# wyf0912/ContextGS

Measured on AMD Instinct MI355X. Metric: views/sec fwd+bwd @1920×1080, 1M anchors, higher is better.
Workload: dtype f32

## Files before the change

### contextgs_amd/_lib.py

```python
from __future__ import annotations

import ctypes as C
import os
import threading

_HERE = os.path.dirname(os.path.abspath(__file__))
LIB_PATH = os.environ.get("CGS_LIB_PATH") or os.path.join(_HERE, "libcgs_hip.so")

_lib = None
_lock = threading.Lock()

c_void_p, c_int, c_int32, c_int64, c_size_t, c_float = C.c_void_p, C.c_int, C.c_int32, C.c_int64, C.c_size_t, C.c_float


class RasterCfg(C.Structure):
    _fields_ = [
        ("image_height", c_int32),
        ("image_width", c_int32),
        ("tanfovx", c_float),
        ("tanfovy", c_float),
        ("scale_modifier", c_float),
        ("prefiltered", c_int32),
        ("debug", c_int32),
        ("viewmatrix", c_void_p),
        ("projmatrix", c_void_p),
        ("campos", c_void_p),
        ("bg", c_void_p),
    ]


class AdamTensor(C.Structure):
    _fields_ = [
        ("p", c_void_p),
        ("g", c_void_p),
        ("m", c_void_p),
        ("v", c_void_p),
        ("numel", c_int64),
        ("beta1", C.c_double),
        ("beta2", C.c_double),
        ("width", c_int32),
        ("step_size", c_float),
        ("bias2_sqrt", c_float),
        ("eps", c_float),
        ("weight_decay", c_float),
    ]


_BWD_HEAD = [C.POINTER(RasterCfg), c_int64, c_int64]
_BWD_WS = [c_void_p, c_size_t, c_void_p, c_size_t, c_void_p, c_size_t]
_BWD_TAIL = [c_void_p, c_size_t, c_void_p]
_BWD_FORMS = _BWD_HEAD + [c_void_p] * 3 + [c_int32] * 2 + [c_void_p] * 5 + _BWD_WS + [c_void_p]
_BWD_MAPS = _BWD_FORMS + [c_void_p] * 3
_BWD_OUT = [c_void_p] * 8 + _BWD_TAIL
_BWD_FEAT = [c_void_p, c_int32, c_void_p, c_void_p]

SIGNATURES = {
    "cgs_version": (c_int, []),
    "cgs_last_error": (C.c_char_p, []),
    "cgs_filter": (c_int, [C.POINTER(RasterCfg), c_int64, c_void_p, c_void_p, c_void_p, c_void_p, c_void_p]),
    "cgs_filter_voxel": (c_int, [C.POINTER(RasterCfg), c_int64, c_void_p, c_void_p, c_int64, c_int, c_void_p, c_void_p, c_void_p]),
    "cgs_raster_geom_bytes": (c_size_t, [c_int64]),
    "cgs_raster_bin_bytes": (c_size_t, [c_int64, c_int64]),
    "cgs_raster_img_bytes": (c_size_t, [c_int32, c_int32]),
    "cgs_raster_bwd_scratch_bytes": (c_size_t, [c_int64]),
    "cgs_raster_preprocess": (c_int, [C.POINTER(RasterCfg), c_int64, c_void_p, c_void_p, c_void_p, c_void_p,
                                      c_void_p, c_void_p, c_size_t, c_void_p, C.POINTER(c_int64), c_void_p]),
    "cgs_raster_preprocess_launch": (c_int, [C.POINTER(RasterCfg), c_int64, c_void_p, c_void_p, c_void_p, c_void_p,
                                             c_void_p, c_void_p, c_size_t, c_void_p, c_void_p, C.POINTER(C.c_uint64)]),
    "cgs_raster_preprocess_launch_ex": (c_int, [C.POINTER(RasterCfg), c_int64, c_void_p, c_void_p, c_void_p, c_int32, c_int32,
                                                c_void_p, c_void_p, c_void_p, c_void_p, c_void_p, c_size_t, c_void_p, c_void_p,
                                                C.POINTER(C.c_uint64)]),
    "cgs_raster_backward_ex": (c_int, _BWD_FORMS + _BWD_OUT),
    "cgs_raster_render_aux": (c_int, [C.POINTER(RasterCfg), c_int64, c_int64, c_void_p, c_size_t, c_void_p, c_size_t,
                                      c_void_p, c_size_t, c_void_p, c_void_p, c_void_p, c_void_p]),
    "cgs_raster_backward_aux": (c_int, _BWD_MAPS + _BWD_OUT),
    "cgs_raster_bwd_aux_scratch_bytes": (c_size_t, [c_int64]),
    "cgs_raster_preprocess_launch_opt": (c_int, [C.POINTER(RasterCfg), c_int64, c_void_p, c_void_p, c_void_p, c_int32, c_int32,
                                                 c_void_p, c_void_p, c_void_p, c_void_p, c_void_p, c_size_t, c_void_p, c_void_p,
                                                 C.POINTER(C.c_uint64), C.c_uint32]),
    "cgs_raster_backward_opt": (c_int, _BWD_MAPS + _BWD_OUT + [C.c_uint32]),
    "cgs_raster_render_features": (c_int, [C.POINTER(RasterCfg), c_int64, c_int64, c_void_p, c_size_t, c_void_p, c_size_t,
                                           c_void_p, c_size_t, c_void_p, c_int32, c_void_p, c_void_p]),
    "cgs_raster_backward_feat": (c_int, _BWD_MAPS + _BWD_OUT + [C.c_uint32] + _BWD_FEAT),
    "cgs_raster_bwd_abs_scratch_bytes": (c_size_t, [c_int64]),
    "cgs_raster_backward_abs": (c_int, _BWD_MAPS + _BWD_OUT + [C.c_uint32] + _BWD_FEAT),
    "cgs_raster_bwd_det_bytes": (c_size_t, [c_int64, c_int64, c_int32]),
    "cgs_raster_backward_det": (c_int, _BWD_MAPS + _BWD_OUT + [C.c_uint32, c_int32, c_void_p, c_size_t]),
    "cgs_raster_render_geom": (c_int, [C.POINTER(RasterCfg), c_int64, c_int64, c_void_p, c_size_t, c_void_p, c_size_t,
                                       c_void_p, c_size_t, c_void_p, c_void_p, c_void_p, c_void_p, c_void_p]),
    "cgs_raster_backward_geom": (c_int, _BWD_MAPS + _BWD_OUT + [C.c_uint32] + _BWD_FEAT + [c_void_p] * 4),
    "cgs_raster_contrib": (c_int, [C.POINTER(RasterCfg), c_int64, c_int64, c_void_p, c_size_t, c_void_p, c_size_t, c_void_p,
                                   c_size_t, c_void_p, c_int64] + [c_void_p] * 8),
    "cgs_raster_camera_bytes": (c_size_t, [c_int64]),
    "cgs_raster_camera_backward": (c_int, [C.POINTER(RasterCfg), c_int64, c_void_p, c_void_p, c_int32, c_int32, c_void_p, c_void_p,
                                           c_void_p, c_void_p, c_void_p, c_void_p, c_size_t, c_void_p, c_void_p, C.c_uint32,
                                           c_void_p, c_void_p, c_void_p, c_void_p, c_size_t, c_void_p]),
    "cgs_gaussian_normals_fwd": (c_int, [C.POINTER(RasterCfg), c_int64] + [c_void_p] * 5),
    "cgs_gaussian_normals_bwd": (c_int, [C.POINTER(RasterCfg), c_int64] + [c_void_p] * 6),
    "cgs_depth_normals_fwd": (c_int, [c_int32, c_int32, c_float, c_float, c_float] + [c_void_p] * 3),
    "cgs_depth_normals_bwd": (c_int, [c_int32, c_int32, c_float, c_float, c_float] + [c_void_p] * 4),
    "cgs_normal_consistency_fwd": (c_int, [c_int32, c_int32, c_float, c_float, c_float] + [c_void_p] * 5),
    "cgs_normal_consistency_bwd": (c_int, [c_int32, c_int32, c_float, c_float, c_float] + [c_void_p] * 7),
    "cgs_filter_cov": (c_int,[C.POINTER(RasterCfg), c_int64, c_void_p, c_void_p, c_void_p, c_void_p]),
    "cgs_raster_preprocess_wait": (c_int, [C.c_uint64, C.POINTER(c_int64)]),
    "cgs_raster_preprocess_wait2": (c_int, [C.c_uint64, C.POINTER(c_int64), C.POINTER(c_int)]),
    "cgs_debug_set_depth_keys_full": (c_int, [c_int]),
    "cgs_sort_depth_keys": (c_int, [c_void_p, c_void_p, c_void_p, c_void_p, c_void_p, c_int64, c_void_p, c_size_t, c_void_p,
                                    C.c_uint32, c_void_p]),
    "cgs_raster_render_spec": (c_int, [C.POINTER(RasterCfg), c_int64, c_int64, c_void_p, c_size_t, c_void_p, c_size_t,
                                       c_void_p, c_size_t, c_void_p, c_void_p]),
    "cgs_raster_render": (c_int, [C.POINTER(RasterCfg), c_int64, c_int64, c_void_p, c_size_t, c_void_p, c_size_t,
                                  c_void_p, c_size_t, c_void_p, c_void_p]),
    "cgs_raster_backward": (c_int, _BWD_HEAD + [c_void_p] * 6 + _BWD_WS + [c_void_p] * 7 + _BWD_TAIL),
    "cgs_raster_preprocess_expand_launch": (c_int, [C.POINTER(RasterCfg), c_int64, c_int] + [c_void_p] * 9 + [c_int64, c_void_p,
                                                    c_void_p, c_void_p, c_void_p, c_size_t, c_void_p, c_void_p, C.POINTER(C.c_uint64)]),
    "cgs_raster_stats": (c_int, [C.POINTER(RasterCfg), c_void_p, c_size_t, c_void_p, c_void_p]),
    "cgs_debug_set_bin_mode": (c_int, [c_int]),
    "cgs_debug_bin_compare": (c_int, [C.POINTER(RasterCfg), c_int64, c_int64, c_int64, c_void_p, c_size_t, c_void_p, c_size_t,
                                      c_void_p, c_size_t, c_void_p, c_size_t, c_void_p, c_void_p, c_void_p]),
    "cgs_build_info": (C.c_char_p, []),
    "cgs_scan_scratch_bytes": (c_size_t, [c_int64]),
    "cgs_scan_exclusive_u32": (c_int, [c_void_p, c_void_p, c_int64, c_void_p, c_size_t, c_void_p]),
    "cgs_sort_scratch_bytes": (c_size_t, [c_int64]),
    "cgs_sort_pairs_u32": (c_int, [c_void_p, c_void_p, c_void_p, c_void_p, c_void_p, c_void_p, c_int64, c_int, c_int,
                                   c_void_p, c_size_t, c_void_p]),
    "cgs_quantize_anchor": (c_int, [c_void_p, c_void_p, c_void_p, c_int64, c_int, c_void_p, c_void_p, c_void_p]),
    "cgs_ste_multistep": (c_int, [c_void_p, c_void_p, c_int64, c_int64, c_int, c_void_p, c_void_p]),
    "cgs_entropy_gaussian_fwd": (c_int, [c_void_p, c_void_p, c_void_p, c_void_p, c_int64, c_int64, c_void_p, c_int,
                                         c_void_p, c_void_p]),
    "cgs_entropy_gaussian_bwd": (c_int, [c_void_p, c_void_p, c_void_p, c_void_p, c_int64, c_int64, c_void_p, c_int,
                                         c_void_p, c_void_p, c_void_p, c_void_p, c_void_p, c_void_p]),
    "cgs_mlp2_forward": (c_int, [c_int, c_int, c_int, c_int, c_void_p, c_int64, c_void_p, c_void_p, c_void_p, c_void_p,
                                 c_void_p, c_int64, c_void_p, c_int64, c_void_p]),
    "cgs_mlp2_backward": (c_int, [c_int, c_int, c_int, c_int, c_void_p, c_int64, c_void_p, c_void_p, c_void_p, c_void_p, c_void_p,
                                  c_int64, c_void_p, c_void_p, c_int64, c_int, c_void_p, c_void_p, c_void_p, c_void_p,
                                  c_void_p, c_void_p, c_int64, c_void_p, c_size_t, c_void_p]),
    "cgs_mlp2_backward_rows": (c_int, [c_int, c_int, c_int, c_int, c_void_p, c_int64, c_void_p, c_void_p, c_void_p, c_void_p,
                                       c_void_p, c_int64, c_void_p, c_void_p, c_int64, c_int, c_void_p, c_void_p, c_void_p,
                                       c_void_p, c_void_p, c_void_p, c_void_p, c_int64, c_void_p, c_size_t, c_void_p]),
    "cgs_mlp_wgrad_scratch_bytes": (c_size_t, []),
    "cgs_mlp2_wgrad": (c_int, [c_int, c_int, c_int, c_void_p, c_int64, c_void_p, c_void_p, c_int64, c_void_p, c_void_p, c_void_p,
                               c_void_p, c_void_p, c_int64, c_void_p, c_size_t, c_void_p]),
    "cgs_anchor_mlp3_wgrad": (c_int, [c_void_p, c_int64] + [c_void_p] * 9 + [c_int64, c_void_p, c_size_t, c_void_p]),
    "cgs_anchor_mlp3_forward": (c_int, [c_void_p, c_int64, c_void_p, c_void_p, c_void_p, c_void_p, c_void_p, c_void_p,
                                        c_void_p, c_void_p, c_int64, c_void_p]),
    "cgs_anchor_mlp3_backward": (c_int, [c_void_p, c_int64, c_void_p, c_void_p, c_void_p, c_void_p, c_void_p, c_void_p,
                                         c_void_p, c_void_p, c_void_p, c_int64, c_void_p, c_void_p, c_void_p, c_void_p,
                                         c_void_p, c_void_p, c_void_p, c_int64, c_void_p, c_size_t, c_void_p]),
    "cgs_anchor_mlp3_forward_rows": (c_int, [c_void_p] * 13 + [c_int64, c_void_p]),
    "cgs_anchor_mlp3_backward_rows": (c_int, [c_void_p] * 22 + [c_int64, c_void_p, c_size_t, c_void_p]),
    "cgs_anchor_mlp3_forward_rows_t": (c_int, [c_void_p] * 13 + [c_int64, c_int, c_void_p]),
    "cgs_anchor_mlp3_backward_rows_t": (c_int, [c_void_p] * 22 + [c_int64, c_int, c_void_p, c_size_t, c_void_p]),
    "cgs_rowcat_fwd": (c_int, [c_int, c_void_p, c_void_p, c_void_p, c_void_p, c_int64, c_void_p, c_void_p]),
    "cgs_rowcat_bwd": (c_int, [c_int, c_void_p, c_void_p, c_void_p, c_void_p, c_void_p, c_int64, c_void_p, c_void_p]),
    "cgs_anchor_mlp3_layout": (c_int, [c_void_p]),
    "cgs_gather_rows_segmented": (c_int, [c_int, c_void_p, c_void_p, c_void_p, c_void_p, c_int64, c_int, c_void_p, c_void_p]),
    "cgs_scatter_rows_sorted": (c_int, [c_void_p, c_void_p, c_int64, c_int64, c_int, c_void_p, c_void_p]),
    "cgs_add_rows": (c_int, [c_void_p, c_void_p, c_int64, c_int64, c_int, c_void_p, c_void_p]),
    "cgs_weighted_sum_scratch_bytes": (c_size_t, []),
    "cgs_weighted_sum_fwd": (c_int, [c_void_p, c_void_p, c_int64, c_void_p, c_float, c_void_p, c_size_t, c_void_p, c_void_p]),
    "cgs_weighted_sum_bwd": (c_int, [c_void_p, c_void_p, c_int64, c_float, c_void_p, c_void_p, c_void_p]),
    "cgs_gather_rows": (c_int, [c_void_p, c_void_p, c_int64, c_int, c_void_p, c_void_p]),
    "cgs_mark_rows": (c_int, [c_void_p, c_int64, c_int64, C.c_uint32, c_void_p, c_void_p]),
    "cgs_zero_unmarked_rows": (c_int, [c_void_p, C.c_uint32, c_int64, c_int, c_void_p, c_void_p, c_void_p]),
    "cgs_rowcat_fwd_masked": (c_int, [c_int, c_void_p, c_void_p, c_void_p, c_void_p, c_void_p, c_int64, c_void_p, c_void_p]),
    "cgs_rowcat_bwd_masked": (c_int, [c_int, c_void_p, c_void_p, c_void_p, c_void_p, c_void_p, c_void_p, c_int64, c_void_p,
                                      c_void_p]),
    "cgs_ctx_gather_bwd": (c_int, [c_void_p, c_int64, c_int64, c_void_p, c_void_p, c_void_p, c_void_p, c_void_p, c_void_p,
                                   c_int, c_int, c_int, c_void_p]),
    "cgs_ctx_gather_bwd_acc": (c_int, [c_void_p, c_int64, c_int64, c_void_p, c_void_p, c_void_p, c_void_p, c_void_p, c_void_p,
                                       c_int, c_int, c_int, c_int, c_void_p]),
    "cgs_noise_quant_fwd": (c_int, [c_void_p, c_void_p, c_void_p, c_void_p, c_void_p, c_int64, c_int, c_int, c_int,
                                    C.c_uint64, c_float, c_float, c_float, c_void_p, c_void_p, c_void_p, c_void_p,
                                    c_void_p, c_void_p]),
    "cgs_hyper_noise_gather": (c_int, [c_void_p, c_void_p, c_int64, c_int, C.c_uint64, c_void_p, c_void_p]),
    "cgs_eb_bits_scratch_bytes": (c_size_t, []),
    "cgs_eb_bits_fwd": (c_int, [c_void_p, c_void_p, c_void_p, c_int64, c_int, c_void_p, c_size_t, c_void_p, c_void_p]),
    "cgs_eb_bits_bwd": (c_int, [c_void_p, c_void_p, c_void_p, c_void_p, c_int64, c_int, c_void_p, c_void_p, c_void_p]),
    "cgs_rate_finish_fwd": (c_int, [c_void_p, c_int, c_void_p, c_float, C.c_double, C.c_double, C.c_double, c_float, c_void_p,
                                    c_void_p, c_void_p]),
    "cgs_rate_finish_bwd": (c_int, [c_void_p, c_int, c_float, C.c_double, C.c_double, C.c_double, c_void_p, c_void_p, c_void_p]),
    "cgs_rate_finish_bwd4": (c_int, [c_void_p, c_void_p, c_void_p, c_void_p, c_int, c_float, C.c_double, C.c_double, C.c_double, c_void_p,
                                     c_void_p, c_void_p]),
    "cgs_ctx_choose_blocks": (c_size_t, [c_int64]),
    "cgs_ctx_choose_flags": (c_int, [c_void_p, c_int64, c_void_p, c_void_p, C.c_uint64, c_float, c_void_p, c_void_p, c_void_p,
                                     c_void_p, c_int, c_void_p, c_void_p, c_void_p, c_void_p]),
    "cgs_ctx_choose_slot_ints": (c_int, []),
    "cgs_ctx_choose_flags_slots": (c_int, [c_void_p, c_int64, c_void_p, c_void_p, C.c_uint64, c_float, c_void_p, c_void_p, c_void_p,
                                           c_void_p, c_int, c_void_p, c_void_p, c_void_p, c_int, c_void_p]),
    "cgs_ctx_choose_compact": (c_int, [c_void_p, c_void_p, c_void_p, c_int64, c_void_p, c_int, c_void_p, c_void_p, c_void_p,
                                       c_void_p, c_void_p, c_void_p]),
    "cgs_means_accum_doubles": (c_size_t, []),
    "cgs_means_finalize": (c_int, [c_void_p, c_int64, c_int64, c_int64, c_void_p, c_void_p]),
    "cgs_noise_quant_bwd": (c_int, [c_void_p, c_void_p, c_void_p, c_void_p, c_void_p, c_int64, c_int, c_int, c_int,
                                    C.c_uint64, c_float, c_float, c_float, c_void_p, c_void_p, c_void_p, c_void_p,
                                    c_void_p, c_void_p, c_void_p, c_void_p, c_void_p, c_void_p, c_void_p]),
    "cgs_ctx_level_fwd": (c_int, [c_int, c_void_p, c_int64, c_void_p, c_void_p, c_void_p, c_void_p, c_int64, c_void_p, c_void_p,
                                  c_int64] + [c_void_p] * 8 + [C.c_uint64, c_float, c_float, c_float] + [c_void_p] * 7),
    "cgs_ctx_level_bwd_scratch_bytes": (c_size_t, []),
    "cgs_ctx_level_bwd": (c_int, [c_int] + [c_void_p] * 9 + [c_int64, C.c_uint64, c_float, c_float, c_float, c_void_p, c_int64] +
                          [c_void_p] * 4 + [c_int64] + [c_void_p] * 11 + [c_size_t, c_void_p]),
    "cgs_ctx_level_bwd2": (c_int, [c_int] + [c_void_p] * 9 + [c_int64, C.c_uint64, c_float, c_float, c_float, c_void_p, c_int64] +
                           [c_void_p] * 4 + [c_int64] + [c_void_p] * 12 + [c_size_t, c_void_p]),
    "cgs_ctx_level_hidden_bytes": (c_size_t, [c_int64]),
    "cgs_ctx_level_fwd_h": (c_int, [c_int, c_void_p, c_int64, c_void_p, c_void_p, c_void_p, c_void_p, c_int64, c_void_p, c_void_p,
                                    c_int64] + [c_void_p] * 8 + [C.c_uint64, c_float, c_float, c_float] + [c_void_p] * 8),
    "cgs_ctx_level_bwd_h": (c_int, [c_int] + [c_void_p] * 9 + [c_int64, C.c_uint64, c_float, c_float, c_float, c_void_p, c_int64] +
                            [c_void_p] * 4 + [c_int64] + [c_void_p] * 13 + [c_size_t, c_void_p]),
    "cgs_level_rate_fwd": (c_int, [c_void_p] * 9 + [c_int, c_int64, c_int, c_int, c_int64, c_void_p, c_void_p]),
    "cgs_level_rate_bwd": (c_int, [c_void_p] * 9 + [c_int, c_int64, c_int, c_int, c_int64] + [c_void_p] * 7 +
                           [c_int, c_void_p]),
    "cgs_rate_sub_fwd": (c_int, [c_int, c_void_p, c_int64, c_void_p, c_int64] + [c_void_p] * 10 + [c_int, c_void_p, c_void_p]),
    "cgs_rate_sub_bwd_scratch_bytes": (c_size_t, [c_int, c_int64]),
    "cgs_rate_sub_bwd": (c_int, [c_int, c_void_p, c_int64, c_void_p, c_int64] + [c_void_p] * 10 + [c_int] + [c_void_p] * 12 +
                         [c_size_t, c_void_p]),
    "cgs_eb_likelihood_fwd": (c_int, [c_void_p, c_void_p, c_int64, c_int, c_void_p, c_void_p]),
    "cgs_eb_likelihood_bwd": (c_int, [c_void_p, c_void_p, c_void_p, c_int64, c_int, c_void_p, c_void_p, c_void_p]),
    "cgs_ac_max_bytes": (c_size_t, [c_int64]),
    "cgs_cdf_float_to_u16_host": (c_int, [c_void_p, c_int64, c_int, c_void_p]),
    "cgs_ac_encode_table_host": (c_int, [c_void_p, c_int, c_void_p, c_int64, c_void_p, c_size_t, C.POINTER(c_size_t)]),
    "cgs_ac_decode_table_host": (c_int, [c_void_p, c_int, c_int64, c_void_p, c_size_t, c_void_p]),
    "cgs_ac_encode_const_host": (c_int, [c_void_p, c_int, c_void_p, c_int64, c_void_p, c_size_t, C.POINTER(c_size_t)]),
    "cgs_ac_decode_const_host": (c_int, [c_void_p, c_int, c_int64, c_void_p, c_size_t, c_void_p]),
    "cgs_gaussian_stream_minmax": (c_int, [c_void_p, c_void_p, c_int64, c_void_p, c_int, c_void_p, c_void_p, c_void_p]),
    "cgs_gaussian_ac_encode": (c_int, [c_void_p, c_void_p, c_void_p, c_void_p, c_int64, c_void_p, c_int, c_void_p,
                                       c_void_p, c_void_p, c_void_p, c_void_p, c_void_p, c_void_p]),
    "cgs_gaussian_ac_decode": (c_int, [c_void_p, c_void_p, c_void_p, c_int64, c_void_p, c_int, c_void_p, c_void_p,
                                       c_void_p, c_void_p, c_void_p, c_void_p]),
    "cgs_gaussian_ac_encode_lanes": (c_int, [c_void_p, c_void_p, c_void_p, c_void_p, c_int64, c_void_p, c_int, c_void_p,
                                             c_void_p, c_void_p, c_void_p, c_void_p, c_void_p, c_void_p]),
    "cgs_gaussian_ac_decode_lanes": (c_int, [c_void_p, c_void_p, c_void_p, c_int64, c_void_p, c_int, c_void_p, c_void_p,
                                             c_void_p, c_void_p, c_void_p, c_void_p, c_void_p]),
    "cgs_lanes_compact": (c_int, [c_void_p, c_void_p, c_void_p, c_void_p, c_int, c_void_p, c_int, c_void_p]),
    "cgs_lanes_block_slot_bytes": (c_size_t, [c_int64, c_int]),
    "cgs_table_ac_encode_lanes": (c_int, [c_void_p, c_void_p, c_void_p, c_int, c_void_p, c_int, c_void_p, c_void_p, c_void_p,
                                          c_void_p, c_void_p, c_void_p, c_void_p]),
    "cgs_table_ac_decode_lanes": (c_int, [c_void_p, c_void_p, c_int, c_void_p, c_int, c_void_p, c_void_p, c_void_p, c_int64,
                                          c_void_p, c_void_p, c_void_p, c_int64, c_void_p, c_void_p]),
    "cgs_bernoulli_ac_encode": (c_int, [c_void_p, C.c_uint32, c_void_p, c_int, c_void_p, c_void_p, c_void_p, c_void_p, c_void_p]),
    "cgs_bernoulli_ac_decode": (c_int, [C.c_uint32, c_void_p, c_int, c_void_p, c_void_p, c_void_p, c_void_p]),
    "cgs_means3_scratch_bytes": (c_size_t, []),
    "cgs_means3": (c_int, [c_void_p, c_int64, c_void_p, c_int64, c_int, c_void_p, c_int64, c_void_p, c_size_t, c_void_p,
                           c_void_p]),
    "cgs_mask_ste_fwd":(c_int, [c_void_p, c_int64, c_int, c_void_p, c_void_p, c_void_p]),
    "cgs_mask_ste_bwd": (c_int, [c_void_p, c_void_p, c_int64, c_void_p, c_void_p]),
    "cgs_knn_scratch_bytes": (c_size_t, [c_int64]),
    "cgs_knn_mean_dist2": (c_int, [c_void_p, c_int64, c_void_p, c_void_p, c_size_t, c_void_p]),
    "cgs_streams_compact":(c_int, [c_void_p, c_void_p, c_void_p, c_void_p, c_int, c_void_p, c_void_p]),
    "cgs_anchor_order_scratch_bytes": (c_size_t, [c_int64]),
    "cgs_anchor_order": (c_int, [c_void_p, c_int64, c_void_p, c_void_p, c_void_p, c_void_p, c_size_t, c_void_p]),
    "cgs_anchor_pack_slot_bytes": (c_size_t, [c_int]),
    "cgs_anchor_pack": (c_int, [c_void_p, c_int64, c_int, c_void_p, c_void_p, c_void_p, c_void_p, c_void_p, c_void_p]),
    "cgs_anchor_unpack": (c_int, [c_void_p, c_int64, c_int, c_void_p, c_void_p, c_void_p, c_void_p, c_void_p, c_void_p]),
    "cgs_pread_ranges": (c_int, [c_int, c_void_p, c_void_p, c_void_p, c_void_p, c_int]),
    "cgs_pwrite_ranges": (c_int, [c_int, c_void_p, c_void_p, c_void_p, c_void_p, c_int]),
    "cgs_gaussian_cdf_table": (c_int, [c_void_p, c_void_p, c_void_p, c_int64, c_int64, c_int, c_int, c_void_p, c_void_p]),
    "cgs_rans_max_bytes": (c_size_t, [c_int64]),
    "cgs_rans_encode_host": (c_int, [c_void_p, c_int, c_int64, c_void_p, c_int, c_void_p, c_void_p, c_int, c_void_p,
                                     c_size_t, C.POINTER(c_size_t)]),
    "cgs_rans_decode_host": (c_int, [c_void_p, c_size_t, c_int, c_int64, c_void_p, c_int, c_void_p, c_void_p, c_int,
                                     c_void_p]),
    "cgs_rans_decode_rows_host": (c_int, [c_void_p, c_size_t, c_int, c_int64, c_void_p, c_int, c_void_p, c_void_p, c_int,
                                          c_void_p, c_void_p, c_int64]),
    "cgs_prof_enable": (c_int, [c_int]),
    "cgs_prof_count": (c_int, []),
    "cgs_prof_name": (C.c_char_p, [c_int]),
    "cgs_prof_read": (c_int, [c_int, C.POINTER(C.c_double), C.POINTER(c_int64)]),
    "cgs_densify_stats": (c_int, [c_int64, c_int] + [c_void_p] * 11),
    "cgs_densify_stats_ex": (c_int, [c_int64, c_int] + [c_void_p] * 11 + [c_int32, c_int32]),
    "cgs_nonzero_scratch_bytes": (c_size_t, [c_int64]),
    "cgs_nonzero_launch": (c_int, [c_void_p, c_int64, c_void_p, c_void_p, c_size_t, c_void_p, C.POINTER(C.c_uint64)]),
    "cgs_nonzero_wait": (c_int, [C.c_uint64, C.POINTER(c_int64)]),
    "cgs_level_key_range": (c_int, [c_void_p, c_int64, c_void_p, c_void_p, c_void_p]),
    "cgs_level_unique_scratch_bytes": (c_size_t, [c_int64]),
    "cgs_level_unique": (c_int, [c_void_p, c_int64, c_void_p, c_void_p, c_void_p, c_void_p, c_void_p, c_void_p,
                                 C.POINTER(c_int64), c_void_p, c_size_t, c_void_p]),
    "cgs_compact_rows": (c_int, [c_int, c_void_p, c_void_p, c_void_p, c_void_p, c_float, c_void_p, c_int64, c_void_p]),
    "cgs_adam_step": (c_int, [c_int, C.POINTER(AdamTensor), c_void_p, c_int64, c_void_p]),
    "cgs_l1_ssim_partials": (c_size_t, [c_int, c_int, c_int]),
    "cgs_l1_ssim_fwd": (c_int, [c_void_p, c_void_p, c_int, c_int, c_int, c_void_p, c_void_p, c_void_p]),
    "cgs_l1_ssim_bwd": (c_int, [c_void_p, c_void_p, c_void_p, c_void_p, c_int, c_int, c_int, c_void_p, c_void_p]),
    "cgs_l1_ssim_finish": (c_int, [c_void_p, c_int, c_int, c_int, c_float, c_void_p, c_void_p]),
    "cgs_l1_ssim_bwd_loss": (c_int, [c_void_p, c_void_p, c_void_p, c_void_p, c_void_p, c_float, c_int, c_int, c_int, c_void_p, c_void_p]),
    "cgs_reg_partials": (c_size_t, [c_int64]),
    "cgs_scaling_reg_fwd": (c_int, [c_void_p, c_int64, c_void_p, c_void_p]),
    "cgs_scaling_reg_bwd": (c_int, [c_void_p, c_void_p, c_int64, c_void_p, c_void_p]),
    "cgs_sigmoid_mean_fwd": (c_int, [c_void_p, c_int64, c_void_p, c_void_p]),
    "cgs_sigmoid_mean_bwd": (c_int, [c_void_p, c_void_p, c_int64, c_void_p, c_void_p]),
    "cgs_anchor_gen_count": (c_int, [c_void_p] * 14 + [c_int64, c_int, C.POINTER(c_int64), c_void_p]),
    "cgs_anchor_gen_write": (c_int, [c_void_p] * 20 + [c_int64, c_int, c_void_p]),
    "cgs_anchor_gen_bwd_scratch_bytes": (c_size_t, [c_int64, c_int]),
    "cgs_anchor_gen_backward": (c_int, [c_void_p] * 32 + [c_int64, c_int, c_int, c_void_p, c_size_t, c_void_p]),
    "cgs_expand_scratch_bytes": (c_size_t, [c_int64, c_int]),
    "cgs_expand_count": (c_int, [c_int64, c_int, c_void_p, c_void_p, c_void_p, c_void_p, c_void_p, c_void_p, c_void_p,
                                 c_size_t, C.POINTER(c_int64), c_void_p]),
    "cgs_expand_count_launch": (c_int, [c_int64, c_int, c_void_p, c_void_p, c_void_p, c_void_p, c_void_p, c_void_p, c_void_p,
                                        c_size_t, c_void_p, C.POINTER(C.c_uint64)]),
    "cgs_expand_count_wait": (c_int, [C.c_uint64, C.POINTER(c_int64)]),
    "cgs_expand_write": (c_int, [c_int64, c_int] + [c_void_p] * 15),
    "cgs_expand_backward": (c_int, [c_int64, c_int] + [c_void_p] * 22),
}


def lib() -> C.CDLL:
    global _lib
    if _lib is not None:
        return _lib
    with _lock:
        if _lib is not None:
            return _lib
        import torch
        if not os.path.exists(LIB_PATH):
            raise RuntimeError(
                f"{LIB_PATH} not found. Build it with `python -m contextgs_amd.build` "
                "(or __graft_entry__.build()); contextgs_amd has no CPU fallback.")
        handle = C.CDLL(LIB_PATH)
        for name, (res, args) in SIGNATURES.items():
            fn = getattr(handle, name)
            fn.restype = res
            fn.argtypes = args
        if os.environ.get("CGS_LIB_PATH"):
            import sys
            from . import build as _build
            info = (handle.cgs_build_info() or b"").decode()
            want = _build.source_digest()
            if info.split("|")[0] != want and not os.environ.get("CGS_LIB_ALLOW_STALE"):
                raise RuntimeError(f"CGS_LIB_PATH={LIB_PATH} was built from other sources ({info.split('|')[0][:12]}... vs "
                                   f"{want[:12]}...): rebuild it (tools/variant_lib.sh) or set CGS_LIB_ALLOW_STALE=1")
            print(f"[contextgs_amd] variant library {LIB_PATH} ({info[:12]}...|{info.split('|')[-1]})", file=sys.stderr)
        if os.environ.get("CGS_BIN_MODE"):
            if handle.cgs_debug_set_bin_mode(int(os.environ["CGS_BIN_MODE"])) != 0:
                raise RuntimeError("CGS_BIN_MODE must be 0, 1 or 2")
        _lib = handle
    return _lib


def check(rc: int, what: str) -> None:
    if rc != 0:
        msg = lib().cgs_last_error()
        raise RuntimeError(f"{what} failed (code {rc}): {msg.decode() if msg else '?'}")


def ptr(t) -> int:
    if t is None:
        return None
    assert t.is_contiguous(), "libcgs_hip takes dense row-major buffers"
    return t.data_ptr()


_raw_stream = None


def current_stream() -> int:
    global _raw_stream
    import torch
    if _raw_stream is None:
        _raw_stream = getattr(torch._C, "_cuda_getCurrentRawStream", False)
    if _raw_stream:
        return _raw_stream(torch.cuda.current_device())
    return torch.cuda.current_stream().cuda_stream


def require_device(*tensors) -> None:
    import torch
    cur = None
    for t in tensors:
        if t is None:
            continue
# ... 9 lines not shown
```

### contextgs_amd/csrc/cgs_internal.h

```cpp
#pragma once
#include <hip/hip_runtime.h>
#include <stdint.h>
#include <stdio.h>
#include "../../include/cgs.h"

#define CGS_TILE 16
#define CGS_WAVE 64

void cgs_set_error(const char *fmt, ...);
uint64_t cgs_new_ticket(int kind);

#define CGS_CHECK_HIP(expr)                                                   \
    do {                                                                      \
        hipError_t e__ = (expr);                                              \
        if (e__ != hipSuccess) {                                              \
            cgs_set_error("%s:%d: %s -> %s", __FILE__, __LINE__, #expr,       \
                          hipGetErrorString(e__));                            \
            return CGS_ERR_HIP;                                               \
        }                                                                     \
    } while (0)

#define CGS_CHECK_LAUNCH(stream, debug)                                       \
    do {                                                                      \
        CGS_CHECK_HIP(hipGetLastError());                                     \
// ... 28 lines not shown
    template <typename T> T *take(size_t count) {
        off = cgs_align_up(off, 256);
        size_t bytes = count * sizeof(T);
        T *r = (T *)(base ? base + off : nullptr);
        off += bytes;
        if (base && off > cap) ok = false;
        return r;
    }
    size_t used() const { return cgs_align_up(off, 256); }
};

struct CgsGeom {
    float4 *rec;
    uint32_t *depth_key;
    uint32_t *tiles;
    uint2 *rect;
    uint32_t *order;
    uint32_t *offsets;
    uint32_t *sort_a;
    uint32_t *sort_b;
    uint32_t *sort_c;
    uint32_t *sort_d;
    uint32_t *total;
    void *scratch;
    size_t scratch_bytes;
};

struct CgsBin {
    uint32_t *tile_key_a;
    uint32_t *tile_key_b;
    uint32_t *gid_a;
    uint32_t *gid_b;
    uint32_t *tile_key_c;
    uint32_t *gid_sorted;
    void *scratch;
    size_t scratch_bytes;
    uint32_t *bk_tab;
    uint32_t *bk_counts;
    uint32_t *bk_scan;
    void *bk_scan_scratch;
    size_t bk_scan_scratch_bytes;
};

struct CgsImg {
    uint2 *ranges;
    float *final_T;
    uint32_t *n_contrib;
    uint32_t *tile_last;
    uint32_t *tile_order;
};

size_t cgs_geom_carve(CgsGeom *g, void *ws, size_t bytes, int64_t P);
size_t cgs_bin_carve(CgsBin *b, void *ws, size_t bytes, int64_t P, int64_t R);
size_t cgs_img_carve(CgsImg *im, void *ws, size_t bytes, int32_t H, int32_t W);

int cgs_launch_preprocess(const cgs_raster_cfg *cfg, int64_t P, const float *means3D,
                          const float *colors, const float *opacities, const float *scales,
                          const float *rotations, CgsGeom &g, int32_t *radii, bool filter_only,
                          hipStream_t stream, bool aa = false);
int cgs_launch_emit_pairs(const cgs_raster_cfg *cfg, int64_t P, CgsGeom &g, CgsBin &b,
                          hipStream_t stream);
int cgs_launch_ranges(const cgs_raster_cfg *cfg, int64_t R, CgsBin &b, CgsImg &im,
                      hipStream_t stream);
int cgs_launch_gather_rects(int64_t P, CgsGeom &g, hipStream_t stream);
bool cgs_tile_bin16_ok(int tile_bits);
bool cgs_tile_bin_buckets_ok(const cgs_raster_cfg *cfg);
bool cgs_tile_bin_buckets_fits(int64_t R);
int64_t cgs_bucket_count_slots(int64_t R);
size_t cgs_bucket_tab_words(void);
int cgs_launch_tile_bin_buckets(const cgs_raster_cfg *cfg, int64_t P, int64_t R, CgsGeom &g, CgsBin &b, CgsImg &im,
                                hipStream_t stream, const uint32_t *R_dev);
int cgs_launch_tile_bin16(const cgs_raster_cfg *cfg, int64_t P, int64_t R, int tile_bits, CgsGeom &g, CgsBin &b, CgsImg &im,
                          hipStream_t stream, const uint32_t *R_dev = nullptr);
int cgs_launch_blend_fwd_rows(const cgs_raster_cfg *cfg, CgsGeom &g, CgsBin &b, CgsImg &im, float *out_color,
                              hipStream_t stream);
int cgs_launch_blend_bwd_rows(const cgs_raster_cfg *cfg, CgsGeom &g, CgsBin &b, CgsImg &im, const float *dL_dout,
                              float *dL_dmean2D_px, float *dL_dconic, float *dL_dopacity, float *dL_dcolors,
                              hipStream_t stream, float *dL_dabs_px = nullptr);
int cgs_launch_tile_order(const cgs_raster_cfg *cfg, CgsImg &im, hipStream_t stream);
int cgs_launch_blend_bwd_rows_det(const cgs_raster_cfg *cfg, int64_t P, int64_t R, CgsGeom &g, CgsBin &b, CgsImg &im,
                                  const float *dL_dout, const uint32_t *slot_base, void *slots, float *dL_dmean2D_px,
                                  float *dL_dconic, float *dL_dopacity, float *dL_dcolors, float *dL_dz, float *dL_dabs_px,
                                  hipStream_t stream);
int cgs_launch_blend_fwd(const cgs_raster_cfg *cfg, CgsGeom &g, CgsBin &b, CgsImg &im,
                         float *out_color, hipStream_t stream);
int cgs_launch_blend_bwd(const cgs_raster_cfg *cfg, CgsGeom &g, CgsBin &b, CgsImg &im,
                         const float *dL_dout, float *dL_dmean2D_px, float *dL_dconic,
                         float *dL_dopacity, float *dL_dcolors, hipStream_t stream, float *dL_dabs_px = nullptr);
int cgs_launch_preprocess_bwd(const cgs_raster_cfg *cfg, int64_t P, const float *means3D,
                              const float *scales, const float *rotations,
                              const int32_t *radii, const float *dL_dmean2D_px,
                              const float *dL_dconic, float *dL_dmeans3D, float *dL_dmeans2D,
                              float *dL_dscales, float *dL_drotations, hipStream_t stream,
                              const float *aa_opacities = nullptr, float *aa_dL_dopacities = nullptr,
                              const float *dL_dabs_px = nullptr);

struct CgsExpandSrc {
    int64_t n_anchor;
    int K;
    const uint8_t *flags;
    const uint32_t *pos;
    const float *anchor, *gscaling, *offsets, *neural_opacity, *color_in, *cov_in;
    const int64_t *src_row;
};
int cgs_launch_expand_preprocess(const cgs_raster_cfg *cfg, const CgsExpandSrc &x, float *scaling_out, float *xyz_out,
                                 float *rot_out, CgsGeom &g, int32_t *radii, hipStream_t stream);

#ifdef __HIPCC__
__device__ __forceinline__ int64_t cgs_xcd_item(int64_t n_items) {
    const int64_t chunk = (n_items + 7) / 8;
    const int64_t t = (int64_t)(blockIdx.x & 7u) * chunk + (int64_t)(blockIdx.x >> 3);
    return ((int64_t)(blockIdx.x >> 3) < chunk && t < n_items) ? t : -1;
}
#endif
static inline unsigned cgs_xcd_grid(int64_t n_items) { return (unsigned)(8 * ((n_items + 7) / 8)); }
#define CGS_TICKET_SLOTS 8
#define CGS_TICKET_BYTES ((CGS_TICKET_SLOTS + 1) * 128)
#ifdef __HIPCC__
__device__ __forceinline__ void cgs_publish(double *slot, double v) {
    const unsigned long long old = atomicExch((unsigned long long *)slot, (unsigned long long)__double_as_longlong(v));
    asm volatile("" ::"v"(old) : "memory");
}
__device__ __forceinline__ double cgs_published(const double *slot) {
    return __longlong_as_double((long long)__hip_atomic_load((const unsigned long long *)slot, __ATOMIC_RELAXED, __HIP_MEMORY_SCOPE_AGENT));
}
__device__ __forceinline__ bool cgs_ticket_last(unsigned int *t) {
    const unsigned nb = gridDim.x, S = CGS_TICKET_SLOTS, slot = blockIdx.x % S;
    const unsigned in_slot = (nb - slot + S - 1) / S;
    if (atomicAdd(&t[32 * (1 + slot)], 1u) != in_slot - 1u) return false;
    t[32 * (1 + slot)] = 0u;
    if (atomicAdd(&t[0], 1u) != (nb < S ? nb : S) - 1u) return false;
    t[0] = 0u;
    __threadfence();
    return true;
}
#endif
int cgs_launch_digit_scan(uint32_t *hist, uint32_t *totals, int digits, int64_t ncols, hipStream_t stream);

static inline int cgs_tiles_x(const cgs_raster_cfg *c) { return (c->image_width + CGS_TILE - 1) / CGS_TILE; }
static inline int cgs_tiles_y(const cgs_raster_cfg *c) { return (c->image_height + CGS_TILE - 1) / CGS_TILE; }

int cgs_launch_wgrad2(const float *P, int64_t ldp, int DA, const float *Q, int64_t ldq, int DB, float *dW, float *db,
                      int64_t n, int num_cus, void *scratch, size_t scratch_bytes, hipStream_t s);
size_t cgs_wgrad_scratch_bytes_for(int num_cus);
int cgs_launch_mlp2_bwd_recompute(int in, int hid, int out, const float *X, int64_t ldx, const float *W1,
                                  const float *b1, const float *W2, const float *dY, int64_t ldy, float *dX,
                                  int64_t lddx, int acc, float *dZ1, float *dW2, float *db2, int64_t n, int num_cus,
                                  void *scratch, size_t scratch_bytes, hipStream_t s);
struct CgsWgProduct { const float *P; int64_t ldp; int DA; const float *Q; int64_t ldq; int DB; float *dW; float *db; };
int cgs_launch_wgrad_multi(const CgsWgProduct *prods, int nprod, int64_t n, int num_cus, void *scratch,
                           size_t scratch_bytes, hipStream_t s);
int cgs_launch_wgrad_reduce(const float *partial, int blocks, const CgsWgProduct *prods, int nprod, hipStream_t s);
int cgs_launch_wgrad_reduce_assign(const float *partial, int blocks, const CgsWgProduct *prods, int nprod, hipStream_t s);
```

### contextgs_amd/csrc/mlp_wgrad.hip

```cpp
#include "cgs_internal.h"
#include "mlp_frag.h"

typedef int i32x4 __attribute__((ext_vector_type(4)));

struct WgStream {
    __amdgpu_buffer_rsrc_t rsrc;
    int ld4;
    int col4;
    bool m[4];
    bool partial;
    bool narrow;
};

__device__ __forceinline__ WgStream wg_stream(const float *base, int64_t ld, int dim, int group, int c, int64_t r_begin,
                                              int64_t r_end, bool narrow = false) {
    WgStream st;
    st.narrow = narrow;
    const float *p = base + r_begin * ld;
    const int64_t rows = r_end - r_begin;
    const uint32_t bytes = rows > 0 ? (uint32_t)(((rows - 1) * ld + dim) * 4) : 0u;
    st.rsrc = __builtin_amdgcn_make_buffer_rsrc((void *)p, 0, bytes, 0x00020000);
    st.ld4 = (int)ld * 4;
    const int col0 = narrow ? 64 * group + c : 64 * group + 4 * c;
    st.col4 = col0 * 4;
// ... 157 lines not shown
        if (e < DADB) dW[e] += t;
        else if (db) db[e - DADB] += t;
    }
}

static int wgrad_blocks_per_cu() {
    static int v = 0;
    if (!v) {
        const char *e = nullptr;
        v = e ? atoi(e) : 1;
        if (v < 1) v = 1;
        if (v > 2) v = 2;
    }
    return v;
}

size_t cgs_wgrad_scratch_bytes_for(int num_cus) { return (size_t)2 * num_cus * 25000 * sizeof(float); }

int cgs_launch_wgrad2(const float *P, int64_t ldp, int DA, const float *Q, int64_t ldq, int DB, float *dW, float *db,
                      int64_t n, int num_cus, void *scratch, size_t scratch_bytes, hipStream_t s) {
    if (n <= 0) return CGS_OK;
    constexpr int UNR = 2;
    const int GA = (DA + 63) / 64, GB = (DB + 63) / 64, npairs = GA * GB;
    const int E = DA * DB + DA;
    if (npairs > 8 || E > WG_MAX_E) { cgs_set_error("wgrad: %d x %d not supported", DA, DB); return CGS_ERR_ARG; }
    const int nsub = 8 / npairs;
    int64_t blocks = (n + 255) / 256;
    int64_t cap = (int64_t)(scratch ? wgrad_blocks_per_cu() : 1) * num_cus;
    if (scratch) {
        const int64_t fit = (int64_t)(scratch_bytes / ((size_t)E * sizeof(float)));
        if (fit < 1) { cgs_set_error("wgrad: scratch too small"); return CGS_ERR_ARG; }
        if (cap > fit) cap = fit;
    }
    if (blocks > cap) blocks = cap;
    int64_t rpb = (n + blocks - 1) / blocks;
    const int64_t quantum = (int64_t)nsub * 4 * UNR;
    rpb = (rpb + quantum - 1) / quantum * quantum;
    blocks = (n + rpb - 1) / rpb;
#define WG_LAUNCH(U)                                                                                                  \
    hipLaunchKernelGGL((wgrad4_kernel<U>), dim3((unsigned)blocks), dim3(512), 0, s, P, ldp, DA, Q, ldq, DB, dW, db, n, rpb, \
                       GB, npairs, nsub, (float *)scratch)
    if (UNR == 4) WG_LAUNCH(4);
    else if (UNR == 1) WG_LAUNCH(1);
    else WG_LAUNCH(2);
#undef WG_LAUNCH
    CGS_CHECK_HIP(hipGetLastError());
    if (scratch) {
        hipLaunchKernelGGL(wgrad_reduce_kernel, dim3((unsigned)((E + 63) / 64)), dim3(256), 0, s, (const float *)scratch,
                           (int)blocks, E, DA * DB, dW, db);
        CGS_CHECK_HIP(hipGetLastError());
    }
    return CGS_OK;
}

#define WGM_MAX_TASKS 16
#define WGM_MAX_PROD 4
#define WGM_MAX_E 25000
struct WgmTask {
    const float *P, *Q;
    int ldp, ldq, DA, DB, ga, gb, img_off;
    int narrow;
};
struct WgmArgs {
    WgmTask t[WGM_MAX_TASKS];
    int ntask, nsub, E;
};
struct WgmProducts {
    float *dW[WGM_MAX_PROD], *db[WGM_MAX_PROD];
    int off[WGM_MAX_PROD + 1], dadb[WGM_MAX_PROD];
    int nprod;
};

template <int UNR>
__global__ void __launch_bounds__(1024)
    wgrad_multi_kernel(WgmArgs a, int64_t n, int64_t rows_per_block, float *__restrict__ partial) {
    __shared__ float img[WGM_MAX_E];
    const int tid = threadIdx.x, lane = tid & 63, g = lane >> 4, c = lane & 15;
    const int wave = __builtin_amdgcn_readfirstlane(tid >> 6);
    for (int i = tid; i < a.E; i += 1024) img[i] = 0.f;
    const int ti = wave % a.ntask, sub = wave / a.ntask;
    const int nsub = sub < a.nsub ? a.nsub : 0;
    const float *P = nullptr, *Q = nullptr;
    int ldp = 0, ldq = 0, DA = 0, DB = 0, ga = 0, gb = 0, img_off = 0, narrow = 0;
#pragma unroll
    for (int k = 0; k < WGM_MAX_TASKS; ++k)
        if (k == ti) {
            P = a.t[k].P; Q = a.t[k].Q; ldp = a.t[k].ldp; ldq = a.t[k].ldq; DA = a.t[k].DA; DB = a.t[k].DB;
            ga = a.t[k].ga; gb = a.t[k].gb; img_off = a.t[k].img_off; narrow = a.t[k].narrow;
        }
    const bool nA = narrow & 1, nB = narrow & 2;
    f32x4 acc[4][4], bsum = (f32x4){0.f, 0.f, 0.f, 0.f};
#pragma unroll
    for (int ja = 0; ja < 4; ++ja)
#pragma unroll
        for (int jb = 0; jb < 4; ++jb) acc[ja][jb] = (f32x4){0.f, 0.f, 0.f, 0.f};
    if (nsub > 0) {
        const int64_t r_begin = (int64_t)blockIdx.x * rows_per_block;
        const int64_t r_end = min(n, r_begin + rows_per_block);
        const WgStream sa = wg_stream(P, ldp, DA, ga, c, r_begin, r_end, nA);
        const WgStream sb = wg_stream(Q, ldq, DB, gb, c, r_begin, r_end, nB);
        const int rows = (int)(r_end - r_begin), stride = nsub * 4 * UNR;
        int row0 = sub * 4 * UNR;
        WgFrag<UNR> f0, f1;
        wg_fetch<UNR>(f0, sa, sb, row0, g);
        for (; row0 < rows; row0 += 2 * stride) {
            wg_fetch<UNR>(f1, sa, sb, row0 + stride, g);
            WG_FENCE();
            wg_consume<UNR>(f0, sa, sb, acc, bsum);
            WG_FENCE();
            wg_fetch<UNR>(f0, sa, sb, row0 + 2 * stride, g);
            WG_FENCE();
            wg_consume<UNR>(f1, sa, sb, acc, bsum);
            WG_FENCE();
        }
    }
    __syncthreads();
    for (int s = 0; s < a.nsub; ++s) {
        if (nsub > 0 && sub == s) {
            float *const outW = img + img_off;
            float *const outb = outW + DA * DB;
#pragma unroll
            for (int ja = 0; ja < 4; ++ja) {
                if (ja > 0 && nA) break;
#pragma unroll
                for (int r = 0; r < 4; ++r) {
                    const int ar = nA ? 64 * ga + 4 * g + r : 64 * ga + 4 * (4 * g + r) + ja;
                    if (ar >= DA) continue;
#pragma unroll
                    for (int jb = 0; jb < 4; ++jb) {
                        if (jb > 0 && nB) break;
                        const int b = nB ? 64 * gb + c : 64 * gb + 4 * c + jb;
                        if (b < DB) outW[ar * DB + b] += acc[ja][jb][r];
                    }
                }
            }
            if (gb == 0) {
#pragma unroll
                for (int j = 0; j < 4; ++j) {
                    if (j > 0 && nA) break;
                    float v = bsum[j];
                    v += __shfl_xor(v, 16);
                    v += __shfl_xor(v, 32);
                    const int ac = nA ? 64 * ga + c : 64 * ga + 4 * c + j;
                    if (g == 0 && ac < DA) outb[ac] += v;
                }
            }
        }
        __syncthreads();
    }
    float *dst = partial + (int64_t)blockIdx.x * a.E;
    for (int i = tid; i < a.E; i += 1024) dst[i] = img[i];
}

__global__ void __launch_bounds__(256)
    wgrad_multi_reduce_kernel(const float *__restrict__ partial, int blocks, int E, WgmProducts pr, int assign) {
    __shared__ float s[4][64];
    const int tx = threadIdx.x & 63, ty = threadIdx.x >> 6;
    const int e = blockIdx.x * 64 + tx;
    float a0 = 0.f, a1 = 0.f, a2 = 0.f, a3 = 0.f;
    if (e < E) {
        int b = ty;
        for (; b + 12 < blocks; b += 16) {
            a0 += partial[(int64_t)b * E + e];
            a1 += partial[(int64_t)(b + 4) * E + e];
            a2 += partial[(int64_t)(b + 8) * E + e];
            a3 += partial[(int64_t)(b + 12) * E + e];
        }
        for (; b < blocks; b += 4) a0 += partial[(int64_t)b * E + e];
    }
    s[ty][tx] = (a0 + a1) + (a2 + a3);
    __syncthreads();
    if (ty == 0 && e < E) {
        const float t = (s[0][tx] + s[1][tx]) + (s[2][tx] + s[3][tx]);
        int k = 0;
#pragma unroll
        for (int q = 1; q < WGM_MAX_PROD; ++q)
            if (q < pr.nprod && e >= pr.off[q]) k = q;
        float *dW = nullptr, *db = nullptr;
        int off = 0, dadb = 0;
#pragma unroll
        for (int q = 0; q < WGM_MAX_PROD; ++q)
            if (q == k) { dW = pr.dW[q]; db = pr.db[q]; off = pr.off[q]; dadb = pr.dadb[q]; }
        const int le = e - off;
        if (le < dadb) dW[le] = assign ? t : dW[le] + t;
        else if (db) db[le - dadb] = assign ? t : db[le - dadb] + t;
    }
}

#ifndef WG_TAIL_MIN_WAVES
#define WG_TAIL_MIN_WAVES 1
#endif
template <int UNR>
__global__ void __launch_bounds__(512, WG_TAIL_MIN_WAVES)
    wgrad_tail_kernel(const float *__restrict__ P, int64_t ldp, int DA, const float *__restrict__ Q, int64_t ldq, int DB,
                      int64_t n, int64_t rows_per_block, int GA, int nsub, float *__restrict__ partial) {
    __shared__ float img[128 * 80 + 128];
    const int tid = threadIdx.x, lane = tid & 63, g = lane >> 4, c = lane & 15;
    const int wave = __builtin_amdgcn_readfirstlane(tid >> 6);
    const int E = DA * DB + DA;
    for (int i = tid; i < E; i += 512) img[i] = 0.f;
    const int ga = wave % GA, sub = wave / GA;
    const bool active = sub < nsub;
    f32x4 acc[4][4], accT[4], bsum = (f32x4){0.f, 0.f, 0.f, 0.f};
#pragma unroll
    for (int ja = 0; ja < 4; ++ja) {
        accT[ja] = (f32x4){0.f, 0.f, 0.f, 0.f};
#pragma unroll
        for (int jb = 0; jb < 4; ++jb) acc[ja][jb] = (f32x4){0.f, 0.f, 0.f, 0.f};
    }
    if (active) {
        const int64_t r_begin = (int64_t)blockIdx.x * rows_per_block;
        const int64_t r_end = min(n, r_begin + rows_per_block);
        const WgStream sa = wg_stream(P, ldp, DA, ga, c, r_begin, r_end);
        const WgStream sb = wg_stream(Q, ldq, DB, 0, c, r_begin, r_end);
        const WgStream st = wg_stream(Q, ldq, DB, 1, c, r_begin, r_end, true);
        const int rows = (int)(r_end - r_begin), stride = nsub * 4 * UNR;
        int row0 = sub * 4 * UNR;
        WgFrag<UNR> f0, f1;
        float t0[UNR], t1[UNR];
        auto fetch = [&](WgFrag<UNR> &f, float (&t)[UNR], int rel) {
            wg_fetch<UNR>(f, sa, sb, rel, g);
#pragma unroll
            for (int q = 0; q < UNR; ++q) t[q] = wg_load4(st, rel + 4 * q + g)[0];
        };
        auto consume = [&](const WgFrag<UNR> &f, const float (&t)[UNR]) {
            wg_consume<UNR>(f, sa, sb, acc, bsum);
#pragma unroll
            for (int q = 0; q < UNR; ++q) {
                const f32x4 a = wg_mask(sa, f.a[q]);
                const float tv = st.m[0] ? t[q] : 0.f;
#pragma unroll
                for (int ja = 0; ja < 4; ++ja) accT[ja] = frag_mfma(a[ja], tv, accT[ja]);
            }
        };
        fetch(f0, t0, row0);
        for (; row0 < rows; row0 += 2 * stride) {
            fetch(f1, t1, row0 + stride);
            WG_FENCE();
            consume(f0, t0);
            WG_FENCE();
            fetch(f0, t0, row0 + 2 * stride);
            WG_FENCE();
            consume(f1, t1);
            WG_FENCE();
        }
    }
    __syncthreads();
    for (int s = 0; s < nsub; ++s) {
        if (active && sub == s) {
            float *const outW = img, *const outb = img + DA * DB;
#pragma unroll
            for (int ja = 0; ja < 4; ++ja)
#pragma unroll
                for (int r = 0; r < 4; ++r) {
                    const int ar = 64 * ga + 4 * (4 * g + r) + ja;
                    if (ar >= DA) continue;
#pragma unroll
                    for (int jb = 0; jb < 4; ++jb) outW[ar * DB + 4 * c + jb] += acc[ja][jb][r];
                    if (64 + c < DB) outW[ar * DB + 64 + c] += accT[ja][r];
                }
#pragma unroll
            for (int j = 0; j < 4; ++j) {
                float v = bsum[j];
                v += __shfl_xor(v, 16);
                v += __shfl_xor(v, 32);
                const int ac = 64 * ga + 4 * c + j;
                if (g == 0 && ac < DA) outb[ac] += v;
            }
        }
        __syncthreads();
    }
    float *dst = partial + (int64_t)blockIdx.x * E;
    for (int i = tid; i < E; i += 512) dst[i] = img[i];
}

static int launch_wgrad_tail(const CgsWgProduct &p, int64_t n, int num_cus, void *scratch, size_t scratch_bytes, hipStream_t s) {
    constexpr int UNR = 2;
    const int GA = (p.DA + 63) / 64, nsub = 8 / GA, E = p.DA * p.DB + p.DA;
    int64_t blocks = (n + 255) / 256;
    int64_t cap = (int64_t)num_cus * 2;
    const int64_t fit_blocks = (int64_t)(scratch_bytes / ((size_t)E * sizeof(float)));
    if (cap > fit_blocks) cap = fit_blocks;
    if (blocks > cap) blocks = cap;
    int64_t rpb = (n + blocks - 1) / blocks;
    const int64_t quantum = (int64_t)nsub * 4 * UNR;
    rpb = (rpb + quantum - 1) / quantum * quantum;
    blocks = (n + rpb - 1) / rpb;
    hipLaunchKernelGGL((wgrad_tail_kernel<UNR>), dim3((unsigned)blocks), dim3(512), 0, s, p.P, p.ldp, p.DA, p.Q, p.ldq, p.DB, n, rpb,
                       GA, nsub, (float *)scratch);
    CGS_CHECK_HIP(hipGetLastError());
    hipLaunchKernelGGL(wgrad_reduce_kernel, dim3((unsigned)((E + 63) / 64)), dim3(256), 0, s, (const float *)scratch, (int)blocks, E,
                       p.DA * p.DB, p.dW, p.db);
    CGS_CHECK_HIP(hipGetLastError());
    return CGS_OK;
}

int cgs_launch_wgrad_multi(const CgsWgProduct *prods, int nprod, int64_t n, int num_cus, void *scratch,
                           size_t scratch_bytes, hipStream_t s) {
    if (n <= 0 || nprod <= 0) return CGS_OK;
    if (nprod == 1 && scratch && prods[0].DB > 64 && prods[0].DB <= 80 && prods[0].DA <= 128 && prods[0].db &&
        (size_t)(prods[0].DA * prods[0].DB + prods[0].DA) * sizeof(float) <= scratch_bytes)
        return launch_wgrad_tail(prods[0], n, num_cus, scratch, scratch_bytes, s);
    WgmArgs a;
    WgmProducts pr;
    int ntask = 0, E = 0;
    bool fits = scratch != nullptr && nprod <= WGM_MAX_PROD;
    for (int k = 0; k < nprod && fits; ++k) {
        const CgsWgProduct &p = prods[k];
        const int GA = (p.DA + 63) / 64, GB = (p.DB + 63) / 64;
        pr.dW[k] = p.dW; pr.db[k] = p.db; pr.off[k] = E; pr.dadb[k] = p.DA * p.DB;
        for (int ga = 0; ga < GA && fits; ++ga)
            for (int gb = 0; gb < GB; ++gb) {
                if (ntask >= WGM_MAX_TASKS) { fits = false; break; }
                const int narrow = (p.DA - 64 * ga <= 16 ? 1 : 0) | (p.DB - 64 * gb <= 16 ? 2 : 0);
                a.t[ntask++] = WgmTask{p.P, p.Q, (int)p.ldp, (int)p.ldq, p.DA, p.DB, ga, gb, E, narrow};
            }
        E += p.DA * p.DB + p.DA;
    }
    if (fits && E > WGM_MAX_E) fits = false;
    if (fits && (size_t)E * sizeof(float) > scratch_bytes) fits = false;
    if (!fits) {
        for (int k = 0; k < nprod; ++k) {
            const CgsWgProduct &p = prods[k];
            int rc = cgs_launch_wgrad2(p.P, p.ldp, p.DA, p.Q, p.ldq, p.DB, p.dW, p.db, n, num_cus, scratch, scratch_bytes, s);
            if (rc) return rc;
        }
        return CGS_OK;
    }
    for (int k = ntask; k < WGM_MAX_TASKS; ++k) a.t[k] = WgmTask{nullptr, nullptr, 0, 0, 0, 0, 0, 0, 0, 0};
    {
        bool uniform = ntask > 0;
        for (int k = 1; k < ntask; ++k) uniform = uniform && a.t[k].narrow == a.t[0].narrow;
        for (int k = 0; k < ntask; ++k)
            if (!uniform) a.t[k].narrow = 0;
        a.nsub = 16 / ntask;
    }
    for (int k = nprod; k < WGM_MAX_PROD; ++k) { pr.dW[k] = nullptr; pr.db[k] = nullptr; pr.off[k] = E; pr.dadb[k] = 0; }
    pr.off[WGM_MAX_PROD] = E;
    pr.nprod = nprod;
#ifndef WGM_UNR
#define WGM_UNR 2
#endif
    constexpr int UNR = WGM_UNR;
    a.ntask = ntask;
    a.E = E;
#ifndef WGM_MIN_ROWS
#define WGM_MIN_ROWS 256
#endif
    int64_t blocks = (n + WGM_MIN_ROWS - 1) / WGM_MIN_ROWS;
    int64_t cap = num_cus;
    const int64_t fit_blocks = (int64_t)(scratch_bytes / ((size_t)E * sizeof(float)));
    if (cap > fit_blocks) cap = fit_blocks;
    if (blocks > cap) blocks = cap;
    int64_t rpb = (n + blocks - 1) / blocks;
    const int64_t quantum = (int64_t)a.nsub * 4 * UNR;
    rpb = (rpb + quantum - 1) / quantum * quantum;
    blocks = (n + rpb - 1) / rpb;
    hipLaunchKernelGGL((wgrad_multi_kernel<UNR>), dim3((unsigned)blocks), dim3(1024), 0, s, a, n, rpb, (float *)scratch);
    CGS_CHECK_HIP(hipGetLastError());
    hipLaunchKernelGGL(wgrad_multi_reduce_kernel, dim3((unsigned)((E + 63) / 64)), dim3(256), 0, s, (const float *)scratch,
                       (int)blocks, E, pr, 0);
    CGS_CHECK_HIP(hipGetLastError());
    return CGS_OK;
}

static int wgrad_reduce_launch(const float *partial, int blocks, const CgsWgProduct *prods, int nprod, int assign, hipStream_t s);
int cgs_launch_wgrad_reduce(const float *partial, int blocks, const CgsWgProduct *prods, int nprod, hipStream_t s) {
    return wgrad_reduce_launch(partial, blocks, prods, nprod, 0, s);
}
int cgs_launch_wgrad_reduce_assign(const float *partial, int blocks, const CgsWgProduct *prods, int nprod, hipStream_t s) {
    return wgrad_reduce_launch(partial, blocks, prods, nprod, 1, s);
}
static int wgrad_reduce_launch(const float *partial, int blocks, const CgsWgProduct *prods, int nprod, int assign, hipStream_t s) {
    if (nprod <= 0 || nprod > WGM_MAX_PROD || blocks <= 0) { cgs_set_error("wgrad_reduce: bad args"); return CGS_ERR_ARG; }
    WgmProducts pr;
    int E = 0;
    for (int k = 0; k < nprod; ++k) {
        pr.dW[k] = prods[k].dW; pr.db[k] = prods[k].db; pr.off[k] = E; pr.dadb[k] = prods[k].DA * prods[k].DB;
        E += prods[k].DA * prods[k].DB + prods[k].DA;
    }
    for (int k = nprod; k < WGM_MAX_PROD; ++k) { pr.dW[k] = nullptr; pr.db[k] = nullptr; pr.off[k] = E; pr.dadb[k] = 0; }
    pr.off[WGM_MAX_PROD] = E;
    pr.nprod = nprod;
    hipLaunchKernelGGL(wgrad_multi_reduce_kernel, dim3((unsigned)((E + 63) / 64)), dim3(256), 0, s, partial, blocks, E, pr, assign);
    CGS_CHECK_HIP(hipGetLastError());
    return CGS_OK;
}
```

### contextgs_amd/csrc/rate_sub.hip

```cpp
#include "cgs_internal.h"
#include "mlp_frag.h"
#include "buf_access.h"
#include "ctx_rows.h"
#include "rate_math.h"

#define RS_NB 6
#define RS_NT2 12
#define RS_OP 192
#define RS_SA 116
#define RS_OUT 175
#define RS_K 10
#ifndef RS_WAVES_F
#define RS_WAVES_F 8
#endif
#ifndef RS_WAVES_B
#define RS_WAVES_B 8
#endif

__host__ __device__ __forceinline__ int rs_w2row(int op) {
    const int u = op >> 4, b = u >> 1, sc = u & 1, l = op & 15;
    if (b < 3) { const int e = 16 * b + l; return sc ? 50 + e : e; }
    if (b == 3) {
        if (l < 2) return sc ? 98 + l : 48 + l;
        if (l >= 4 && l < 8) return (sc ? 106 : 100) + (l - 4);
        if (l >= 8 && l < 10) return (sc ? 110 : 104) + (l - 8);
        return -1;
    }
    const int e = (b == 4 ? 0 : 16) + l;
    if (e >= 30) return -1;
    return (sc ? 142 : 112) + e;
}

__device__ __forceinline__ int rs_w2perm(int row) {
    int sc = 0, e = row, base;
    if (row < 100) { sc = row >= 50; e = row - 50 * sc; base = e < 48 ? 32 * (e >> 4) + (e & 15) : 96 + (e - 48); }
    else if (row < 112) { sc = row >= 106; e = row - 100 - 6 * sc; base = e < 4 ? 100 + e : 104 + (e - 4); }
    else { sc = row >= 142; e = row - 112 - 30 * sc; base = e < 16 ? 128 + e : 160 + (e - 16); }
    return base + 16 * sc;
}

struct RsArgs {
    const float *X;
    const int64_t *loc;
    const float *W1, *b1, *W2, *b2;
    const float *yf, *ys, *yo, *Q;
    const float *masks;
    const float *x_means;
    int64_t n, m;
    int use_clamp;
    float *sums;
    const float *g_sums;
    float *side_f, *side_s, *side_o, *side_Q;
    float *dx_sub;
    float *d_masks;
    float *dZ2t, *Ht, *dZ1t, *Xt;
};

template <int IN>
struct RsOps {
    f32x4 xb[ClShape<IN>::NTI];
    ClRow y;
    f32x4 q3, mk4, mk5;
};

template <int IN, bool BWD>
__global__ void __launch_bounds__((BWD ? RS_WAVES_B : RS_WAVES_F) * 64) rs_main_kernel(RsArgs a) {
    constexpr int RS_WAVES = BWD ? RS_WAVES_B : RS_WAVES_F;
    constexpr int NTI = ClShape<IN>::NTI, XP = ClShape<IN>::XP, SB = ClShape<IN>::SB;
    __shared__ __attribute__((aligned(16))) float W2n[RS_OP * RS_SA];
    __shared__ __attribute__((aligned(16))) float W1n[CL_HP * SB];
    __shared__ float b1s[CL_HP];
    __shared__ float b2p[RS_OP];
    __shared__ float part[RS_WAVES][3];
    const int tid = threadIdx.x, nthr = RS_WAVES * 64;
    for (int i = tid; i < (RS_OP * RS_SA + CL_HP * SB) / 4; i += nthr) {
        float *dst = i < RS_OP * RS_SA / 4 ? W2n + 4 * i : W1n + 4 * (i - RS_OP * RS_SA / 4);
        *(f32x4 *)dst = (f32x4){0.f, 0.f, 0.f, 0.f};
    }
    for (int i = tid; i < CL_HP; i += nthr) b1s[i] = i < CL_HID ? a.b1[i] : 0.f;
    for (int i = tid; i < RS_OP; i += nthr) {
        const int row = rs_w2row(i);
        b2p[i] = row >= 0 ? a.b2[row] : 0.f;
    }
    __syncthreads();
    {
        constexpr int N2 = (RS_OUT - 3) * CL_HID / 4;
        constexpr int PER = (N2 + RS_WAVES * 64 - 1) / (RS_WAVES * 64);
        f32x4 v[PER];
#pragma unroll
        for (int k = 0; k < PER; ++k) {
            const int i = tid + k * nthr;
            v[k] = i < N2 ? *(const f32x4 *)(a.W2 + 4 * i) : (f32x4){0.f, 0.f, 0.f, 0.f};
        }
#pragma unroll
        for (int k = 0; k < PER; ++k) {
            const int i = tid + k * nthr;
            if (i < N2) {
                const int row = (4 * i) / CL_HID, h = (4 * i) % CL_HID;
                *(f32x4 *)(W2n + rs_w2perm(row) * RS_SA + h) = v[k];
            }
        }
        constexpr int N1 = CL_HID * IN;
        constexpr int PER1 = (N1 + RS_WAVES * 64 - 1) / (RS_WAVES * 64);
        float w[PER1];
#pragma unroll
        for (int k = 0; k < PER1; ++k) {
            const int i = tid + k * nthr;
            w[k] = i < N1 ? a.W1[i] : 0.f;
        }
#pragma unroll
        for (int k = 0; k < PER1; ++k) {
            const int i = tid + k * nthr;
            if (i < N1) W1n[(i / IN) * SB + i % IN] = w[k];
        }
    }
    __syncthreads();

    const int lane = tid & 63, wave = tid >> 6, g = lane >> 4, c = lane & 15;
    const int64_t m = a.m, ntiles = (m + 15) / 16;
    const uint64_t nb = (uint64_t)a.n, mb = (uint64_t)m, tb = (uint64_t)ntiles * 64;
    const ClBuf bX = cl_buf(a.X, nb * IN * 4), bLoc = cl_buf(a.loc, mb * 8), bQ = cl_buf(a.Q, nb * 12),
                bM = cl_buf(a.masks, mb * RS_K * 4);
    const ClRowBufs YB = {cl_buf(a.yf, nb * CL_D * 4), cl_buf(a.ys, nb * CL_S * 4), cl_buf(a.yo, nb * CL_O * 4)};
    const bool has_masks = a.masks != nullptr;
    float xm[3] = {0.f, 0.f, 0.f}, gsum[3] = {0.f, 0.f, 0.f};
    if (a.use_clamp) { xm[0] = a.x_means[0]; xm[1] = a.x_means[1]; xm[2] = a.x_means[2]; }
    if (BWD) { gsum[0] = a.g_sums[0]; gsum[1] = a.g_sums[1]; gsum[2] = a.g_sums[2]; }
    const int use_clamp = a.use_clamp;
    const int lo4 = (4 * g) / 3, lo5 = (16 + 4 * g) / 3;

    auto idx_issue = [&](int64_t s) { return cl_li64(bLoc, cl_sel(s < m, (uint32_t)s * 8)); };
    auto op_issue = [&](RsOps<IN> &op, int64_t s, int64_t r) {
        const bool v = s < m;
        cl_xrow_load<IN>(bX, (uint32_t)r * (IN * 4), g, v, op.xb);
        cl_row_issue(op.y, YB, (uint32_t)r, g, v);
        op.q3 = cl_l96(bQ, cl_sel(v, (uint32_t)r * 12));
        op.mk4 = cl_l64(bM, cl_sel(v && has_masks, (uint32_t)s * (RS_K * 4) + (uint32_t)lo4 * 4));
        op.mk5 = cl_l64(bM, cl_sel(v && has_masks, (uint32_t)s * (RS_K * 4) + (uint32_t)lo5 * 4));
    };

    const int64_t tstride = (int64_t)gridDim.x * RS_WAVES;
    int64_t tile = (int64_t)blockIdx.x * RS_WAVES + wave;
    float accb[3] = {0.f, 0.f, 0.f};
    RsOps<IN> opn;
    int64_t rn;
    {
        const int64_t s0 = tile < ntiles ? tile * 16 + c : m;
        const int64_t r0 = idx_issue(s0);
        op_issue(opn, s0, r0);
        rn = idx_issue(s0 + tstride * 16);
    }
    for (; tile < ntiles; tile += tstride) {
        const int64_t s = tile * 16 + c, sn = s + tstride * 16;
        const bool valid = s < m;
        asm volatile("" ::: "memory");
        RsOps<IN> op = opn;
        cl_xrow_mask<IN>(g, op.xb);
        cl_row_mask(op.y, g);
        CLB_FENCE();
        op_issue(opn, sn, rn);
        rn = idx_issue(sn + tstride * 16);
        CLB_FENCE();

        f32x4 acc1[CL_NT1];
#pragma unroll
        for (int t = 0; t < CL_NT1; ++t) acc1[t] = (f32x4){0.f, 0.f, 0.f, 0.f};
        {
            f32x4 wc[4], wn[4];
#pragma unroll
            for (int i = 0; i < 4; ++i) wc[i] = *(const f32x4 *)(W1n + (16 * i + c) * SB + 4 * g);
#pragma unroll
            for (int grp = 0; grp < 2 * NTI; ++grp) {
                const int q = grp >> 1, t0 = (grp & 1) * 4, nt = (grp & 1) ? 3 : 4;
                if (grp + 1 < 2 * NTI) {
                    const int qn = (grp + 1) >> 1, tn = ((grp + 1) & 1) * 4;
#pragma unroll
                    for (int i = 0; i < 4; ++i)
                        if (tn + i < CL_NT1) wn[i] = *(const f32x4 *)(W1n + (16 * (tn + i) + c) * SB + 16 * qn + 4 * g);
                }
                CLB_FENCE();
#pragma unroll
                for (int j = 0; j < 4; ++j)
#pragma unroll
                    for (int i = 0; i < 4; ++i)
                        if (i < nt) acc1[t0 + i] = frag_mfma(wc[i][j], op.xb[q][j], acc1[t0 + i]);
                CLB_FENCE();
#pragma unroll
                for (int i = 0; i < 4; ++i) wc[i] = wn[i];
            }
        }
#pragma unroll
        for (int t = 0; t < CL_NT1; ++t)
#pragma unroll
            for (int r = 0; r < 4; ++r) acc1[t][r] = fmaxf(acc1[t][r] + b1s[16 * t + 4 * g + r], 0.f);
        uint32_t hpos = 0;
        if (BWD) {
            const ClBuf bXt = cl_buf(a.Xt, tb * XP * 4), bHt = cl_buf(a.Ht, tb * CL_HP * 4);
#pragma unroll
            for (int q = 0; q < NTI; ++q)
#pragma unroll
                for (int r = 0; r < 4; ++r) {
                    const int col = 16 * q + 4 * g + r;
                    const float v = col == IN ? (valid ? 1.f : 0.f) : op.xb[q][r];
                    cl_s32(bXt, (((uint32_t)tile * XP + (uint32_t)col) * 16 + (uint32_t)c) * 4, v);
                }
#pragma unroll
            for (int t = 0; t < CL_NT1; ++t)
#pragma unroll
                for (int r = 0; r < 4; ++r) {
                    const int col = 16 * t + 4 * g + r;
                    const float v = valid ? (col == CL_HID ? 1.f : acc1[t][r]) : 0.f;
                    cl_s32(bHt, (((uint32_t)tile * CL_HP + (uint32_t)col) * 16 + (uint32_t)c) * 4, v);
                    hpos |= acc1[t][r] > 0.f ? (1u << (4 * t + r)) : 0u;
                }
        }
        f32x4 acc2[RS_NT2];
#pragma unroll
        for (int u = 0; u < RS_NT2; ++u) acc2[u] = (f32x4){0.f, 0.f, 0.f, 0.f};
        {
            f32x4 wa = *(const f32x4 *)(W2n + c * RS_SA + 4 * g), wb = *(const f32x4 *)(W2n + (16 + c) * RS_SA + 4 * g);
#pragma unroll
            for (int grp = 0; grp < CL_NT1 * (RS_NT2 / 2); ++grp) {
                const int t = grp / (RS_NT2 / 2), u = 2 * (grp % (RS_NT2 / 2));
                f32x4 na = wa, nb = wb;
                if (grp + 1 < CL_NT1 * (RS_NT2 / 2)) {
                    const int tn = (grp + 1) / (RS_NT2 / 2), un = 2 * ((grp + 1) % (RS_NT2 / 2));
                    na = *(const f32x4 *)(W2n + (16 * un + c) * RS_SA + 16 * tn + 4 * g);
                    nb = *(const f32x4 *)(W2n + (16 * (un + 1) + c) * RS_SA + 16 * tn + 4 * g);
                }
                CLB_FENCE();
#pragma unroll
                for (int r = 0; r < 4; ++r) {
                    acc2[u] = frag_mfma(wa[r], acc1[t][r], acc2[u]);
                    acc2[u + 1] = frag_mfma(wb[r], acc1[t][r], acc2[u + 1]);
                }
                CLB_FENCE();
                wa = na; wb = nb;
            }
        }
        ClRow sd;
        float gq[3] = {0.f, 0.f, 0.f};
        float pm[4] = {0.f, 0.f, 0.f, 0.f};
#pragma unroll
        for (int b = 0; b < RS_NB; ++b) {
            const f32x4 yv = b < 3 ? op.y.F[b] : (b == 3 ? (g == 0 ? op.y.F[3] : op.y.S) : op.y.O[b - 4]);
            f32x4 gxv = (f32x4){0.f, 0.f, 0.f, 0.f};
#pragma unroll
            for (int r = 0; r < 4; ++r) {
                bool slot = true;
                if (b == 3) slot = g == 1 || ((g == 0 || g == 2) && r < 2);
                if (b == 5) slot = g != 3 || r < 2;
                const int kind = b < 3 ? 0 : (b == 3 ? (g == 0 ? 0 : 1) : 2);
                const bool ok = valid && slot;
                const float mean = acc2[2 * b][r] + b2p[32 * b + 4 * g + r];
                const float scale = acc2[2 * b + 1][r] + b2p[32 * b + 16 + 4 * g + r];
                const float q = kind == 0 ? op.q3[0] : (kind == 1 ? op.q3[1] : op.q3[2]);
                const float xmean = kind == 0 ? xm[0] : (kind == 1 ? xm[1] : xm[2]);
                float w = 1.f;
                int wi = 0;
                if (b >= 4) {
                    wi = (b == 4 ? (4 * g + r) / 3 - lo4 : (16 + 4 * g + r) / 3 - lo5);
                    const f32x4 mk = b == 4 ? op.mk4 : op.mk5;
                    if (has_masks) w = wi ? mk[1] : mk[0];
                }
                const RateTerms rt = rate_terms(yv[r], mean, scale, q, xmean, use_clamp);
                if (!BWD) {
                    const float bits = rate_bits(rt) * w;
                    if (kind == 0) accb[0] += ok ? bits : 0.f;
                    else if (kind == 1) accb[1] += ok ? bits : 0.f;
                    else accb[2] += ok ? bits : 0.f;
                } else {
                    const float gb = (kind == 0 ? gsum[0] : (kind == 1 ? gsum[1] : gsum[2])) * w;
                    const RateGrads G = rate_grads(rt, scale, gb);
                    acc2[2 * b][r] = ok ? G.gm : 0.f;
                    acc2[2 * b + 1][r] = ok ? G.gs : 0.f;
                    gxv[r] = ok ? G.gx : 0.f;
                    const float gqv = ok ? G.gq : 0.f;
                    if (kind == 0) gq[0] += gqv;
                    else if (kind == 1) gq[1] += gqv;
                    else gq[2] += gqv;
                    if (b >= 4) {
                        const float bw = ok ? gsum[2] * rate_bits(rt) : 0.f;
                        const int pi = 2 * (b - 4);
                        pm[pi] += wi ? 0.f : bw;
                        pm[pi + 1] += wi ? bw : 0.f;
                    }
                }
            }
            if (BWD) {
                if (b < 3) sd.F[b] = gxv;
                else if (b == 3) { sd.F[3] = gxv; sd.S = gxv; }
                else sd.O[b - 4] = gxv;
            }
        }
        if (!BWD) continue;

        const ClRowBufs SDB = {cl_buf(a.side_f, mb * CL_D * 4), cl_buf(a.side_s, mb * CL_S * 4), cl_buf(a.side_o, mb * CL_O * 4)};
        cl_row_store(sd, SDB, (uint32_t)s, g, valid);
#pragma unroll
        for (int k = 0; k < 3; ++k) {
            gq[k] += __shfl_xor(gq[k], 16);
            gq[k] += __shfl_xor(gq[k], 32);
        }
        cl_s32(cl_buf(a.side_Q, mb * 12), cl_sel(valid && g < 3, (uint32_t)s * 12 + (uint32_t)g * 4), g == 0 ? gq[0] : (g == 1 ? gq[1] : gq[2]));
        if (a.d_masks) {
            float P[4][4];
#pragma unroll
            for (int gg = 0; gg < 4; ++gg)
#pragma unroll
                for (int i = 0; i < 4; ++i) P[gg][i] = __shfl(pm[i], gg * 16 + c, 64);
            float mw[3] = {0.f, 0.f, 0.f};
#pragma unroll
            for (int j = 0; j < 3; ++j) {
                const int k = g < 3 ? 3 * g + j : 9;
#pragma unroll
                for (int gg = 0; gg < 4; ++gg) {
                    const int l4 = (4 * gg) / 3, l5 = (16 + 4 * gg) / 3;
                    mw[j] += (l4 == k ? P[gg][0] : 0.f) + (l4 + 1 == k ? P[gg][1] : 0.f);
                    mw[j] += (l5 == k ? P[gg][2] : 0.f) + (l5 + 1 == k ? P[gg][3] : 0.f);
                }
            }
            const ClBuf bDm = cl_buf(a.d_masks, mb * RS_K * 4);
            const uint32_t o = (uint32_t)s * (RS_K * 4) + (uint32_t)g * 12;
            cl_s96(bDm, cl_sel(valid && g < 3, o), (f32x4){mw[0], mw[1], mw[2], 0.f});
            cl_s32(bDm, cl_sel(valid && g == 3, o), mw[0]);
        }
        {
            const ClBuf bZ2 = cl_buf(a.dZ2t, tb * RS_OP * 4);
#pragma unroll
            for (int u = 0; u < RS_NT2; ++u)
#pragma unroll
                for (int r = 0; r < 4; ++r)
                    cl_s32(bZ2, (((uint32_t)tile * RS_OP + (uint32_t)(16 * u + 4 * g + r)) * 16 + (uint32_t)c) * 4, acc2[u][r]);
        }
        f32x4 adh[CL_NT1];
#pragma unroll
        for (int t = 0; t < CL_NT1; ++t) adh[t] = (f32x4){0.f, 0.f, 0.f, 0.f};
        {
            float wc[CL_NT1], wn[CL_NT1];
#pragma unroll
            for (int t = 0; t < CL_NT1; ++t) wc[t] = W2n[(4 * g) * RS_SA + 16 * t + c];
#pragma unroll
            for (int st = 0; st < 4 * RS_NT2; ++st) {
                const int u = st >> 2, j = st & 3;
                if (st + 1 < 4 * RS_NT2) {
                    const int un = (st + 1) >> 2, jn = (st + 1) & 3;
#pragma unroll
                    for (int t = 0; t < CL_NT1; ++t) wn[t] = W2n[(16 * un + 4 * g + jn) * RS_SA + 16 * t + c];
                }
                CLB_FENCE();
#pragma unroll
                for (int t = 0; t < CL_NT1; ++t) adh[t] = frag_mfma(wc[t], acc2[u][j], adh[t]);
                CLB_FENCE();
#pragma unroll
                for (int t = 0; t < CL_NT1; ++t) wc[t] = wn[t];
            }
        }
        {
            const ClBuf bZ1 = cl_buf(a.dZ1t, tb * CL_HP * 4);
#pragma unroll
            for (int t = 0; t < CL_NT1; ++t)
#pragma unroll
                for (int r = 0; r < 4; ++r) {
                    adh[t][r] = (hpos >> (4 * t + r)) & 1u ? adh[t][r] : 0.f;
                    cl_s32(bZ1, (((uint32_t)tile * CL_HP + (uint32_t)(16 * t + 4 * g + r)) * 16 + (uint32_t)c) * 4, adh[t][r]);
                }
        }
        f32x4 adx[NTI];
#pragma unroll
        for (int v = 0; v < NTI; ++v) adx[v] = (f32x4){0.f, 0.f, 0.f, 0.f};
        {
            constexpr int NST = 4 * CL_NT1;
            float wc[NTI], wn[NTI];
#pragma unroll
            for (int v = 0; v < NTI; ++v) wc[v] = W1n[(4 * g) * SB + 16 * v + c];
#pragma unroll
            for (int st = 0; st < NST; ++st) {
                const int t = st >> 2, r = st & 3;
                if (st + 1 < NST) {
                    const int tn = (st + 1) >> 2, rn = (st + 1) & 3;
#pragma unroll
                    for (int v = 0; v < NTI; ++v) wn[v] = W1n[(16 * tn + 4 * g + rn) * SB + 16 * v + c];
                }
                CLB_FENCE();
#pragma unroll
                for (int v = 0; v < NTI; ++v) adx[v] = frag_mfma(wc[v], adh[t][r], adx[v]);
                CLB_FENCE();
#pragma unroll
                for (int v = 0; v < NTI; ++v) wc[v] = wn[v];
            }
        }
        cl_xrow_store<IN>(cl_buf(a.dx_sub, mb * IN * 4), (uint32_t)s * (IN * 4), g, valid, adx);
    }
    if (!BWD) {
#pragma unroll
        for (int k = 0; k < 3; ++k) {
            float v = accb[k];
#pragma unroll
            for (int o = 32; o >= 1; o >>= 1) v += __shfl_xor(v, o);
            if (lane == 0) part[wave][k] = v;
        }
        __syncthreads();
        if (tid < 3) {
            float v = 0.f;
            for (int w = 0; w < RS_WAVES; ++w) v += part[w][tid];
            atomicAdd(&a.sums[tid], v);
        }
    }
}

#define RW_WAVES 8
struct RwArgs {
    const float *dZ2t, *Ht, *dZ1t, *Xt;
    int64_t ntiles, tiles_per_block;
    float *partial;
};

template <int NA, int NB>
__device__ __forceinline__ void rw_accumulate(ClBuf A, int colsA, int a0, ClBuf B, int colsB, int64_t t0, int64_t t1, int g, int c,
                                              f32x4 (&acc)[NA][NB]) {
#pragma unroll
    for (int i = 0; i < NA; ++i)
#pragma unroll
        for (int j = 0; j < NB; ++j) acc[i][j] = (f32x4){0.f, 0.f, 0.f, 0.f};
    f32x4 an[2][NA], bn[2][NB];
    auto issue = [&](int64_t tile, f32x4 (&pa)[NA], f32x4 (&pb)[NB]) {
        const bool on = tile < t1;
#pragma unroll
        for (int i = 0; i < NA; ++i)
            pa[i] = cl_l128(A, cl_sel(on, (((uint32_t)tile * (uint32_t)colsA + (uint32_t)(16 * (a0 + i) + c)) * 16 + 4 * (uint32_t)g) * 4));
#pragma unroll
        for (int j = 0; j < NB; ++j)
            pb[j] = cl_l128(B, cl_sel(on, (((uint32_t)tile * (uint32_t)colsB + (uint32_t)(16 * j + c)) * 16 + 4 * (uint32_t)g) * 4));
    };
    auto products = [&](const f32x4 (&av)[NA], const f32x4 (&bv)[NB]) {
#pragma unroll
        for (int r = 0; r < 4; ++r)
#pragma unroll
            for (int i = 0; i < NA; ++i)
#pragma unroll
                for (int j = 0; j < NB; ++j) acc[i][j] = frag_mfma(av[i][r], bv[j][r], acc[i][j]);
    };
    issue(t0, an[0], bn[0]);
    issue(t0 + 1, an[1], bn[1]);
    for (int64_t tile = t0; tile < t1; tile += 2) {
#pragma unroll
        for (int st = 0; st < 2; ++st) {
            f32x4 av[NA], bv[NB];
#pragma unroll
            for (int i = 0; i < NA; ++i) av[i] = an[st][i];
#pragma unroll
            for (int j = 0; j < NB; ++j) bv[j] = bn[st][j];
            CLB_FENCE();
            issue(tile + st + 2, an[st], bn[st]);
            CLB_FENCE();
            products(av, bv);
        }
    }
}

template <int IN>
__global__ void __launch_bounds__(RW_WAVES * 64) rs_wgrad_kernel(RwArgs a) {
    constexpr int NTI = ClShape<IN>::NTI, XP = ClShape<IN>::XP;
    constexpr int E1 = CL_HID * IN + CL_HID, E = E1 + RS_OUT * CL_HID + RS_OUT;
    const int tid = threadIdx.x, lane = tid & 63, wave = tid >> 6, g = lane >> 4, c = lane & 15;
    const int64_t t0 = (int64_t)blockIdx.x * a.tiles_per_block;
    const int64_t t1 = t0 + a.tiles_per_block < a.ntiles ? t0 + a.tiles_per_block : a.ntiles;
    const uint64_t tb = (uint64_t)a.ntiles * 64;
    float *img = a.partial + (int64_t)blockIdx.x * E;
    float *img1 = img, *imgb1 = img + CL_HID * IN, *img2 = img + E1, *imgb2 = img2 + RS_OUT * CL_HID;
    if (wave < 6) {
        f32x4 acc[2][CL_NT1];
        rw_accumulate<2, CL_NT1>(cl_buf(a.dZ2t, tb * RS_OP * 4), RS_OP, 2 * wave, cl_buf(a.Ht, tb * CL_HP * 4), CL_HP, t0, t1, g, c, acc);
#pragma unroll
        for (int i = 0; i < 2; ++i)
#pragma unroll
            for (int r = 0; r < 4; ++r) {
                const int row = rs_w2row(16 * (2 * wave + i) + 4 * g + r);
                if (row < 0) continue;
#pragma unroll
                for (int j = 0; j < CL_NT1; ++j) {
                    const int h = 16 * j + c;
                    if (h < CL_HID) img2[row * CL_HID + h] = acc[i][j][r];
                    else if (h == CL_HID) imgb2[row] = acc[i][j][r];
                }
            }
        if (wave == 0) {
            for (int i = lane; i < 3 * CL_HID; i += 64) img2[(RS_OUT - 3) * CL_HID + i] = 0.f;
            if (lane < 3) imgb2[RS_OUT - 3 + lane] = 0.f;
        }
    } else {
        const ClBuf bA = cl_buf(a.dZ1t, tb * CL_HP * 4), bB = cl_buf(a.Xt, tb * XP * 4);
        auto dump = [&](int t, const f32x4 (&row)[NTI]) {
#pragma unroll
            for (int r = 0; r < 4; ++r) {
                const int hid = 16 * t + 4 * g + r;
                if (hid >= CL_HID) continue;
#pragma unroll
                for (int j = 0; j < NTI; ++j) {
                    const int k = 16 * j + c;
                    if (k < IN) img1[hid * IN + k] = row[j][r];
                    else if (k == IN) imgb1[hid] = row[j][r];
                }
            }
        };
        if (wave == 6) {
            f32x4 acc[4][NTI];
            rw_accumulate<4, NTI>(bA, CL_HP, 0, bB, XP, t0, t1, g, c, acc);
#pragma unroll
            for (int i = 0; i < 4; ++i) dump(i, acc[i]);
        } else {
            f32x4 acc[3][NTI];
            rw_accumulate<3, NTI>(bA, CL_HP, 4, bB, XP, t0, t1, g, c, acc);
#pragma unroll
            for (int i = 0; i < 3; ++i) dump(4 + i, acc[i]);
        }
    }
}

static int rs_cus() {
    static int cus = 0;
    if (!cus) {
        int dev = 0;
        hipDeviceProp_t p;
        if (hipGetDevice(&dev) == hipSuccess && hipGetDeviceProperties(&p, dev) == hipSuccess) cus = p.multiProcessorCount;
        if (cus <= 0) cus = 256;
    }
    return cus;
}

static bool rs_fits(int64_t rows, int64_t row_bytes) { return rows >= 0 && (uint64_t)rows * (uint64_t)row_bytes < CL_MAX_BYTES; }

static int rs_check(const char *what, int in_dim, const float *X, int64_t n, const int64_t *loc, int64_t m, const float *W1,
                    const float *b1, const float *W2, const float *b2, const float *yf, const float *ys, const float *yo,
                    const float *Q, const float *x_means, int use_clamp) {
    if (n < 0 || m < 0 || (in_dim != 71 && in_dim != 15)) { cgs_set_error("%s: bad args (in_dim 71 or 15)", what); return CGS_ERR_ARG; }
    if (m == 0) return CGS_OK;
    if (!X || !loc || !W1 || !b1 || !W2 || !b2 || !yf || !ys || !yo || !Q || (use_clamp && !x_means)) { cgs_set_error("%s: NULL", what); return CGS_ERR_ARG; }
    const int64_t ntiles = (m + 15) / 16;
    if (!rs_fits(n, in_dim * 4) || !rs_fits(n, CL_D * 4) || !rs_fits(m, CL_D * 4) || !rs_fits(ntiles * 16, RS_OP * 4)) {
        cgs_set_error("%s: an operand exceeds 4 GB (n %lld, m %lld)", what, (long long)n, (long long)m);
        return CGS_ERR_ARG;
    }
    return CGS_OK;
}

static int64_t rs_grid(int64_t m, int waves) {
    const int64_t tiles = (m + 15) / 16, want = (tiles + waves - 1) / waves;
    return want < rs_cus() ? want : rs_cus();
}

extern "C" int cgs_rate_sub_fwd(int in_dim, const float *X, int64_t n, const int64_t *loc, int64_t m, const float *W1,
                                const float *b1, const float *W2, const float *b2, const float *yf, const float *ys,
                                const float *yo, const float *Q, const float *masks, const float *x_means, int use_clamp,
                                float *sums3, void *stream) {
    int rc = rs_check("rate_sub_fwd", in_dim, X, n, loc, m, W1, b1, W2, b2, yf, ys, yo, Q, x_means, use_clamp);
    if (rc || m == 0) return rc;
    if (!sums3) { cgs_set_error("rate_sub_fwd: NULL"); return CGS_ERR_ARG; }
    RsArgs a = {};
    a.X = X; a.loc = loc; a.W1 = W1; a.b1 = b1; a.W2 = W2; a.b2 = b2; a.yf = yf; a.ys = ys; a.yo = yo; a.Q = Q; a.masks = masks;
    a.x_means = use_clamp ? x_means : nullptr; a.n = n; a.m = m; a.use_clamp = use_clamp ? 1 : 0; a.sums = sums3;
    const unsigned grid = (unsigned)rs_grid(m, RS_WAVES_F);
    CgsProfScope prof(CGS_PROF_RATE_FWD, (hipStream_t)stream);
    if (in_dim == 71) hipLaunchKernelGGL((rs_main_kernel<71, false>), dim3(grid), dim3(RS_WAVES_F * 64), 0, (hipStream_t)stream, a);
    else hipLaunchKernelGGL((rs_main_kernel<15, false>), dim3(grid), dim3(RS_WAVES_F * 64), 0, (hipStream_t)stream, a);
    CGS_CHECK_HIP(hipGetLastError());
    return CGS_OK;
}

static int64_t rw_blocks(int64_t ntiles) {
    int64_t blocks = (ntiles + 7) / 8;
    if (blocks > rs_cus()) blocks = rs_cus();
    return blocks < 1 ? 1 : blocks;
}

extern "C" size_t cgs_rate_sub_bwd_scratch_bytes(int in_dim, int64_t m) {
    if (m <= 0 || (in_dim != 71 && in_dim != 15)) return 0;
    const int64_t ntiles = (m + 15) / 16, xp = in_dim == 71 ? 80 : 16;
    const int64_t E = (int64_t)CL_HID * in_dim + CL_HID + RS_OUT * CL_HID + RS_OUT;
    return (size_t)(ntiles * 16 * (RS_OP + 2 * CL_HP + xp) + rw_blocks(ntiles) * E) * sizeof(float);
}

extern "C" int cgs_rate_sub_bwd(int in_dim, const float *X, int64_t n, const int64_t *loc, int64_t m, const float *W1,
                                const float *b1, const float *W2, const float *b2, const float *yf, const float *ys,
                                const float *yo, const float *Q, const float *masks, const float *x_means, int use_clamp,
                                const float *g_sums3, float *side_f, float *side_s, float *side_o, float *side_Q, float *dx_sub,
                                float *d_masks, float *dW1, float *db1, float *dW2, float *db2, void *scratch, size_t scratch_bytes,
                                void *stream) {
    int rc = rs_check("rate_sub_bwd", in_dim, X, n, loc, m, W1, b1, W2, b2, yf, ys, yo, Q, x_means, use_clamp);
    if (rc) return rc;
    if (m == 0) { cgs_set_error("rate_sub_bwd: m == 0 (the caller zero-fills the weight gradients of an empty subset)"); return CGS_ERR_ARG; }
    if (!g_sums3 || !side_f || !side_s || !side_o || !side_Q || !dx_sub || !dW1 || !db1 || !dW2 || !db2 || !scratch) {
        cgs_set_error("rate_sub_bwd: NULL");
        return CGS_ERR_ARG;
    }
    if (scratch_bytes < cgs_rate_sub_bwd_scratch_bytes(in_dim, m)) { cgs_set_error("rate_sub_bwd: scratch too small"); return CGS_ERR_WORKSPACE; }
    const int64_t ntiles = (m + 15) / 16, xp = in_dim == 71 ? 80 : 16;
    float *ws = (float *)scratch;
    RsArgs a = {};
    a.X = X; a.loc = loc; a.W1 = W1; a.b1 = b1; a.W2 = W2; a.b2 = b2; a.yf = yf; a.ys = ys; a.yo = yo; a.Q = Q; a.masks = masks;
    a.x_means = use_clamp ? x_means : nullptr; a.n = n; a.m = m; a.use_clamp = use_clamp ? 1 : 0; a.g_sums = g_sums3;
    a.side_f = side_f; a.side_s = side_s; a.side_o = side_o; a.side_Q = side_Q; a.dx_sub = dx_sub; a.d_masks = masks ? d_masks : nullptr;
    a.dZ2t = ws; a.Ht = a.dZ2t + ntiles * 16 * RS_OP; a.dZ1t = a.Ht + ntiles * 16 * CL_HP; a.Xt = a.dZ1t + ntiles * 16 * CL_HP;
    float *partial = a.Xt + ntiles * 16 * xp;
    const unsigned grid = (unsigned)rs_grid(m, RS_WAVES_B);
    {
        CgsProfScope prof(CGS_PROF_RATE_BWD, (hipStream_t)stream);
        if (in_dim == 71) hipLaunchKernelGGL((rs_main_kernel<71, true>), dim3(grid), dim3(RS_WAVES_B * 64), 0, (hipStream_t)stream, a);
        else hipLaunchKernelGGL((rs_main_kernel<15, true>), dim3(grid), dim3(RS_WAVES_B * 64), 0, (hipStream_t)stream, a);
        CGS_CHECK_HIP(hipGetLastError());
    }
    CgsProfScope prof(CGS_PROF_LMLP_WGRAD, (hipStream_t)stream);
    RwArgs w;
    w.dZ2t = a.dZ2t; w.Ht = a.Ht; w.dZ1t = a.dZ1t; w.Xt = a.Xt; w.ntiles = ntiles; w.partial = partial;
    const int64_t blocks = rw_blocks(ntiles);
    w.tiles_per_block = (ntiles + blocks - 1) / blocks;
    const unsigned wgrid = (unsigned)((ntiles + w.tiles_per_block - 1) / w.tiles_per_block);
    if (in_dim == 71) hipLaunchKernelGGL((rs_wgrad_kernel<71>), dim3(wgrid), dim3(RW_WAVES * 64), 0, (hipStream_t)stream, w);
    else hipLaunchKernelGGL((rs_wgrad_kernel<15>), dim3(wgrid), dim3(RW_WAVES * 64), 0, (hipStream_t)stream, w);
    CGS_CHECK_HIP(hipGetLastError());
    const CgsWgProduct prods[2] = {{nullptr, 0, CL_HID, nullptr, 0, in_dim, dW1, db1}, {nullptr, 0, RS_OUT, nullptr, 0, CL_HID, dW2, db2}};
    return cgs_launch_wgrad_reduce_assign(partial, (int)wgrid, prods, 2, (hipStream_t)stream);
}
```

### contextgs_amd/ctx_ops.py

```python
from __future__ import annotations

import ctypes as C
import itertools
import threading
import weakref

import collections
import os

import torch

from . import _lib

_f32 = torch.float32


def _c(t):
    t = t if t.dtype == _f32 else t.float()
    return t if t.is_contiguous() else t.contiguous()


def _ptrs(ts):
    return (C.c_void_p * len(ts))(*[None if t is None else t.data_ptr() for t in ts])


def _ints(v):
    return (C.c_int * len(v))(*v)


def _u8(t):
    return None if t is None else (t if t.dtype == torch.uint8 else t.view(torch.uint8)).contiguous()


class _RowCat(torch.autograd.Function):
    @staticmethod
    def forward(ctx, spec, *srcs):
        srcs = [_c(s) for s in srcs]
        _lib.require_device(*srcs)
        idxs = [sp[0] for sp in spec]
        masks = ctx.masks = [_u8(sp[2]) for sp in spec]
        n = next((i.shape[0] for i in idxs if i is not None), srcs[0].shape[0])
        for s, i in zip(srcs, idxs):
            if i is None and s.shape[0] != n:
                raise ValueError("rowcat: an un-indexed source must have one row per output row")
        widths = [int(s.shape[1]) for s in srcs]
        out = torch.empty(n, sum(widths), dtype=_f32, device=srcs[0].device)
        if n > 0:
            _lib.check(_lib.lib().cgs_rowcat_fwd_masked(len(srcs), _ptrs(srcs), _ptrs(idxs), _ptrs(masks), _ints(widths),
                                                        _ints(widths), n, _lib.ptr(out), _lib.current_stream()),
                       "cgs_rowcat_fwd")
        ctx.spec, ctx.widths, ctx.n = spec, widths, n
        ctx.rows = [int(s.shape[0]) for s in srcs]
        return out

    @staticmethod
    def backward(ctx, g):
        g = _c(g)
        grads, modes = [], []
        for k, ((idx, distinct, _m), w, rows) in enumerate(zip(ctx.spec, ctx.widths, ctx.rows)):
            if not ctx.needs_input_grad[1 + k]:
                grads.append(None)
                modes.append(0)
            elif idx is None:
                grads.append(torch.empty(rows, w, dtype=_f32, device=g.device))
                modes.append(1)
            else:
                full = distinct and ctx.n == rows
                grads.append((torch.empty if full else torch.zeros)(rows, w, dtype=_f32, device=g.device))
                modes.append(1 if distinct else 2)
        if any(modes) and ctx.n > 0:
            _lib.check(_lib.lib().cgs_rowcat_bwd_masked(len(grads), _ptrs(grads), _ptrs([sp[0] for sp in ctx.spec]),
                                                        _ptrs(ctx.masks), _ints(ctx.widths), _ints(ctx.widths), _ints(modes),
                                                        ctx.n, _lib.ptr(g), _lib.current_stream()), "cgs_rowcat_bwd")
        return (None, *grads)


def rowcat(parts):
    spec = tuple((p[1], bool(p[2]), p[3] if len(p) > 3 else None) for p in parts)
    return _RowCat.apply(spec, *[p[0] for p in parts])


def gather_rows_nograd(x, idx):
    x = _c(x)
    n, w = int(idx.shape[0]), int(x[0].numel())
    out = torch.empty((n,) + tuple(x.shape[1:]), dtype=_f32, device=x.device)
    if n > 0:
        _lib.check(_lib.lib().cgs_rowcat_fwd(1, _ptrs([x]), _ptrs([idx]), _ints([w]), _ints([w]), n, _lib.ptr(out),
                                             _lib.current_stream()), "cgs_rowcat_fwd")
    return out


_ROW_STAMPS = {}
_ROW_STAMPS_LOCK = threading.Lock()


def add_rows_(out, idx, g):
    n = int(idx.shape[0])
    if n == 0:
        return out
    w = int(out[0].numel())
    if (out.is_cuda and out.dtype == _f32 and g.dtype == _f32 and out.is_contiguous() and idx.dtype == torch.int64
            and idx.is_contiguous() and 1 <= w <= 256 and int(g.numel()) == n * w):
        g = g.contiguous()
        _lib.check(_lib.lib().cgs_add_rows(_lib.ptr(g), _lib.ptr(idx), n, int(out.shape[0]), w, _lib.ptr(out), _lib.current_stream()),
                   "cgs_add_rows")
        return out
    out.view(out.shape[0], -1).index_add_(0, idx, g.reshape(n, -1).to(out.dtype))
    return out


def zero_unlisted_rows(idx, n_full, arrays):
    if int(n_full) == 0 or not arrays:
        return
    dev = arrays[0].device
    L = _lib.lib()
    key = (str(dev), int(n_full))
    stream = _lib.current_stream()
    with _ROW_STAMPS_LOCK:
        st = _ROW_STAMPS.get(key)
        if st is None or st[1] >= 0xFFFFFFF0:
            if st is None and len(_ROW_STAMPS) >= 8:
                _ROW_STAMPS.pop(next(iter(_ROW_STAMPS)))
            st = _ROW_STAMPS[key] = [torch.zeros(max(int(n_full), 1), dtype=torch.int32, device=dev), 0]
        st[1] += 1
        gen, stamp = st[1], st[0]
        _lib.check(L.cgs_mark_rows(_lib.ptr(idx), int(idx.shape[0]), int(n_full), gen, _lib.ptr(stamp), stream), "cgs_mark_rows")
        for a0 in range(0, len(arrays), 4):
            part = arrays[a0:a0 + 4]
            _lib.check(L.cgs_zero_unmarked_rows(_lib.ptr(stamp), gen, int(n_full), len(part), _ptrs(part),
                                                _ints([int(a[0].numel()) for a in part]), stream), "cgs_zero_unmarked_rows")


_seed_counter = itertools.count(1)


def next_seed() -> int:
    return (torch.initial_seed() * 0x9E3779B97F4A7C15 + next(_seed_counter) * 0xD1B54A32D192ED03) & (2 ** 63 - 1)


class HyperDirect:

    def __init__(self, n_rows: int, channels: int, sizes):
        self.n, self.c, self.sizes = int(n_rows), int(channels), tuple(int(t) for t in sizes)
        self.buf, self.done = None, set()

    def buffer(self, device):
        if self.buf is None:
            self.buf = torch.empty(self.n, self.c, dtype=_f32, device=device)
        return self.buf

    def take(self):
        buf, done = self.buf, self.done
        self.buf, self.done = None, set()
        return buf, done
# ... 122 lines not shown
    def forward(ctx, src, feat, scal, off):
        ctx.src_ref = weakref.ref(src)
        ctx.joined = src.joined
        ctx.set_materialize_grads(False)
        return feat.new_empty(1)

    @staticmethod
    def backward(ctx, _g):
        ctx.joined.clear()
        src = ctx.src_ref()
        if src is None:
            return None, None, None, None
        if src.rows_written != src.rows_read:
            raise RuntimeError("RowSource: a level that read rows in the forward did not run its backward "
                               f"({src.rows_written} of {src.rows_read} rows have gradients)")
        src.anchor_finish()
        gf, gs, go = src.grad_buffers()
        src.grads = None
        need = ctx.needs_input_grad
        return (None, gf.view(src.shapes[0]) if need[1] else None, gs.view(src.shapes[1]) if need[2] else None,
                go.view(src.shapes[2]) if need[3] else None)


class RateSide:

    _ABSENT = (None,) * 5

    def __init__(self):
        self._loan = self._rate = self._branch = None

    def lend(self, X, weights):
        assert self._loan is None, "RateSide: this level's input rows were lent twice"
        self._loan = (X, weights)

    @property
    def lazy(self) -> bool:
        return self._loan is not None

    def loan(self):
        assert self._loan is not None, "RateSide: the level lent nothing (or its backward already took the loan back)"
        return self._loan

    def give(self, smap, f, s, o, q, dx=None, dW=None):
        assert self._rate is None and self._branch is None, "RateSide: rate gradients given twice before the level took them"
        self._rate = (smap, f, s, o, q)
        if dW is not None:
            self._branch = (dx, dW)

    def take(self):
        rate, self._rate = self._rate, None
        return rate if (rate is not None and rate[1].numel() > 0) else self._ABSENT

    def take_branch(self):
        branch, self._branch, self._loan = self._branch, None, None
        return branch if branch is not None else (None, None)


class _NoiseQuant(torch.autograd.Function):
    @staticmethod
    def forward(ctx, xf, xs, xo, qadj, seed, q0, outs, src, rows, token, side):
        qadj = _c(qadj)
        if src is not None:
            xf, xs, xo = src.f, src.s, src.o
            n = int(rows.shape[0])
            assert rows.dtype == torch.int64 and rows.is_contiguous()
            src.rows_read += n
        else:
            xf, xs, xo = _c(xf), _c(xs), _c(xo)
            n = xf.shape[0]
        _lib.require_device(xf, xs, xo, qadj)
        ctx.set_materialize_grads(False)
        D, S, O = xf.shape[1], xs.shape[1], xo.shape[1]
        if outs is None:
            mk = lambda w: torch.empty(n, w, dtype=_f32, device=qadj.device)
            yf, ys, yo = mk(D), mk(S), mk(O)
        else:
            yf, ys, yo = outs
            assert yf.shape == (n, D) and ys.shape == (n, S) and yo.shape == (n, O)
            assert yf.is_contiguous() and ys.is_contiguous() and yo.is_contiguous()
        Q = torch.empty(n, 3, dtype=_f32, device=qadj.device)
        _lib.check(_lib.lib().cgs_noise_quant_fwd(
            _lib.ptr(xf), _lib.ptr(xs), _lib.ptr(xo), _lib.ptr(qadj), _lib.ptr(rows), n, D, S, O, seed,
            q0[0], q0[1], q0[2], _lib.ptr(yf), _lib.ptr(ys), _lib.ptr(yo), _lib.ptr(Q),
            _lib.ptr(src.sums_buffer()) if src is not None else None, _lib.current_stream()), "cgs_noise_quant_fwd")
        ctx.save_for_backward(qadj, rows)
        ctx.dims, ctx.seed, ctx.q0, ctx.src, ctx.side = (n, D, S, O), seed, q0, src, side
        return yf, ys, yo, Q

    @staticmethod
    def backward(ctx, gf, gs, go, gQ):
        qadj, rows = ctx.saved_tensors
        n, D, S, O = ctx.dims
        src = ctx.src
        gf, gs, go, gQ = (None if t is None else _c(t) for t in (gf, gs, go, gQ))
        dq = torch.empty(n, 3, dtype=_f32, device=qadj.device) if (ctx.needs_input_grad[3] or src is not None) else None
        dx = src.grad_buffers() if src is not None else (None, None, None)
        sd = ctx.side.take() if ctx.side is not None else (None,) * 5
        if dq is not None:
            _lib.check(_lib.lib().cgs_noise_quant_bwd(
                _lib.ptr(gf), _lib.ptr(gs), _lib.ptr(go), _lib.ptr(gQ), _lib.ptr(qadj), n, D, S, O, ctx.seed, ctx.q0[0],
                ctx.q0[1], ctx.q0[2], _lib.ptr(dq), _lib.ptr(rows) if src is not None else None, _lib.ptr(dx[0]),
                _lib.ptr(dx[1]), _lib.ptr(dx[2]), *[_lib.ptr(t) for t in sd], _lib.current_stream()), "cgs_noise_quant_bwd")
        if src is not None:
            src.rows_written += n
            gf = gs = go = None
        return gf, gs, go, dq, None, None, None, None, None, None, None


def noise_quant(xf, xs, xo, qadj, q0, seed=None, outs=None, src=None, rows=None, side=None):
    assert side is None or src is not None
    return _NoiseQuant.apply(xf, xs, xo, qadj, next_seed() if seed is None else int(seed),
                             tuple(float(v) for v in q0), outs, src, rows, None if src is None else src.token, side)


def _carve(n, widths, device, zero=False):
    flat = (torch.zeros if zero else torch.empty)(n * sum(widths), dtype=_f32, device=device)
    return [t.view(n, w) for t, w in zip(torch.split(flat, [n * w for w in widths]), widths)]


def _sub_map(loc, n_level):
    m = torch.full((n_level,), -1, dtype=torch.int32, device=loc.device)
    m[loc] = torch.arange(int(loc.shape[0]), dtype=torch.int32, device=loc.device)
    return m


def _level_rate_fwd(lv, masks_p, grows, x_means, use_clamp, K, sums_p, stream):
    yf, ys, yo, Q, pred, loc = lv
    _lib.check(_lib.lib().cgs_level_rate_fwd(
        _lib.ptr(yf), _lib.ptr(ys), _lib.ptr(yo), _lib.ptr(Q), _lib.ptr(loc), _lib.ptr(pred), masks_p, _lib.ptr(grows),
        _lib.ptr(x_means), use_clamp, int(pred.shape[0]), int(yf.shape[1]), K, int(pred.shape[1]), sums_p, stream), "cgs_level_rate_fwd")


def _level_rate_bwd(lv, masks_p, grows, x_means, use_clamp, K, g_p, d_masks_p, compact, stream):
    yf, ys, yo, Q, pred, loc = lv
    n_sub, D = int(pred.shape[0]), int(yf.shape[1])
    d = _carve(n_sub if compact else int(yf.shape[0]), (D, 6, 3 * K, 3), yf.device, zero=not compact)
    d_pred = torch.empty_like(pred)
    _lib.check(_lib.lib().cgs_level_rate_bwd(
        _lib.ptr(yf), _lib.ptr(ys), _lib.ptr(yo), _lib.ptr(Q), _lib.ptr(loc), _lib.ptr(pred), masks_p, _lib.ptr(grows),
        _lib.ptr(x_means), use_clamp, n_sub, D, K, int(pred.shape[1]), g_p, _lib.ptr(d_pred), *[_lib.ptr(t) for t in d], d_masks_p,
        int(compact), stream), "cgs_level_rate_bwd")
    return d, d_pred


def _rate_sub_fwd(side, lv, masks_p, x_means, use_clamp, sums_p, stream):
    yf, ys, yo, Q, _pred, loc = lv
    X, (W1, b1, W2, b2) = side.loan()
    _lib.check(_lib.lib().cgs_rate_sub_fwd(
        int(X.shape[1]), _lib.ptr(X), int(X.shape[0]), _lib.ptr(loc), int(loc.shape[0]), _lib.ptr(W1), _lib.ptr(b1), _lib.ptr(W2),
        _lib.ptr(b2), _lib.ptr(yf), _lib.ptr(ys), _lib.ptr(yo), _lib.ptr(Q), masks_p, _lib.ptr(x_means), use_clamp, sums_p, stream),
        "cgs_rate_sub_fwd")


def _rate_sub_bwd(side, lv, masks_p, x_means, use_clamp, K, g_p, d_masks_p, stream):
    Lc = _lib.lib()
    yf, ys, yo, Q, _pred, loc = lv
    X, W = side.loan()
    n_sub, in_f, dev = int(loc.shape[0]), int(X.shape[1]), yf.device
    *d, dx = _carve(n_sub, (int(yf.shape[1]), 6, 3 * K, 3, in_f), dev)
    wflat = torch.empty(sum(w.numel() for w in W), dtype=_f32, device=dev)
    dW = tuple(t.view(w.shape) for t, w in zip(torch.split(wflat, [w.numel() for w in W]), W))
    ws = torch.empty(int(Lc.cgs_rate_sub_bwd_scratch_bytes(in_f, n_sub)), dtype=torch.uint8, device=dev)
    _lib.check(Lc.cgs_rate_sub_bwd(
        in_f, _lib.ptr(X), int(X.shape[0]), _lib.ptr(loc), n_sub, *[_lib.ptr(w) for w in W], _lib.ptr(yf), _lib.ptr(ys), _lib.ptr(yo),
        _lib.ptr(Q), masks_p, _lib.ptr(x_means), use_clamp, g_p, *[_lib.ptr(t) for t in d], _lib.ptr(dx), d_masks_p,
        *[_lib.ptr(t) for t in dW], _lib.ptr(ws), ws.numel(), stream), "cgs_rate_sub_bwd")
    return d, dx, dW


def _rate_finish_fwd(table_p, levels, hsum, finish, device, stream):
    out = torch.empty(4, dtype=_f32, device=device)
    raw = torch.empty(2 + levels, dtype=_f32, device=device)
    _lib.check(_lib.lib().cgs_rate_finish_fwd(table_p, levels, _lib.ptr(_c(hsum)), *[float(v) for v in finish], _lib.ptr(out),
                                              _lib.ptr(raw), stream), "cgs_rate_finish_fwd")
    return out, raw


def _rate_finish_bwd(gs, levels, finish, device, stream):
    dS = torch.empty(levels, 3, dtype=_f32, device=device)
    dh = torch.empty(1, dtype=_f32, device=device)
    entry = _lib.lib().cgs_rate_finish_bwd if len(gs) == 1 else _lib.lib().cgs_rate_finish_bwd4
    _lib.check(entry(*[_lib.ptr(None if g is None else _c(g)) for g in gs], levels, *[float(v) for v in finish[:4]], _lib.ptr(dS),
                     _lib.ptr(dh), stream), "cgs_rate_finish_bwd")
    return dS, dh


class _LevelRate(torch.autograd.Function):
    @staticmethod
    def forward(ctx, yf, ys, yo, Q, pred, loc, masks, grows, x_means, use_clamp, K, side, out):
        lv = (_c(yf), _c(ys), _c(yo), _c(Q), _c(pred), loc)
        _lib.require_device(lv[0], lv[4])
        if out is not None:
            sums = torch.empty(0, dtype=_f32, device=yf.device).set_(out.untyped_storage(), out.storage_offset(), (3,), (1,))
        else:
            sums = torch.zeros(3, dtype=_f32, device=yf.device)
        masks = None if masks is None else _c(masks)
        x_means = None if x_means is None else _c(x_means)
        _level_rate_fwd(lv, _lib.ptr(masks), grows, x_means, int(use_clamp), K, _lib.ptr(sums), _lib.current_stream())
        ctx.save_for_backward(*lv, masks, grows, x_means)
        ctx.cfg = (int(use_clamp), K)
        ctx.side = side
        return sums

    @staticmethod
    def backward(ctx, g):
        *lv, masks, grows, x_means = ctx.saved_tensors
        use_clamp, K = ctx.cfg
        loc = lv[5]
        side = ctx.side if loc is not None else None
        d_masks = torch.zeros_like(masks) if (masks is not None and ctx.needs_input_grad[6]) else None
        d, d_pred = _level_rate_bwd(lv, _lib.ptr(masks), grows, x_means, use_clamp, K, _lib.ptr(_c(g)), _lib.ptr(d_masks),
                                    side is not None, _lib.current_stream())
        if side is not None:
            side.give(_sub_map(loc, int(lv[0].shape[0])), *d)
            d = (None,) * 4
        return (*d, d_pred, None, d_masks, None, None, None, None, None, None)


def level_rate(yf, ys, yo, Q, pred, loc, masks, grows, x_means, use_clamp, K, side=None, out=None):
    return _LevelRate.apply(yf, ys, yo, Q, pred, loc, masks, grows, x_means, bool(use_clamp), int(K), side, out)


class _RateFinish(torch.autograd.Function):

    @staticmethod
    def forward(ctx, hsum, cfg, *rows):
        base = rows[0]
        for j, r in enumerate(rows):
            if r.data_ptr() != base.data_ptr() + 12 * j:
                raise ValueError("rate_finish: level sums must be consecutive rows of one table")
        out, raw = _rate_finish_fwd(_lib.ptr(base), len(rows), hsum, cfg, base.device, _lib.current_stream())
        ctx.cfg, ctx.L = cfg, len(rows)
        ctx.mark_non_differentiable(raw)
        return out, raw

    @staticmethod
    def backward(ctx, g, _g_raw):
        dS, dh = _rate_finish_bwd((g,), ctx.L, ctx.cfg, g.device, _lib.current_stream())
        return (dh, None, *dS.unbind(0))


def rate_finish(level_sums, hsum, rate, n_feat, n_scaling, n_offsets, dead_frac):
    return _RateFinish.apply(hsum, (float(rate), float(n_feat), float(n_scaling), float(n_offsets), float(dead_frac)), *level_sums)


class _RateAll(torch.autograd.Function):

    @staticmethod
    def forward(ctx, hsum, masks, x_means, meta, *lv):
        nl = len(lv) // 6
        K, use_clamp = int(meta["K"]), int(bool(meta["use_clamp"]))
        masks, x_means, hsum = _c(masks), _c(x_means), _c(hsum)
        lv = [t.contiguous() if k % 6 == 5 else _c(t) for k, t in enumerate(lv)]
        _lib.require_device(masks, x_means, lv[0], lv[4])
        S = meta.get("sum_table")
        if S is None or tuple(S.shape) != (nl, 3):
            S = torch.zeros(nl, 3, dtype=_f32, device=masks.device)
        stream = _lib.current_stream()
        ctx.lazy = tuple(sd is not None and sd.lazy for sd in meta["sides"])
        for j in range(nl):
            lvj, (lo, hi) = lv[6 * j:6 * j + 6], meta["spans"][j]
            n_sub = int(lvj[5].shape[0])
            assert hi - lo == n_sub and (ctx.lazy[j] or int(lvj[4].shape[0]) == n_sub)
            masks_p, sums_p = masks.data_ptr() + 4 * K * lo, S.data_ptr() + 12 * j
            if not ctx.lazy[j]:
                _level_rate_fwd(lvj, masks_p, None, x_means, use_clamp, K, sums_p, stream)
            elif n_sub > 0:
                _rate_sub_fwd(meta["sides"][j], lvj, masks_p, x_means, use_clamp, sums_p, stream)
        out, raw = _rate_finish_fwd(_lib.ptr(S), nl, hsum, meta["finish"], masks.device, stream)
        ctx.save_for_backward(masks, x_means, *lv)
        ctx.meta = meta
        ctx.mark_non_differentiable(raw)
        ctx.set_materialize_grads(False)
        return out[0], out[1], out[2], out[3], raw

    @staticmethod
    def backward(ctx, g0, g1, g2, g3, _g_raw):
        masks, x_means, *lv = ctx.saved_tensors
        meta, nl = ctx.meta, len(lv) // 6
        K, use_clamp = int(meta["K"]), int(bool(meta["use_clamp"]))
        stream = _lib.current_stream()
        dS, dh = _rate_finish_bwd((g0, g1, g2, g3), nl, meta["finish"], masks.device, stream)
        d_masks = (torch.empty_like if all(ctx.lazy) else torch.zeros_like)(masks) if ctx.needs_input_grad[1] else None
        grads = []
        for j in range(nl):
            lvj, (lo, _hi), side, mp = lv[6 * j:6 * j + 6], meta["spans"][j], meta["sides"][j], meta["maps"][j]
            loc, n_l = lvj[5], int(lvj[0].shape[0])
            masks_p, g_p = masks.data_ptr() + 4 * K * lo, dS.data_ptr() + 12 * j
            d_masks_p = None if d_masks is None else d_masks.data_ptr() + 4 * K * lo
            if ctx.lazy[j]:
                if int(loc.shape[0]) > 0:
                    d, dx, dW = _rate_sub_bwd(side, lvj, masks_p, x_means, use_clamp, K, g_p, d_masks_p, stream)
                    side.give(mp if mp is not None else _sub_map(loc, n_l), *d, dx=dx, dW=dW)
                grads += [None] * 6
                continue
            d, d_pred = _level_rate_bwd(lvj, masks_p, None, x_means, use_clamp, K, g_p, d_masks_p, side is not None, stream)
            if side is not None:
                side.give(mp if mp is not None else _sub_map(loc, n_l), *d)
                d = [None] * 4
            grads += [*d, d_pred, None]
        return (dh, d_masks, None, None, *grads)


def rate_all(hsum, masks, x_means, meta, level_tensors):
    o = _RateAll.apply(hsum, masks, x_means, meta, *level_tensors)
    return o[:4], o[4]


class _CtxAssemble(torch.autograd.Function):

    @staticmethod
    def forward(ctx, anchor, base_f, base_s, own, idx, pos, csr):
        anchor, base_f, base_s, own = _c(anchor), _c(base_f), _c(base_s), _c(own)
        _lib.require_device(anchor, base_f, base_s, own)
        n = idx.shape[0]
        srcs, idxs = [anchor, base_f, base_s, own], [idx, pos, pos, None]
        widths = [int(s.shape[1]) for s in srcs]
        out = torch.empty(n, sum(widths), dtype=_f32, device=anchor.device)
        if n > 0:
            _lib.check(_lib.lib().cgs_rowcat_fwd(4, _ptrs(srcs), _ptrs(idxs), _ints(widths), _ints(widths), n,
                                                 _lib.ptr(out), _lib.current_stream()), "cgs_rowcat_fwd")
        ctx.csr, ctx.widths, ctx.n = csr, widths, n
        ctx.rows = (anchor.shape[0], base_f.shape[0])
        return out

    @staticmethod
    def backward(ctx, g):
        g = _c(g)
        offs, order, prow = ctx.csr
        wa, DF, DS, WO = ctx.widths
        n_anchor, n_par = ctx.rows
        need = ctx.needs_input_grad
        dev = g.device
        d_anchor = torch.zeros(n_anchor, wa, dtype=_f32, device=dev) if need[0] else None
        d_f = torch.empty(n_par, DF, dtype=_f32, device=dev) if need[1] else None
        d_s = torch.empty(n_par, DS, dtype=_f32, device=dev) if need[2] else None
        d_own = None
        if ctx.n > 0:
            if d_anchor is not None or d_f is not None or d_s is not None:
                _lib.check(_lib.lib().cgs_ctx_gather_bwd(_lib.ptr(g), g.shape[1], n_par, _lib.ptr(offs), _lib.ptr(order),
                                                         _lib.ptr(prow), _lib.ptr(d_anchor), _lib.ptr(d_f), _lib.ptr(d_s),
                                                         wa, DF, DS, _lib.current_stream()), "cgs_ctx_gather_bwd")
            if need[3]:
                d_own = g[:, wa + DF + DS:]
        else:
            d_f = None if d_f is None else d_f.zero_()
            d_s = None if d_s is None else d_s.zero_()
            d_own = torch.zeros(0, WO, dtype=_f32, device=dev) if need[3] else None
        return d_anchor, d_f, d_s, d_own, None, None, None


def ctx_assemble(anchor, base_f, base_s, own, idx, pos, csr):
    return _CtxAssemble.apply(anchor, base_f, base_s, own, idx, pos, csr)


def _mask_ste_bwd(x, g):
    d = torch.empty_like(x)
    _lib.check(_lib.lib().cgs_mask_ste_bwd(_lib.ptr(x), _lib.ptr(_c(g)), x.numel(), _lib.ptr(d), _lib.current_stream()),
               "cgs_mask_ste_bwd")
    return d


class _MaskSTE(torch.autograd.Function):

    @staticmethod
    def forward(ctx, logits):
        x = _c(logits)
        _lib.require_device(x)
        n, K = x.shape[0], x[0].numel() if x.shape[0] else 1
        mask = torch.empty_like(x)
        alive = torch.empty(n, dtype=torch.bool, device=x.device)
        _lib.check(_lib.lib().cgs_mask_ste_fwd(_lib.ptr(x), n, K, _lib.ptr(mask), _lib.ptr(alive), _lib.current_stream()),
                   "cgs_mask_ste_fwd")
        ctx.save_for_backward(x)
        ctx.mark_non_differentiable(alive)
        ctx.set_materialize_grads(False)
        return mask, alive

    @staticmethod
    def backward(ctx, g, _g_alive):
        (x,) = ctx.saved_tensors
        return None if g is None else _mask_ste_bwd(x, g)


class _MaskSTEAttach(torch.autograd.Function):

    @staticmethod
    def forward(ctx, logits, values):
        ctx.save_for_backward(logits.detach())
        ctx.set_materialize_grads(False)
        return values.view_as(values)

    @staticmethod
    def backward(ctx, g):
        (x,) = ctx.saved_tensors
        return (None if g is None else _mask_ste_bwd(_c(x), g)), None


def mask_ste_values(logits):
    with torch.no_grad():
        m, alive = _MaskSTE.apply(logits.detach())
    return m, alive


def mask_ste_attach(logits, values):
    return _MaskSTEAttach.apply(logits, values)


def mask_ste(logits):
    return _MaskSTE.apply(logits)


_means3_ws = {}


def means3(a, b, c, exp_b=False):
    a, b, c = _c(a.detach()), _c(b.detach()), _c(c.detach())
    _lib.require_device(a, b, c)
    L = _lib.lib()
    ws = _means3_ws.get(a.device)
    if ws is None:
        ws = _means3_ws[a.device] = torch.empty(L.cgs_means3_scratch_bytes(), dtype=torch.uint8, device=a.device)
    out = torch.empty(3, dtype=_f32, device=a.device)
    _lib.check(L.cgs_means3(_lib.ptr(a), a.numel(), _lib.ptr(b), b.numel(), int(bool(exp_b)), _lib.ptr(c), c.numel(),
                            _lib.ptr(ws), ws.numel(), _lib.ptr(out), _lib.current_stream()), "cgs_means3")
    return out


_PINNED_FREE = []
CHOOSE_SLOTS = 32


def _pinned_i32(k):
    while _PINNED_FREE:
        b = _PINNED_FREE.pop()
        if b.numel() >= k:
            return b
    return torch.empty(max(k, 16), dtype=torch.int32, pin_memory=True)


def choose_rows_begin(perm, n, mask, given, seed, thresh, anchor, anchor_ref, mask_ref, bounds):
    L = _lib.lib()
    dev = (perm if perm is not None else anchor if anchor is not None else mask).device
    mask_u8, given_u8, mref_u8 = _u8(mask), _u8(given), _u8(mask_ref)
    nlev = len(bounds) - 1
    nblk = int(L.cgs_ctx_choose_blocks(n))
    flags = torch.empty(max(n, 1), dtype=torch.uint8, device=dev)
    counts = torch.empty(max(nblk, 1), dtype=torch.int32, device=dev)
    slots, sw = CHOOSE_SLOTS, int(L.cgs_ctx_choose_slot_ints())
    meta = torch.empty(slots * sw, dtype=torch.int32, device=dev)
    b_host = (C.c_int64 * (nlev + 1))(*[int(b) for b in bounds])
    args = (_lib.ptr(perm), n, _lib.ptr(mask_u8), _lib.ptr(given_u8), int(seed), float(thresh),
            _lib.ptr(None if anchor is None else _c(anchor)), _lib.ptr(None if anchor_ref is None else _c(anchor_ref)), _lib.ptr(mref_u8),
# ... 246 lines not shown
```

### include/cgs.h

```cpp
#ifndef CGS_H
#define CGS_H

#include <stddef.h>
#include <stdint.h>

#ifdef __cplusplus
extern "C" {
#endif

#define CGS_VERSION 100

#define CGS_OK 0
#define CGS_ERR_ARG 1
#define CGS_ERR_HIP 2
#define CGS_ERR_WORKSPACE 3
#define CGS_ERR_BOUNDS 4
#define CGS_ERR_RESPEC 5

int cgs_version(void);
const char *cgs_last_error(void);


typedef struct cgs_raster_cfg {
    int32_t image_height;
// ... 295 lines not shown
                        size_t scratch_bytes, uint32_t *overflow, uint32_t epoch, void *stream);

int cgs_prof_enable(int on);
int cgs_prof_count(void);
const char *cgs_prof_name(int id);
int cgs_prof_read(int id, double *total_ms, int64_t *launches);


int cgs_quantize_anchor(const float *anchors, const float *min_v,
                        const float *max_v, int64_t N, int round_digits,
                        float *anchors_q, float *quantized, void *stream);

int cgs_ste_multistep(const float *x, const float *Q, int64_t n, int64_t q_div,
                      int use_clamp, float *out, void *stream);

int cgs_entropy_gaussian_fwd(const float *x, const float *mean,
                             const float *scale, const float *Q, int64_t n,
                             int64_t q_div, const float *x_mean, int use_clamp,
                             float *bits, void *stream);
int cgs_entropy_gaussian_bwd(const float *x, const float *mean,
                             const float *scale, const float *Q, int64_t n,
                             int64_t q_div, const float *x_mean, int use_clamp,
                             const float *g_bits, float *g_x, float *g_mean,
                             float *g_scale, float *g_Q, void *stream);

int cgs_mlp2_forward(int in, int hid, int out, int act, const float *X,
                     int64_t ldx, const float *W1, const float *b1,
                     const float *W2, const float *b2, float *Y, int64_t ldy,
                     float *H, int64_t n, void *stream);
size_t cgs_mlp_wgrad_scratch_bytes(void);
int cgs_mlp2_backward(int in, int hid, int out, int act, const float *X,
                      int64_t ldx, const float *W1, const float *b1, const float *W2,
                      const float *Y, const float *dY, int64_t ldy,
                      const float *H, float *dX, int64_t lddx,
                      int accumulate_dx, float *dZ1, float *dZ2, float *dW1,
                      float *db1, float *dW2, float *db2, int64_t n,
                      void *scratch, size_t scratch_bytes, void *stream);
int cgs_mlp2_backward_rows(int in, int hid, int out, int act, const float *X, int64_t ldx,
                           const float *W1, const float *b1, const float *W2, const float *Y,
                           const float *dY, int64_t ldy, const float *H, float *dX, int64_t lddx,
                           int accumulate_dx, const int64_t *dx_rows, float *dZ1, float *dZ2,
                           float *dW1, float *db1, float *dW2, float *db2, int64_t n,
                           void *scratch, size_t scratch_bytes, void *stream);
int cgs_mlp2_wgrad(int in, int hid, int out, const float *X, int64_t ldx, const float *H,
                   const float *dZ2, int64_t lddz2, const float *dZ1, float *dW1, float *db1,
                   float *dW2, float *db2, int64_t n, void *scratch, size_t scratch_bytes,
                   void *stream);

int cgs_rowcat_fwd(int nsrc, const void *const *data, const int64_t *const *idx,
                   const int *width, const int *ld, int64_t n, float *out,
                   void *stream);
int cgs_rowcat_bwd(int nsrc, void *const *ddata, const int64_t *const *idx,
                   const int *width, const int *ld, const int *mode, int64_t n,
                   const float *dout, void *stream);
int cgs_rowcat_fwd_masked(int nsrc, const void *const *data, const int64_t *const *idx,
                          const uint8_t *const *rowmask, const int *width, const int *ld,
                          int64_t n, float *out, void *stream);
int cgs_rowcat_bwd_masked(int nsrc, void *const *ddata, const int64_t *const *idx,
                          const uint8_t *const *rowmask, const int *width, const int *ld,
                          const int *mode, int64_t n, const float *dout, void *stream);

int cgs_scatter_rows_sorted(const float *g, const int64_t *idx, int64_t n, int64_t N, int w,
                            float *out, void *stream);
int cgs_add_rows(const float *g, const int64_t *idx, int64_t n, int64_t N, int w, float *out,
                 void *stream);
int cgs_gather_rows(const float *x, const int64_t *idx, int64_t n, int w,
                    float *out, void *stream);
int cgs_mark_rows(const int64_t *idx, int64_t n, int64_t n_full, uint32_t gen,
                  uint32_t *stamp, void *stream);
int cgs_zero_unmarked_rows(const uint32_t *stamp, uint32_t gen, int64_t n_full,
                           int narr, float *const *dst, const int *width,
                           void *stream);
int cgs_ctx_gather_bwd(const float *dout, int64_t ldo, int64_t n_parents,
                       const int64_t *offs, const int64_t *order,
                       const int64_t *parent_row, float *d_anchor, float *d_f,
                       float *d_s, int wa, int DF, int DS, void *stream);
int cgs_ctx_gather_bwd_acc(const float *dout, int64_t ldo, int64_t n_parents,
                       const int64_t *offs, const int64_t *order,
                       const int64_t *parent_row, float *d_anchor, float *d_f,
                       float *d_s, int wa, int DF, int DS, int accumulate_anchor, void *stream);
int cgs_noise_quant_fwd(const float *xf, const float *xs, const float *xo,
                        const float *qadj, const int64_t *rows, int64_t n, int D,
                        int S, int O, uint64_t seed, float q0f, float q0s, float q0o,
                        float *yf, float *ys, float *yo, float *Q, double *sums3,
                        void *stream);
int cgs_hyper_noise_gather(const float *hyper, const int64_t *perm, int64_t n, int C,
                           uint64_t seed, float *out, void *stream);
size_t cgs_eb_bits_scratch_bytes(void);
int cgs_eb_bits_fwd(const float *v, const int64_t *rows, const float *raw, int64_t n, int C,
                    void *scratch, size_t scratch_bytes, float *out, void *stream);
int cgs_eb_bits_bwd(const float *v, const int64_t *rows, const float *raw, const float *g_sum,
                    int64_t n, int C, float *g_v_sub, float *g_raw, void *stream);
int cgs_rate_finish_fwd(const float *S, int L, const float *hsum, float rate, double n_feat,
                        double n_scaling, double n_offsets, float dead_frac, float *out4,
                        float *raw, void *stream);
int cgs_rate_finish_bwd(const float *g4, int L, float rate, double n_feat, double n_scaling,
                        double n_offsets, float *dS, float *dh, void *stream);
int cgs_rate_finish_bwd4(const float *g_all, const float *g_feat, const float *g_scaling,
                         const float *g_offsets, int L, float rate, double n_feat, double n_scaling,
                         double n_offsets, float *dS, float *dh, void *stream);
size_t cgs_ctx_choose_blocks(int64_t n);
int cgs_ctx_choose_flags(const int64_t *perm, int64_t n, const uint8_t *mask,
                         const uint8_t *given, uint64_t seed, float thresh,
                         const float *anchor, const float *anchor_ref,
                         const uint8_t *mask_ref, const int64_t *bounds_host, int nlevels,
                         uint8_t *flags, uint32_t *block_counts, int32_t *meta, void *stream);
int cgs_ctx_choose_slot_ints(void);
int cgs_ctx_choose_flags_slots(const int64_t *perm, int64_t n, const uint8_t *mask,
                               const uint8_t *given, uint64_t seed, float thresh,
                               const float *anchor, const float *anchor_ref,
                               const uint8_t *mask_ref, const int64_t *bounds_host, int nlevels,
                               uint8_t *flags, uint32_t *block_counts, int32_t *meta_slots, int nslots, void *stream);
int cgs_ctx_choose_compact(const uint8_t *flags, const uint32_t *block_counts,
                           const int64_t *perm, int64_t n, const int64_t *bounds_host,
                           int nlevels, int64_t *nz, int64_t *rows, int64_t *loc,
                           int32_t *sub_map, const int64_t *chosen_counts_host, void *stream);
size_t cgs_means_accum_doubles(void);
int cgs_means_finalize(double *sums3, int64_t na, int64_t nb, int64_t nc, float *out3,
                       void *stream);
int cgs_noise_quant_bwd(const float *dyf, const float *dys, const float *dyo,
                        const float *dQ_ext, const float *qadj, int64_t n, int D,
                        int S, int O, uint64_t seed, float q0f, float q0s, float q0o,
                        float *dqadj, const int64_t *rows, float *dxf, float *dxs,
                        float *dxo, const int32_t *side_map, const float *side_f,
                        const float *side_s, const float *side_o,
                        const float *side_Q, void *stream);
int cgs_level_rate_fwd(const float *yf, const float *ys, const float *yo,
                       const float *Q, const int64_t *loc, const float *pred,
                       const float *masks, const int64_t *grows,
                       const float *x_means, int use_clamp, int64_t n_sub, int D,
                       int K, int64_t ldpred, float *sums, void *stream);
int cgs_level_rate_bwd(const float *yf, const float *ys, const float *yo,
                       const float *Q, const int64_t *loc, const float *pred,
                       const float *masks, const int64_t *grows,
                       const float *x_means, int use_clamp, int64_t n_sub, int D,
                       int K, int64_t ldpred, const float *g_sums, float *d_pred, float *d_yf,
                       float *d_ys, float *d_yo, float *dQ, float *d_masks,
                       int compact, void *stream);

int cgs_rate_sub_fwd(int in_dim, const float *X, int64_t n, const int64_t *loc, int64_t m,
                     const float *W1, const float *b1, const float *W2, const float *b2,
                     const float *yf, const float *ys, const float *yo, const float *Q,
                     const float *masks, const float *x_means, int use_clamp, float *sums3,
                     void *stream);
size_t cgs_rate_sub_bwd_scratch_bytes(int in_dim, int64_t m);
int cgs_rate_sub_bwd(int in_dim, const float *X, int64_t n, const int64_t *loc, int64_t m,
                     const float *W1, const float *b1, const float *W2, const float *b2,
                     const float *yf, const float *ys, const float *yo, const float *Q,
                     const float *masks, const float *x_means, int use_clamp,
                     const float *g_sums3, float *side_f, float *side_s, float *side_o,
                     float *side_Q, float *dx_sub, float *d_masks, float *dW1, float *db1,
                     float *dW2, float *db2, void *scratch, size_t scratch_bytes, void *stream);

int cgs_ctx_level_fwd(int in_dim, const float *anchor, int64_t n_anchor, const int64_t *a_rows,
                      const uint8_t *a_mask, const float *base_f, const float *base_s, int64_t n_par,
                      const int64_t *pos, const float *hyp, int64_t n, const float *W1, const float *b1, const float *W2q, const float *b2q,
                      const float *xf, const float *xs, const float *xo, const int64_t *rows, uint64_t seed,
                      float q0f, float q0s, float q0o, float *X, float *yf, float *ys, float *yo, float *Q,
                      double *sums3, void *stream);
size_t cgs_ctx_level_bwd_scratch_bytes(void);
int cgs_ctx_level_bwd(int in_dim, const float *X, const float *W1, const float *b1, const float *W2q,
                      const float *b2q, const float *dyf, const float *dys, const float *dyo,
                      const float *dQ_ext, int64_t n, uint64_t seed, float q0f, float q0s, float q0o,
                      const int64_t *rows, int64_t n_anchor, float *dxf, float *dxs, float *dxo,
                      const int32_t *side_map, int64_t m_side, const float *side_f, const float *side_s, const float *side_o, const float *side_Q,
                      const float *dx_sub, float *dX, float *dW1, float *db1, float *dW2q, float *db2q,
                      void *scratch, size_t scratch_bytes, void *stream);
int cgs_ctx_level_bwd2(int in_dim, const float *X, const float *W1, const float *b1, const float *W2q,
                       const float *b2q, const float *dyf, const float *dys, const float *dyo,
                       const float *dQ_ext, int64_t n, uint64_t seed, float q0f, float q0s, float q0o,
                       const int64_t *rows, int64_t n_anchor, float *dxf, float *dxs, float *dxo,
                       const int32_t *side_map, int64_t m_side, const float *side_f, const float *side_s, const float *side_o, const float *side_Q,
                       const float *dx_sub, float *dX, float *d_hyp_rows, float *dW1, float *db1, float *dW2q, float *db2q,
                       void *scratch, size_t scratch_bytes, void *stream);
size_t cgs_ctx_level_hidden_bytes(int64_t n);
int cgs_ctx_level_fwd_h(int in_dim, const float *anchor, int64_t n_anchor, const int64_t *a_rows,
                        const uint8_t *a_mask, const float *base_f, const float *base_s, int64_t n_par,
                        const int64_t *pos, const float *hyp, int64_t n, const float *W1, const float *b1, const float *W2q, const float *b2q,
                        const float *xf, const float *xs, const float *xo, const int64_t *rows, uint64_t seed,
                        float q0f, float q0s, float q0o, float *X, float *yf, float *ys, float *yo, float *Q,
                        double *sums3, float *H, void *stream);
int cgs_ctx_level_bwd_h(int in_dim, const float *X, const float *W1, const float *b1, const float *W2q,
                        const float *b2q, const float *dyf, const float *dys, const float *dyo,
                        const float *dQ_ext, int64_t n, uint64_t seed, float q0f, float q0s, float q0o,
                        const int64_t *rows, int64_t n_anchor, float *dxf, float *dxs, float *dxo,
                        const int32_t *side_map, int64_t m_side, const float *side_f, const float *side_s, const float *side_o, const float *side_Q,
                        const float *dx_sub, float *dX, float *d_hyp_rows, float *dW1, float *db1, float *dW2q, float *db2q,
                        const float *H, void *scratch, size_t scratch_bytes, void *stream);

int cgs_anchor_mlp3_layout(int *out4);

int cgs_anchor_mlp3_forward(const float *X, int64_t ldx,
                            const float *const *W1, const float *const *b1,
                            const float *const *W2, const float *const *b2,
                            float *Y_op, float *Y_color, float *Y_cov,
                            float *Hcat, int64_t n, void *stream);
int cgs_anchor_mlp3_backward(const float *X, int64_t ldx,
                             const float *const *W1, const float *const *W2,
                             const float *Y_op, const float *Y_color,
                             const float *dY_op, const float *dY_color,
                             const float *dY_cov, const float *Hcat, float *dX,
                             int64_t lddx, float *dZ1cat, float *dZ2_op,
                             float *dZ2_color, float *dW1cat, float *db1cat,
                             float *const *dW2, float *const *db2, int64_t n,
                             void *scratch, size_t scratch_bytes, void *stream);
int cgs_anchor_mlp3_forward_rows(const float *feat_src, const int64_t *src_row,
                                 const float *anchor_vis, const float *cam3, float *X_out,
                                 const float *const *W1, const float *const *b1,
                                 const float *const *W2, const float *const *b2, float *Y_op,
                                 float *Y_color, float *Y_cov, float *Hcat, int64_t n, void *stream);
int cgs_anchor_mlp3_backward_rows(const float *X, const float *feat_src, const int64_t *src_row, const float *anchor_vis,
                                  const float *cam3, const float *const *W1, const float *const *W2,
                                  const float *Y_op, const float *Y_color, const float *dY_op,
                                  const float *dY_color, const float *dY_cov, const float *Hcat,
                                  float *d_feat_src, float *d_anchor_vis, float *dZ1cat, float *dZ2_op,
                                  float *dZ2_color, float *dW1cat, float *db1cat, float *const *dW2,
                                  float *const *db2, int64_t n, void *scratch, size_t scratch_bytes,
                                  void *stream);
int cgs_anchor_mlp3_forward_rows_t(const float *feat_src, const int64_t *src_row,
                                   const float *anchor_vis, const float *cam3, float *X_out,
                                   const float *const *W1, const float *const *b1,
                                   const float *const *W2, const float *const *b2, float *Y_op,
                                   float *Y_color, float *Y_cov, float *Hcat, int64_t n, int tiled, void *stream);
int cgs_anchor_mlp3_backward_rows_t(const float *X, const float *feat_src, const int64_t *src_row, const float *anchor_vis,
                                    const float *cam3, const float *const *W1, const float *const *W2,
                                    const float *Y_op, const float *Y_color, const float *dY_op,
                                    const float *dY_color, const float *dY_cov, const float *Hcat,
                                    float *d_feat_src, float *d_anchor_vis, float *dZ1cat, float *dZ2_op,
                                    float *dZ2_color, float *dW1cat, float *db1cat, float *const *dW2,
                                    float *const *db2, int64_t n, int tiled, void *scratch, size_t scratch_bytes,
                                    void *stream);
int cgs_anchor_mlp3_wgrad(const float *X, int64_t ldx, const float *Hcat, const float *dZ1cat,
                          const float *dZ2_op, const float *dZ2_color, const float *dY_cov,
                          float *dW1cat, float *db1cat, float *const *dW2, float *const *db2,
                          int64_t n, void *scratch, size_t scratch_bytes, void *stream);

int cgs_gather_rows_segmented(int nseg, const float *const *src, const int64_t *ld,
                              const int64_t *begin, const int64_t *idx, int64_t n, int w,
                              float *out, void *stream);

int cgs_eb_likelihood_fwd(const float *v, const float *raw, int64_t n, int C,
                          float *lik, void *stream);
int cgs_eb_likelihood_bwd(const float *v, const float *raw, const float *g_lik,
                          int64_t n, int C, float *g_v, float *g_raw,
                          void *stream);

size_t cgs_ac_max_bytes(int64_t n_sym);
int cgs_cdf_float_to_u16_host(const float *cdf, int64_t n_sym, int Lp,
                              uint16_t *out);
int cgs_ac_encode_table_host(const uint16_t *cdf, int Lp, const int16_t *sym,
                             int64_t n_sym, uint8_t *out, size_t out_cap,
                             size_t *out_len);
int cgs_ac_decode_table_host(const uint16_t *cdf, int Lp, int64_t n_sym,
                             const uint8_t *in, size_t in_len,
                             int16_t *sym_out);
int cgs_ac_encode_const_host(const uint16_t *row, int Lp, const int16_t *sym,
                             int64_t n_sym, uint8_t *out, size_t out_cap,
                             size_t *out_len);
int cgs_ac_decode_const_host(const uint16_t *row, int Lp, int64_t n_sym,
                             const uint8_t *in, size_t in_len,
                             int16_t *sym_out);

int cgs_gaussian_stream_minmax(const float *x, const float *Q, int64_t q_div,
                               const int64_t *stream_off, int n_streams,
                               int32_t *min_out, int32_t *max_out,
                               void *stream);
int cgs_gaussian_ac_encode(const float *x, const float *mean,
                           const float *scale, const float *Q, int64_t q_div,
                           const int64_t *stream_off, int n_streams,
                           const int32_t *min_v, const int32_t *max_v,
                           uint8_t *out, const int64_t *out_off,
                           uint32_t *out_len, int32_t *status, void *stream);
int cgs_gaussian_ac_decode(const float *mean, const float *scale,
                           const float *Q, int64_t q_div,
                           const int64_t *stream_off, int n_streams,
                           const int32_t *min_v, const int32_t *max_v,
                           const uint8_t *in, const int64_t *in_off,
                           float *x_out, void *stream);
int cgs_streams_compact(const uint8_t *src, const int64_t *src_off,
                        const uint32_t *len, const int64_t *dst_off,
                        int n_streams, uint8_t *dst, void *stream);
int cgs_pread_ranges(int n, const char *const *paths, const int64_t *file_off,
                     const int64_t *nbytes, void *const *dst, int threads);
int cgs_pwrite_ranges(int n, const char *const *paths, const int64_t *file_off,
                      const int64_t *nbytes, const void *const *src, int threads);
size_t cgs_lanes_block_slot_bytes(int64_t n_symbols, int bytes_per_symbol);
int cgs_gaussian_ac_encode_lanes(const float *x, const float *mean,
                                 const float *scale, const float *Q,
                                 int64_t q_div, const int64_t *blk_off,
                                 int n_blocks, const int32_t *min_v,
                                 const int32_t *max_v, uint8_t *out,
                                 const int64_t *out_off, uint32_t *out_len,
                                 int32_t *status, void *stream);
int cgs_lanes_compact(const uint8_t *src, const int64_t *src_off,
                      const int64_t *blk_off, const int64_t *dst_off,
                      int n_blocks, uint8_t *dst, int bytes_per_symbol,
                      void *stream);
int cgs_gaussian_ac_decode_lanes(const float *mean, const float *scale,
                                 const float *Q, int64_t q_div,
                                 const int64_t *blk_off, int n_blocks,
                                 const int32_t *min_v, const int32_t *max_v,
                                 const uint8_t *in, const int64_t *in_off,
                                 float *x_out, int32_t *status, void *stream);
int cgs_table_ac_encode_lanes(const int32_t *sym, const int64_t *blk_off,
                              const int32_t *blk_ch, int n_blocks,
                              const int32_t *cdf, int max_len,
// ... 192 lines not shown
```

Baseline: 166.3.

## Batch rate-sub levels into single multi-level kernel launches with load-balanced block partition

Per-level rate_sub forward/backward launches are grouped, via a begin/end group API, into one multi-level kernel. Each block looks up its level from a prefix table, and a greedy cost-weighted partition spreads the CU budget across levels. Weight-gradient reductions for several levels are also merged into one sets kernel. This targets launch overhead and under-filled grids on small levels, at the cost of more bookkeeping and deferred-launch state.

```diff
diff --git a/contextgs_amd/_lib.py b/contextgs_amd/_lib.py
--- a/contextgs_amd/_lib.py
+++ b/contextgs_amd/_lib.py
@@ -44,6 +44,12 @@
         ("eps", c_float),
         ("weight_decay", c_float),
     ]
+
+
+class RateSubLevel(C.Structure):
+    _fields_ = [("in_dim", c_int32), ("use_clamp", c_int32), ("n", c_int64), ("m", c_int64)] + [
+        (k, c_void_p) for k in ("X", "loc", "W1", "b1", "W2", "b2", "yf", "ys", "yo", "Q", "masks", "x_means", "sums3", "g_sums3",
+                                "side_f", "side_s", "side_o", "side_Q", "dx_sub", "d_masks", "dW1", "db1", "dW2", "db2")]
 
 
 _BWD_HEAD = [C.POINTER(RasterCfg), c_int64, c_int64]
@@ -214,6 +220,12 @@
     "cgs_rate_sub_bwd_scratch_bytes": (c_size_t, [c_int, c_int64]),
     "cgs_rate_sub_bwd": (c_int, [c_int, c_void_p, c_int64, c_void_p, c_int64] + [c_void_p] * 10 + [c_int] + [c_void_p] * 12 +
                          [c_size_t, c_void_p]),
+    "cgs_rate_sub_fwd_multi": (c_int, [c_int, C.POINTER(RateSubLevel), c_void_p]),
+    "cgs_rate_sub_bwd_multi_scratch_bytes": (c_size_t, [c_int, C.POINTER(RateSubLevel)]),
+    "cgs_rate_sub_bwd_multi": (c_int, [c_int, C.POINTER(RateSubLevel), c_void_p, c_size_t, c_void_p]),
+    "cgs_rate_sub_group_begin": (c_int, []),
+    "cgs_rate_sub_group_end": (c_int, [c_int]),
+    "cgs_rate_sub_partition": (c_int, [c_int, C.POINTER(c_int), C.POINTER(c_int64), c_int, C.POINTER(c_int), C.POINTER(c_int)]),
     "cgs_eb_likelihood_fwd": (c_int, [c_void_p, c_void_p, c_int64, c_int, c_void_p, c_void_p]),
     "cgs_eb_likelihood_bwd": (c_int, [c_void_p, c_void_p, c_void_p, c_int64, c_int, c_void_p, c_void_p, c_void_p]),
     "cgs_ac_max_bytes": (c_size_t, [c_int64]),
diff --git a/contextgs_amd/csrc/cgs_internal.h b/contextgs_amd/csrc/cgs_internal.h
--- a/contextgs_amd/csrc/cgs_internal.h
+++ b/contextgs_amd/csrc/cgs_internal.h
@@ -204,3 +204,6 @@
                            size_t scratch_bytes, hipStream_t s);
 int cgs_launch_wgrad_reduce(const float *partial, int blocks, const CgsWgProduct *prods, int nprod, hipStream_t s);
 int cgs_launch_wgrad_reduce_assign(const float *partial, int blocks, const CgsWgProduct *prods, int nprod, hipStream_t s);
+#define CGS_WG_REDUCE_MAX_SETS 8
+struct CgsWgReduceSet { const float *partial; int blocks; const CgsWgProduct *prods; int nprod; };
+int cgs_launch_wgrad_reduce_assign_sets(const CgsWgReduceSet *sets, int nsets, hipStream_t s);
diff --git a/contextgs_amd/csrc/mlp_wgrad.hip b/contextgs_amd/csrc/mlp_wgrad.hip
--- a/contextgs_amd/csrc/mlp_wgrad.hip
+++ b/contextgs_amd/csrc/mlp_wgrad.hip
@@ -333,11 +333,10 @@
     for (int i = tid; i < a.E; i += 1024) dst[i] = img[i];
 }
 
-__global__ void __launch_bounds__(256)
-    wgrad_multi_reduce_kernel(const float *__restrict__ partial, int blocks, int E, WgmProducts pr, int assign) {
-    __shared__ float s[4][64];
+__device__ __forceinline__ void wgrad_multi_reduce_body(const float *__restrict__ partial, int blocks, int E, const WgmProducts &pr,
+                                                        int assign, int bx, float (*s)[64]) {
     const int tx = threadIdx.x & 63, ty = threadIdx.x >> 6;
-    const int e = blockIdx.x * 64 + tx;
+    const int e = bx * 64 + tx;
     float a0 = 0.f, a1 = 0.f, a2 = 0.f, a3 = 0.f;
     if (e < E) {
         int b = ty;
@@ -366,6 +365,30 @@
         if (le < dadb) dW[le] = assign ? t : dW[le] + t;
         else if (db) db[le - dadb] = assign ? t : db[le - dadb] + t;
     }
+}
+
+__global__ void __launch_bounds__(256)
+    wgrad_multi_reduce_kernel(const float *__restrict__ partial, int blocks, int E, WgmProducts pr, int assign) {
+    __shared__ float s[4][64];
+    wgrad_multi_reduce_body(partial, blocks, E, pr, assign, (int)blockIdx.x, s);
+}
+
+struct WgrSet {
+    const float *partial;
+    int blocks, E;
+    WgmProducts pr;
+};
+struct WgrSets {
+    WgrSet s[CGS_WG_REDUCE_MAX_SETS];
+    int first_block[CGS_WG_REDUCE_MAX_SETS + 1];
+    int nsets;
+};
+__global__ void __launch_bounds__(256) wgrad_multi_reduce_sets_kernel(WgrSets t, int assign) {
+    __shared__ float s[4][64];
+    const int bx = (int)blockIdx.x;
+    int k = 0;
+    for (int q = 1; q < CGS_WG_REDUCE_MAX_SETS; ++q) k += (q < t.nsets && bx >= t.first_block[q]) ? 1 : 0;
+    wgrad_multi_reduce_body(t.s[k].partial, t.s[k].blocks, t.s[k].E, t.s[k].pr, assign, bx - t.first_block[k], s);
 }
 
 #ifndef WG_TAIL_MIN_WAVES
@@ -552,9 +575,7 @@
 int cgs_launch_wgrad_reduce_assign(const float *partial, int blocks, const CgsWgProduct *prods, int nprod, hipStream_t s) {
     return wgrad_reduce_launch(partial, blocks, prods, nprod, 1, s);
 }
-static int wgrad_reduce_launch(const float *partial, int blocks, const CgsWgProduct *prods, int nprod, int assign, hipStream_t s) {
-    if (nprod <= 0 || nprod > WGM_MAX_PROD || blocks <= 0) { cgs_set_error("wgrad_reduce: bad args"); return CGS_ERR_ARG; }
-    WgmProducts pr;
+static int wgrad_reduce_table(const CgsWgProduct *prods, int nprod, WgmProducts &pr) {
     int E = 0;
     for (int k = 0; k < nprod; ++k) {
         pr.dW[k] = prods[k].dW; pr.db[k] = prods[k].db; pr.off[k] = E; pr.dadb[k] = prods[k].DA * prods[k].DB;
@@ -563,7 +584,32 @@
     for (int k = nprod; k < WGM_MAX_PROD; ++k) { pr.dW[k] = nullptr; pr.db[k] = nullptr; pr.off[k] = E; pr.dadb[k] = 0; }
     pr.off[WGM_MAX_PROD] = E;
     pr.nprod = nprod;
+    return E;
+}
+static int wgrad_reduce_launch(const float *partial, int blocks, const CgsWgProduct *prods, int nprod, int assign, hipStream_t s) {
+    if (nprod <= 0 || nprod > WGM_MAX_PROD || blocks <= 0) { cgs_set_error("wgrad_reduce: bad args"); return CGS_ERR_ARG; }
+    WgmProducts pr;
+    const int E = wgrad_reduce_table(prods, nprod, pr);
     hipLaunchKernelGGL(wgrad_multi_reduce_kernel, dim3((unsigned)((E + 63) / 64)), dim3(256), 0, s, partial, blocks, E, pr, assign);
     CGS_CHECK_HIP(hipGetLastError());
     return CGS_OK;
 }
+int cgs_launch_wgrad_reduce_assign_sets(const CgsWgReduceSet *sets, int nsets, hipStream_t s) {
+    if (nsets <= 0 || nsets > CGS_WG_REDUCE_MAX_SETS) { cgs_set_error("wgrad_reduce: bad args"); return CGS_ERR_ARG; }
+    if (nsets == 1) return wgrad_reduce_launch(sets[0].partial, sets[0].blocks, sets[0].prods, sets[0].nprod, 1, s);
+    WgrSets t = {};
+    int grid = 0;
+    for (int k = 0; k < nsets; ++k) {
+        if (sets[k].nprod <= 0 || sets[k].nprod > WGM_MAX_PROD || sets[k].blocks <= 0) { cgs_set_error("wgrad_reduce: bad args"); return CGS_ERR_ARG; }
+        t.s[k].partial = sets[k].partial;
+        t.s[k].blocks = sets[k].blocks;
+        t.s[k].E = wgrad_reduce_table(sets[k].prods, sets[k].nprod, t.s[k].pr);
+        t.first_block[k] = grid;
+        grid += (t.s[k].E + 63) / 64;
+    }
+    for (int k = nsets; k <= CGS_WG_REDUCE_MAX_SETS; ++k) t.first_block[k] = grid;
+    t.nsets = nsets;
+    hipLaunchKernelGGL(wgrad_multi_reduce_sets_kernel, dim3((unsigned)grid), dim3(256), 0, s, t, 1);
+    CGS_CHECK_HIP(hipGetLastError());
+    return CGS_OK;
+}
diff --git a/contextgs_amd/csrc/rate_sub.hip b/contextgs_amd/csrc/rate_sub.hip
--- a/contextgs_amd/csrc/rate_sub.hip
+++ b/contextgs_amd/csrc/rate_sub.hip
@@ -47,7 +47,7 @@
     const float *masks;
     const float *x_means;
     int64_t n, m;
-    int use_clamp;
+    int use_clamp, in_dim;
     float *sums;
     const float *g_sums;
     float *side_f, *side_s, *side_o, *side_Q;
@@ -63,15 +63,17 @@
     f32x4 q3, mk4, mk5;
 };
 
+#define RS_LDS_W1 (RS_OP * RS_SA)
+#define RS_LDS_B1 (RS_LDS_W1 + CL_HP * ClShape<71>::SB)
+#define RS_LDS_B2 (RS_LDS_B1 + CL_HP)
+#define RS_LDS_PART (RS_LDS_B2 + RS_OP)
+#define RS_LDS_FLOATS (RS_LDS_PART + 3 * (RS_WAVES_F > RS_WAVES_B ? RS_WAVES_F : RS_WAVES_B))
+
 template <int IN, bool BWD>
-__global__ void __launch_bounds__((BWD ? RS_WAVES_B : RS_WAVES_F) * 64) rs_main_kernel(RsArgs a) {
+__device__ __forceinline__ void rs_main_body(const RsArgs &a, float *lds, int block, int nblocks) {
     constexpr int RS_WAVES = BWD ? RS_WAVES_B : RS_WAVES_F;
     constexpr int NTI = ClShape<IN>::NTI, XP = ClShape<IN>::XP, SB = ClShape<IN>::SB;
-    __shared__ __attribute__((aligned(16))) float W2n[RS_OP * RS_SA];
-    __shared__ __attribute__((aligned(16))) float W1n[CL_HP * SB];
-    __shared__ float b1s[CL_HP];
-    __shared__ float b2p[RS_OP];
-    __shared__ float part[RS_WAVES][3];
+    float *W2n = lds, *W1n = lds + RS_LDS_W1, *b1s = lds + RS_LDS_B1, *b2p = lds + RS_LDS_B2, *part = lds + RS_LDS_PART;
     const int tid = threadIdx.x, nthr = RS_WAVES * 64;
     for (int i = tid; i < (RS_OP * RS_SA + CL_HP * SB) / 4; i += nthr) {
         float *dst = i < RS_OP * RS_SA / 4 ? W2n + 4 * i : W1n + 4 * (i - RS_OP * RS_SA / 4);
@@ -116,7 +118,7 @@
     }
     __syncthreads();
 
-    const int lane = tid & 63, wave = tid >> 6, g = lane >> 4, c = lane & 15;
+    const int lane = tid & 63, wave = __builtin_amdgcn_readfirstlane(tid >> 6), g = lane >> 4, c = lane & 15;
     const int64_t m = a.m, ntiles = (m + 15) / 16;
     const uint64_t nb = (uint64_t)a.n, mb = (uint64_t)m, tb = (uint64_t)ntiles * 64;
     const ClBuf bX = cl_buf(a.X, nb * IN * 4), bLoc = cl_buf(a.loc, mb * 8), bQ = cl_buf(a.Q, nb * 12),
@@ -139,8 +141,8 @@
         op.mk5 = cl_l64(bM, cl_sel(v && has_masks, (uint32_t)s * (RS_K * 4) + (uint32_t)lo5 * 4));
     };
 
-    const int64_t tstride = (int64_t)gridDim.x * RS_WAVES;
-    int64_t tile = (int64_t)blockIdx.x * RS_WAVES + wave;
+    const int64_t tstride = (int64_t)nblocks * RS_WAVES;
+    int64_t tile = (int64_t)block * RS_WAVES + wave;
     float accb[3] = {0.f, 0.f, 0.f};
     RsOps<IN> opn;
     int64_t rn;
@@ -398,15 +400,39 @@
             float v = accb[k];
 #pragma unroll
             for (int o = 32; o >= 1; o >>= 1) v += __shfl_xor(v, o);
-            if (lane == 0) part[wave][k] = v;
+            if (lane == 0) part[3 * wave + k] = v;
         }
         __syncthreads();
         if (tid < 3) {
             float v = 0.f;
-            for (int w = 0; w < RS_WAVES; ++w) v += part[w][tid];
+            for (int w = 0; w < RS_WAVES; ++w) v += part[3 * w + tid];
             atomicAdd(&a.sums[tid], v);
         }
     }
+}
+
+#define RS_MAX_LEVELS 8
+struct RsMulti {
+    RsArgs lv[RS_MAX_LEVELS];
+    int first_block[RS_MAX_LEVELS + 1];
+    int L;
+};
+
+template <class T>
+__device__ __forceinline__ int rs_level_of(const T &t, int bx) {
+    int level = 0;
+#pragma unroll
+    for (int l = 1; l < RS_MAX_LEVELS; ++l) level += (l < t.L && bx >= t.first_block[l]) ? 1 : 0;
+    return level;
+}
+
+template <bool BWD>
+__global__ void __launch_bounds__((BWD ? RS_WAVES_B : RS_WAVES_F) * 64) rs_main_multi_kernel(RsMulti t) {
+    __shared__ __attribute__((aligned(16))) float lds[RS_LDS_FLOATS];
+    const int bx = (int)blockIdx.x, level = rs_level_of(t, bx);
+    const int block = bx - t.first_block[level], nblocks = t.first_block[level + 1] - t.first_block[level];
+    if (t.lv[level].in_dim == 71) rs_main_body<71, BWD>(t.lv[level], lds, block, nblocks);
+    else rs_main_body<15, BWD>(t.lv[level], lds, block, nblocks);
 }
 
 #define RW_WAVES 8
@@ -414,6 +440,7 @@
     const float *dZ2t, *Ht, *dZ1t, *Xt;
     int64_t ntiles, tiles_per_block;
     float *partial;
+    int in_dim;
 };
 
 template <int NA, int NB>
@@ -460,14 +487,14 @@
 }
 
 template <int IN>
-__global__ void __launch_bounds__(RW_WAVES * 64) rs_wgrad_kernel(RwArgs a) {
+__device__ __forceinline__ void rs_wgrad_body(const RwArgs &a, int block) {
     constexpr int NTI = ClShape<IN>::NTI, XP = ClShape<IN>::XP;
     constexpr int E1 = CL_HID * IN + CL_HID, E = E1 + RS_OUT * CL_HID + RS_OUT;
     const int tid = threadIdx.x, lane = tid & 63, wave = tid >> 6, g = lane >> 4, c = lane & 15;
-    const int64_t t0 = (int64_t)blockIdx.x * a.tiles_per_block;
+    const int64_t t0 = (int64_t)block * a.tiles_per_block;
     const int64_t t1 = t0 + a.tiles_per_block < a.ntiles ? t0 + a.tiles_per_block : a.ntiles;
     const uint64_t tb = (uint64_t)a.ntiles * 64;
-    float *img = a.partial + (int64_t)blockIdx.x * E;
+    float *img = a.partial + (int64_t)block * E;
     float *img1 = img, *imgb1 = img + CL_HID * IN, *img2 = img + E1, *imgb2 = img2 + RS_OUT * CL_HID;
     if (wave < 6) {
         f32x4 acc[2][CL_NT1];
@@ -516,6 +543,19 @@
             for (int i = 0; i < 3; ++i) dump(4 + i, acc[i]);
         }
     }
+}
+
+struct RwMulti {
+    RwArgs lv[RS_MAX_LEVELS];
+    int first_block[RS_MAX_LEVELS + 1];
+    int L;
+};
+
+__global__ void __launch_bounds__(RW_WAVES * 64) rs_wgrad_multi_kernel(RwMulti t) {
+    const int bx = (int)blockIdx.x, level = rs_level_of(t, bx);
+    const int block = bx - t.first_block[level];
+    if (t.lv[level].in_dim == 71) rs_wgrad_body<71>(t.lv[level], block);
+    else rs_wgrad_body<15>(t.lv[level], block);
 }
 
 static int rs_cus() {
@@ -531,41 +571,135 @@
 
 static bool rs_fits(int64_t rows, int64_t row_bytes) { return rows >= 0 && (uint64_t)rows * (uint64_t)row_bytes < CL_MAX_BYTES; }
 
-static int rs_check(const char *what, int in_dim, const float *X, int64_t n, const int64_t *loc, int64_t m, const float *W1,
-                    const float *b1, const float *W2, const float *b2, const float *yf, const float *ys, const float *yo,
-                    const float *Q, const float *x_means, int use_clamp) {
-    if (n < 0 || m < 0 || (in_dim != 71 && in_dim != 15)) { cgs_set_error("%s: bad args (in_dim 71 or 15)", what); return CGS_ERR_ARG; }
-    if (m == 0) return CGS_OK;
-    if (!X || !loc || !W1 || !b1 || !W2 || !b2 || !yf || !ys || !yo || !Q || (use_clamp && !x_means)) { cgs_set_error("%s: NULL", what); return CGS_ERR_ARG; }
-    const int64_t ntiles = (m + 15) / 16;
-    if (!rs_fits(n, in_dim * 4) || !rs_fits(n, CL_D * 4) || !rs_fits(m, CL_D * 4) || !rs_fits(ntiles * 16, RS_OP * 4)) {
-        cgs_set_error("%s: an operand exceeds 4 GB (n %lld, m %lld)", what, (long long)n, (long long)m);
+static int rs_check(const char *what, const cgs_rate_sub_level &v) {
+    if (v.n < 0 || v.m < 0 || (v.in_dim != 71 && v.in_dim != 15)) { cgs_set_error("%s: bad args (in_dim 71 or 15)", what); return CGS_ERR_ARG; }
+    if (v.m == 0) return CGS_OK;
+    if (!v.X || !v.loc || !v.W1 || !v.b1 || !v.W2 || !v.b2 || !v.yf || !v.ys || !v.yo || !v.Q || (v.use_clamp && !v.x_means)) {
+        cgs_set_error("%s: NULL", what);
         return CGS_ERR_ARG;
     }
+    const int64_t ntiles = (v.m + 15) / 16;
+    if (!rs_fits(v.n, v.in_dim * 4) || !rs_fits(v.n, CL_D * 4) || !rs_fits(v.m, CL_D * 4) || !rs_fits(ntiles * 16, RS_OP * 4)) {
+        cgs_set_error("%s: an operand exceeds 4 GB (n %lld, m %lld)", what, (long long)v.n, (long long)v.m);
+        return CGS_ERR_ARG;
+    }
     return CGS_OK;
 }
 
-static int64_t rs_grid(int64_t m, int waves) {
-    const int64_t tiles = (m + 15) / 16, want = (tiles + waves - 1) / waves;
-    return want < rs_cus() ? want : rs_cus();
+static int64_t rs_cost(int in_dim) { return 4 * CL_NT1 * ((in_dim + 15) / 16) + 4 * CL_NT1 * RS_NT2; }
+
+extern "C" int cgs_rate_sub_partition(int L, const int *in_dim, const int64_t *m, int C, int *blocks, int *first_block) {
+    if (L < 0 || L > RS_MAX_LEVELS || C < 1 || (L > 0 && (!in_dim || !m || !blocks)) || !first_block) {
+        cgs_set_error("rate_sub_partition: bad args (at most %d levels)", RS_MAX_LEVELS);
+        return CGS_ERR_ARG;
+    }
+    int64_t cap[RS_MAX_LEVELS], load[RS_MAX_LEVELS];
+    int total = 0;
+    for (int l = 0; l < L; ++l) {
+        if (m[l] < 0 || (in_dim[l] != 71 && in_dim[l] != 15)) { cgs_set_error("rate_sub_partition: bad args (in_dim 71 or 15)"); return CGS_ERR_ARG; }
+        const int64_t tiles = (m[l] + 15) / 16;
+        if (tiles > ((int64_t)1 << 40)) { cgs_set_error("rate_sub_partition: bad args (m %lld)", (long long)m[l]); return CGS_ERR_ARG; }
+        cap[l] = (tiles + 7) / 8;
+        load[l] = tiles * rs_cost(in_dim[l]);
+        blocks[l] = tiles > 0 ? 1 : 0;
+        total += blocks[l];
+    }
+    for (; total < C; ++total) {
+        int best = -1;
+        for (int l = 0; l < L; ++l) {
+            if (blocks[l] == 0 || blocks[l] >= cap[l]) continue;
+            if (best < 0 || load[l] * blocks[best] > load[best] * blocks[l]) best = l;
+        }
+        if (best < 0) break;
+        ++blocks[best];
+    }
+    first_block[0] = 0;
+    for (int l = 0; l < L; ++l) first_block[l + 1] = first_block[l] + blocks[l];
+    return CGS_OK;
+}
+
+static void rs_fill(RsArgs &a, const cgs_rate_sub_level &v) {
+    a = RsArgs{};
+    a.X = v.X; a.loc = v.loc; a.W1 = v.W1; a.b1 = v.b1; a.W2 = v.W2; a.b2 = v.b2; a.yf = v.yf; a.ys = v.ys; a.yo = v.yo; a.Q = v.Q;
+    a.masks = v.masks; a.x_means = v.use_clamp ? v.x_means : nullptr; a.n = v.n; a.m = v.m; a.use_clamp = v.use_clamp ? 1 : 0;
+    a.in_dim = v.in_dim;
+}
+
+template <bool BWD>
+static int rs_main_launch(RsMulti &t, hipStream_t stream) {
+    int in_dim[RS_MAX_LEVELS], blocks[RS_MAX_LEVELS];
+    int64_t m[RS_MAX_LEVELS];
+    for (int l = 0; l < t.L; ++l) { in_dim[l] = t.lv[l].in_dim; m[l] = t.lv[l].m; }
+    int rc = cgs_rate_sub_partition(t.L, in_dim, m, rs_cus(), blocks, t.first_block);
+    if (rc) return rc;
+    for (int l = t.L; l < RS_MAX_LEVELS; ++l) t.first_block[l + 1] = t.first_block[t.L];
+    constexpr int waves = BWD ? RS_WAVES_B : RS_WAVES_F;
+    hipLaunchKernelGGL((rs_main_multi_kernel<BWD>), dim3((unsigned)t.first_block[t.L]), dim3(waves * 64), 0, stream, t);
+    CGS_CHECK_HIP(hipGetLastError());
+    return CGS_OK;
+}
+
+struct RsGroup {
+    bool open, failed;
+    int bwd, L;
+    cgs_rate_sub_level lv[RS_MAX_LEVELS];
+    void *scratch[RS_MAX_LEVELS];
+    void *stream;
+};
+static thread_local RsGroup rs_group;
+
+static int rs_group_record(int bwd, const cgs_rate_sub_level &v, void *scratch, void *stream) {
+    RsGroup &g = rs_group;
+    if (g.L >= RS_MAX_LEVELS || (g.L > 0 && (g.bwd != bwd || g.stream != stream))) {
+        g.failed = true;
+        cgs_set_error("rate_sub group: at most %d calls, all forward or all backward, on one stream", RS_MAX_LEVELS);
+        return CGS_ERR_ARG;
+    }
+    g.bwd = bwd; g.stream = stream; g.lv[g.L] = v; g.scratch[g.L] = scratch;
+    ++g.L;
+    return CGS_OK;
+}
+
+static int rs_fwd_check(const cgs_rate_sub_level &v) {
+    int rc = rs_check("rate_sub_fwd", v);
+    if (rc || v.m == 0) return rc;
+    if (!v.sums3) { cgs_set_error("rate_sub_fwd: NULL"); return CGS_ERR_ARG; }
+    return CGS_OK;
+}
+
+static int rs_fwd_run(int L, const cgs_rate_sub_level *levels, hipStream_t stream) {
+    RsMulti t = {};
+    for (int l = 0; l < L; ++l) {
+        if (levels[l].m == 0) continue;
+        RsArgs &a = t.lv[t.L++];
+        rs_fill(a, levels[l]);
+        a.sums = levels[l].sums3;
+    }
+    if (t.L == 0) return CGS_OK;
+    CgsProfScope prof(CGS_PROF_RATE_FWD, stream);
+    return rs_main_launch<false>(t, stream);
+}
+
+extern "C" int cgs_rate_sub_fwd_multi(int L, const cgs_rate_sub_level *levels, void *stream) {
+    if (L < 0 || L > RS_MAX_LEVELS || (L > 0 && !levels)) { cgs_set_error("rate_sub_fwd: bad args (at most %d levels)", RS_MAX_LEVELS); return CGS_ERR_ARG; }
+    for (int l = 0; l < L; ++l) {
+        int rc = rs_fwd_check(levels[l]);
+        if (rc) return rc;
+    }
+    return rs_fwd_run(L, levels, (hipStream_t)stream);
 }
 
 extern "C" int cgs_rate_sub_fwd(int in_dim, const float *X, int64_t n, const int64_t *loc, int64_t m, const float *W1,
                                 const float *b1, const float *W2, const float *b2, const float *yf, const float *ys,
                                 const float *yo, const float *Q, const float *masks, const float *x_means, int use_clamp,
                                 float *sums3, void *stream) {
-    int rc = rs_check("rate_sub_fwd", in_dim, X, n, loc, m, W1, b1, W2, b2, yf, ys, yo, Q, x_means, use_clamp);
+    cgs_rate_sub_level v = {};
+    v.in_dim = in_dim; v.use_clamp = use_clamp; v.n = n; v.m = m; v.X = X; v.loc = loc; v.W1 = W1; v.b1 = b1; v.W2 = W2; v.b2 = b2;
+    v.yf = yf; v.ys = ys; v.yo = yo; v.Q = Q; v.masks = masks; v.x_means = x_means; v.sums3 = sums3;
+    int rc = rs_fwd_check(v);
     if (rc || m == 0) return rc;
-    if (!sums3) { cgs_set_error("rate_sub_fwd: NULL"); return CGS_ERR_ARG; }
-    RsArgs a = {};
-    a.X = X; a.loc = loc; a.W1 = W1; a.b1 = b1; a.W2 = W2; a.b2 = b2; a.yf = yf; a.ys = ys; a.yo = yo; a.Q = Q; a.masks = masks;
-    a.x_means = use_clamp ? x_means : nullptr; a.n = n; a.m = m; a.use_clamp = use_clamp ? 1 : 0; a.sums = sums3;
-    const unsigned grid = (unsigned)rs_grid(m, RS_WAVES_F);
-    CgsProfScope prof(CGS_PROF_RATE_FWD, (hipStream_t)stream);
-    if (in_dim == 71) hipLaunchKernelGGL((rs_main_kernel<71, false>), dim3(grid), dim3(RS_WAVES_F * 64), 0, (hipStream_t)stream, a);
-    else hipLaunchKernelGGL((rs_main_kernel<15, false>), dim3(grid), dim3(RS_WAVES_F * 64), 0, (hipStream_t)stream, a);
-    CGS_CHECK_HIP(hipGetLastError());
-    return CGS_OK;
+    if (rs_group.open) return rs_group_record(0, v, nullptr, stream);
+    return rs_fwd_run(1, &v, (hipStream_t)stream);
 }
 
 static int64_t rw_blocks(int64_t ntiles) {
@@ -579,6 +713,98 @@
     const int64_t ntiles = (m + 15) / 16, xp = in_dim == 71 ? 80 : 16;
     const int64_t E = (int64_t)CL_HID * in_dim + CL_HID + RS_OUT * CL_HID + RS_OUT;
     return (size_t)(ntiles * 16 * (RS_OP + 2 * CL_HP + xp) + rw_blocks(ntiles) * E) * sizeof(float);
+}
+
+static size_t rs_scratch_start(size_t end) { return (end + 255) / 256 * 256; }
+
+extern "C" size_t cgs_rate_sub_bwd_multi_scratch_bytes(int L, const cgs_rate_sub_level *levels) {
+    size_t end = 0;
+    for (int l = 0; l < L && levels; ++l) {
+        const size_t piece = cgs_rate_sub_bwd_scratch_bytes(levels[l].in_dim, levels[l].m);
+        if (piece) end = rs_scratch_start(end) + piece;
+    }
+    return end;
+}
+
+static int rs_bwd_check(const cgs_rate_sub_level &v, const void *scratch) {
+    int rc = rs_check("rate_sub_bwd", v);
+    if (rc || v.m == 0) return rc;
+    if (!v.g_sums3 || !v.side_f || !v.side_s || !v.side_o || !v.side_Q || !v.dx_sub || !v.dW1 || !v.db1 || !v.dW2 || !v.db2 || !scratch) {
+        cgs_set_error("rate_sub_bwd: NULL");
+        return CGS_ERR_ARG;
+    }
+    return CGS_OK;
+}
+
+static int rs_bwd_run(int L, const cgs_rate_sub_level *levels, void *const *scratch, hipStream_t stream) {
+    RsMulti t = {};
+    RwArgs w[RS_MAX_LEVELS];
+    CgsWgProduct prods[RS_MAX_LEVELS][2];
+    int wgrid[RS_MAX_LEVELS];
+    for (int l = 0; l < L; ++l) {
+        const cgs_rate_sub_level &v = levels[l];
+        if (v.m == 0) continue;
+        const int k = t.L++;
+        const int64_t ntiles = (v.m + 15) / 16, xp = v.in_dim == 71 ? 80 : 16;
+        RsArgs &a = t.lv[k];
+        rs_fill(a, v);
+        a.g_sums = v.g_sums3;
+        a.side_f = v.side_f; a.side_s = v.side_s; a.side_o = v.side_o; a.side_Q = v.side_Q; a.dx_sub = v.dx_sub;
+        a.d_masks = v.masks ? v.d_masks : nullptr;
+        a.dZ2t = (float *)scratch[l]; a.Ht = a.dZ2t + ntiles * 16 * RS_OP; a.dZ1t = a.Ht + ntiles * 16 * CL_HP;
+        a.Xt = a.dZ1t + ntiles * 16 * CL_HP;
+        RwArgs &r = w[k];
+        r.dZ2t = a.dZ2t; r.Ht = a.Ht; r.dZ1t = a.dZ1t; r.Xt = a.Xt; r.ntiles = ntiles; r.partial = a.Xt + ntiles * 16 * xp;
+        r.in_dim = v.in_dim;
+        const int64_t blocks = rw_blocks(ntiles);
+        r.tiles_per_block = (ntiles + blocks - 1) / blocks;
+        wgrid[k] = (int)((ntiles + r.tiles_per_block - 1) / r.tiles_per_block);
+        prods[k][0] = CgsWgProduct{nullptr, 0, CL_HID, nullptr, 0, v.in_dim, v.dW1, v.db1};
+        prods[k][1] = CgsWgProduct{nullptr, 0, RS_OUT, nullptr, 0, CL_HID, v.dW2, v.db2};
+    }
+    if (t.L == 0) return CGS_OK;
+    {
+        CgsProfScope prof(CGS_PROF_RATE_BWD, stream);
+        int rc = rs_main_launch<true>(t, stream);
+        if (rc) return rc;
+    }
+    CgsProfScope prof(CGS_PROF_LMLP_WGRAD, stream);
+    int order[RS_MAX_LEVELS];
+    for (int k = 0; k < t.L; ++k) {
+        int i = k;
+        for (; i > 0 && wgrid[order[i - 1]] > wgrid[k]; --i) order[i] = order[i - 1];
+        order[i] = k;
+    }
+    RwMulti wm = {};
+    CgsWgReduceSet sets[RS_MAX_LEVELS];
+    for (int i = 0; i < t.L; ++i) {
+        const int k = order[i];
+        wm.lv[i] = w[k];
+        wm.first_block[i + 1] = wm.first_block[i] + wgrid[k];
+        sets[i] = CgsWgReduceSet{w[k].partial, wgrid[k], prods[k], 2};
+    }
+    for (int i = t.L; i < RS_MAX_LEVELS; ++i) wm.first_block[i + 1] = wm.first_block[t.L];
+    wm.L = t.L;
+    hipLaunchKernelGGL(rs_wgrad_multi_kernel, dim3((unsigned)wm.first_block[t.L]), dim3(RW_WAVES * 64), 0, stream, wm);
+    CGS_CHECK_HIP(hipGetLastError());
+    return cgs_launch_wgrad_reduce_assign_sets(sets, t.L, stream);
+}
+
+extern "C" int cgs_rate_sub_bwd_multi(int L, const cgs_rate_sub_level *levels, void *scratch, size_t scratch_bytes, void *stream) {
+    if (L < 0 || L > RS_MAX_LEVELS || (L > 0 && !levels)) { cgs_set_error("rate_sub_bwd: bad args (at most %d levels)", RS_MAX_LEVELS); return CGS_ERR_ARG; }
+    void *piece[RS_MAX_LEVELS] = {};
+    size_t end = 0;
+    for (int l = 0; l < L; ++l) {
+        const cgs_rate_sub_level &v = levels[l];
+        int rc = rs_bwd_check(v, scratch);
+        if (rc) return rc;
+        if (v.m == 0) continue;
+        const size_t start = rs_scratch_start(end);
+        end = start + cgs_rate_sub_bwd_scratch_bytes(v.in_dim, v.m);
+        if (end > scratch_bytes) { cgs_set_error("rate_sub_bwd: scratch too small"); return CGS_ERR_WORKSPACE; }
+        piece[l] = (char *)scratch + start;
+    }
+    return rs_bwd_run(L, levels, piece, (hipStream_t)stream);
 }
 
 extern "C" int cgs_rate_sub_bwd(int in_dim, const float *X, int64_t n, const int64_t *loc, int64_t m, const float *W1,
@@ -587,38 +813,30 @@
                                 const float *g_sums3, float *side_f, float *side_s, float *side_o, float *side_Q, float *dx_sub,
                                 float *d_masks, float *dW1, float *db1, float *dW2, float *db2, void *scratch, size_t scratch_bytes,
                                 void *stream) {
-    int rc = rs_check("rate_sub_bwd", in_dim, X, n, loc, m, W1, b1, W2, b2, yf, ys, yo, Q, x_means, use_clamp);
+    cgs_rate_sub_level v = {};
+    v.in_dim = in_dim; v.use_clamp = use_clamp; v.n = n; v.m = m; v.X = X; v.loc = loc; v.W1 = W1; v.b1 = b1; v.W2 = W2; v.b2 = b2;
+    v.yf = yf; v.ys = ys; v.yo = yo; v.Q = Q; v.masks = masks; v.x_means = x_means; v.g_sums3 = g_sums3;
+    v.side_f = side_f; v.side_s = side_s; v.side_o = side_o; v.side_Q = side_Q; v.dx_sub = dx_sub; v.d_masks = d_masks;
+    v.dW1 = dW1; v.db1 = db1; v.dW2 = dW2; v.db2 = db2;
+    int rc = rs_bwd_check(v, scratch);
     if (rc) return rc;
     if (m == 0) { cgs_set_error("rate_sub_bwd: m == 0 (the caller zero-fills the weight gradients of an empty subset)"); return CGS_ERR_ARG; }
-    if (!g_sums3 || !side_f || !side_s || !side_o || !side_Q || !dx_sub || !dW1 || !db1 || !dW2 || !db2 || !scratch) {
-        cgs_set_error("rate_sub_bwd: NULL");
-        return CGS_ERR_ARG;
-    }
     if (scratch_bytes < cgs_rate_sub_bwd_scratch_bytes(in_dim, m)) { cgs_set_error("rate_sub_bwd: scratch too small"); return CGS_ERR_WORKSPACE; }
-    const int64_t ntiles = (m + 15) / 16, xp = in_dim == 71 ? 80 : 16;
-    float *ws = (float *)scratch;
-    RsArgs a = {};
-    a.X = X; a.loc = loc; a.W1 = W1; a.b1 = b1; a.W2 = W2; a.b2 = b2; a.yf = yf; a.ys = ys; a.yo = yo; a.Q = Q; a.masks = masks;
-    a.x_means = use_clamp ? x_means : nullptr; a.n = n; a.m = m; a.use_clamp = use_clamp ? 1 : 0; a.g_sums = g_sums3;
-    a.side_f = side_f; a.side_s = side_s; a.side_o = side_o; a.side_Q = side_Q; a.dx_sub = dx_sub; a.d_masks = masks ? d_masks : nullptr;
-    a.dZ2t = ws; a.Ht = a.dZ2t + ntiles * 16 * RS_OP; a.dZ1t = a.Ht + ntiles * 16 * CL_HP; a.Xt = a.dZ1t + ntiles * 16 * CL_HP;
-    float *partial = a.Xt + ntiles * 16 * xp;
-    const unsigned grid = (unsigned)rs_grid(m, RS_WAVES_B);
-    {
-        CgsProfScope prof(CGS_PROF_RATE_BWD, (hipStream_t)stream);
-        if (in_dim == 71) hipLaunchKernelGGL((rs_main_kernel<71, true>), dim3(grid), dim3(RS_WAVES_B * 64), 0, (hipStream_t)stream, a);
-        else hipLaunchKernelGGL((rs_main_kernel<15, true>), dim3(grid), dim3(RS_WAVES_B * 64), 0, (hipStream_t)stream, a);
-        CGS_CHECK_HIP(hipGetLastError());
-    }
-    CgsProfScope prof(CGS_PROF_LMLP_WGRAD, (hipStream_t)stream);
-    RwArgs w;
-    w.dZ2t = a.dZ2t; w.Ht = a.Ht; w.dZ1t = a.dZ1t; w.Xt = a.Xt; w.ntiles = ntiles; w.partial = partial;
-    const int64_t blocks = rw_blocks(ntiles);
-    w.tiles_per_block = (ntiles + blocks - 1) / blocks;
-    const unsigned wgrid = (unsigned)((ntiles + w.tiles_per_block - 1) / w.tiles_per_block);
-    if (in_dim == 71) hipLaunchKernelGGL((rs_wgrad_kernel<71>), dim3(wgrid), dim3(RW_WAVES * 64), 0, (hipStream_t)stream, w);
-    else hipLaunchKernelGGL((rs_wgrad_kernel<15>), dim3(wgrid), dim3(RW_WAVES * 64), 0, (hipStream_t)stream, w);
-    CGS_CHECK_HIP(hipGetLastError());
-    const CgsWgProduct prods[2] = {{nullptr, 0, CL_HID, nullptr, 0, in_dim, dW1, db1}, {nullptr, 0, RS_OUT, nullptr, 0, CL_HID, dW2, db2}};
-    return cgs_launch_wgrad_reduce_assign(partial, (int)wgrid, prods, 2, (hipStream_t)stream);
-}
+    if (rs_group.open) return rs_group_record(1, v, scratch, stream);
+    return rs_bwd_run(1, &v, &scratch, (hipStream_t)stream);
+}
+
+extern "C" int cgs_rate_sub_group_begin(void) {
+    if (rs_group.open) { cgs_set_error("rate_sub group: already open on this thread"); return CGS_ERR_ARG; }
+    rs_group.open = true; rs_group.failed = false; rs_group.bwd = -1; rs_group.L = 0;
+    return CGS_OK;
+}
+
+extern "C" int cgs_rate_sub_group_end(int launch) {
+    RsGroup &g = rs_group;
+    if (!g.open) { cgs_set_error("rate_sub group: not open on this thread"); return CGS_ERR_ARG; }
+    g.open = false;
+    if (!launch || g.L == 0) return CGS_OK;
+    if (g.failed) { cgs_set_error("rate_sub group: a call of the group was refused"); return CGS_ERR_ARG; }
+    return g.bwd ? rs_bwd_run(g.L, g.lv, g.scratch, (hipStream_t)g.stream) : rs_fwd_run(g.L, g.lv, (hipStream_t)g.stream);
+}
diff --git a/contextgs_amd/ctx_ops.py b/contextgs_amd/ctx_ops.py
--- a/contextgs_amd/ctx_ops.py
+++ b/contextgs_amd/ctx_ops.py
@@ -1,5 +1,6 @@
 from __future__ import annotations
 
+import contextlib
 import ctypes as C
 import itertools
 import threading
@@ -428,20 +429,48 @@
         "cgs_rate_sub_fwd")
 
 
-def _rate_sub_bwd(side, lv, masks_p, x_means, use_clamp, K, g_p, d_masks_p, stream):
-    Lc = _lib.lib()
+def _rate_sub_bwd_buffers(levels, K):
+    Lc, dev = _lib.lib(), levels[0][1][0].device
+    shapes = []
+    for side, lv in levels:
+        X, W = side.loan()
+        n_sub, in_f = int(lv[5].shape[0]), int(X.shape[1])
+        ws = int(Lc.cgs_rate_sub_bwd_scratch_bytes(in_f, n_sub))
+        shapes.append((n_sub, (int(lv[0].shape[1]), 6, 3 * K, 3, in_f), W, (ws + 255) // 256 * 256))
+    rows = torch.split(torch.empty(sum(n * sum(ws_) for n, ws_, _, _ in shapes), dtype=_f32, device=dev),
+                       [n * w for n, ws_, _, _ in shapes for w in ws_])
+    wg = torch.split(torch.empty(sum(w.numel() for _, _, W, _ in shapes for w in W), dtype=_f32, device=dev),
+                     [w.numel() for _, _, W, _ in shapes for w in W])
+    scr = torch.split(torch.empty(sum(b for *_, b in shapes), dtype=torch.uint8, device=dev), [b for *_, b in shapes])
+    out = []
+    for j, (n, widths, W, _) in enumerate(shapes):
+        *d, dx = [t.view(n, w) for t, w in zip(rows[5 * j:5 * j + 5], widths)]
+        out.append((d, dx, tuple(t.view(w.shape) for t, w in zip(wg[4 * j:4 * j + 4], W)), scr[j]))
+    return out
+
+
+def _rate_sub_bwd(side, lv, masks_p, x_means, use_clamp, g_p, d_masks_p, bufs, stream):
     yf, ys, yo, Q, _pred, loc = lv
     X, W = side.loan()
-    n_sub, in_f, dev = int(loc.shape[0]), int(X.shape[1]), yf.device
-    *d, dx = _carve(n_sub, (int(yf.shape[1]), 6, 3 * K, 3, in_f), dev)
-    wflat = torch.empty(sum(w.numel() for w in W), dtype=_f32, device=dev)
-    dW = tuple(t.view(w.shape) for t, w in zip(torch.split(wflat, [w.numel() for w in W]), W))
-    ws = torch.empty(int(Lc.cgs_rate_sub_bwd_scratch_bytes(in_f, n_sub)), dtype=torch.uint8, device=dev)
-    _lib.check(Lc.cgs_rate_sub_bwd(
-        in_f, _lib.ptr(X), int(X.shape[0]), _lib.ptr(loc), n_sub, *[_lib.ptr(w) for w in W], _lib.ptr(yf), _lib.ptr(ys), _lib.ptr(yo),
-        _lib.ptr(Q), masks_p, _lib.ptr(x_means), use_clamp, g_p, *[_lib.ptr(t) for t in d], _lib.ptr(dx), d_masks_p,
-        *[_lib.ptr(t) for t in dW], _lib.ptr(ws), ws.numel(), stream), "cgs_rate_sub_bwd")
+    d, dx, dW, ws = bufs
+    _lib.check(_lib.lib().cgs_rate_sub_bwd(
+        int(X.shape[1]), _lib.ptr(X), int(X.shape[0]), _lib.ptr(loc), int(loc.shape[0]), *[_lib.ptr(w) for w in W], _lib.ptr(yf),
+        _lib.ptr(ys), _lib.ptr(yo), _lib.ptr(Q), masks_p, _lib.ptr(x_means), use_clamp, g_p, *[_lib.ptr(t) for t in d], _lib.ptr(dx),
+        d_masks_p, *[_lib.ptr(t) for t in dW], _lib.ptr(ws), ws.numel(), stream), "cgs_rate_sub_bwd")
     return d, dx, dW
+
+
+@contextlib.contextmanager
+def _rate_sub_group():
+    Lc = _lib.lib()
+    _lib.check(Lc.cgs_rate_sub_group_begin(), "cgs_rate_sub_group_begin")
+    done = False
+    try:
+        yield
+        done = True
+    finally:
+        rc = Lc.cgs_rate_sub_group_end(int(done))
+    _lib.check(rc, "cgs_rate_sub_group_end")
 
 
 def _rate_finish_fwd(table_p, levels, hsum, finish, device, stream):
@@ -534,15 +563,16 @@
             S = torch.zeros(nl, 3, dtype=_f32, device=masks.device)
         stream = _lib.current_stream()
         ctx.lazy = tuple(sd is not None and sd.lazy for sd in meta["sides"])
-        for j in range(nl):
-            lvj, (lo, hi) = lv[6 * j:6 * j + 6], meta["spans"][j]
-            n_sub = int(lvj[5].shape[0])
-            assert hi - lo == n_sub and (ctx.lazy[j] or int(lvj[4].shape[0]) == n_sub)
-            masks_p, sums_p = masks.data_ptr() + 4 * K * lo, S.data_ptr() + 12 * j
-            if not ctx.lazy[j]:
-                _level_rate_fwd(lvj, masks_p, None, x_means, use_clamp, K, sums_p, stream)
-            elif n_sub > 0:
-                _rate_sub_fwd(meta["sides"][j], lvj, masks_p, x_means, use_clamp, sums_p, stream)
+        with _rate_sub_group():
+            for j in range(nl):
+                lvj, (lo, hi) = lv[6 * j:6 * j + 6], meta["spans"][j]
+                n_sub = int(lvj[5].shape[0])
+                assert hi - lo == n_sub and (ctx.lazy[j] or int(lvj[4].shape[0]) == n_sub)
+                masks_p, sums_p = masks.data_ptr() + 4 * K * lo, S.data_ptr() + 12 * j
+                if not ctx.lazy[j]:
+                    _level_rate_fwd(lvj, masks_p, None, x_means, use_clamp, K, sums_p, stream)
+                elif n_sub > 0:
+                    _rate_sub_fwd(meta["sides"][j], lvj, masks_p, x_means, use_clamp, sums_p, stream)
         out, raw = _rate_finish_fwd(_lib.ptr(S), nl, hsum, meta["finish"], masks.device, stream)
         ctx.save_for_backward(masks, x_means, *lv)
         ctx.meta = meta
@@ -559,22 +589,25 @@
         dS, dh = _rate_finish_bwd((g0, g1, g2, g3), nl, meta["finish"], masks.device, stream)
         d_masks = (torch.empty_like if all(ctx.lazy) else torch.zeros_like)(masks) if ctx.needs_input_grad[1] else None
         grads = []
-        for j in range(nl):
-            lvj, (lo, _hi), side, mp = lv[6 * j:6 * j + 6], meta["spans"][j], meta["sides"][j], meta["maps"][j]
-            loc, n_l = lvj[5], int(lvj[0].shape[0])
-            masks_p, g_p = masks.data_ptr() + 4 * K * lo, dS.data_ptr() + 12 * j
-            d_masks_p = None if d_masks is None else d_masks.data_ptr() + 4 * K * lo
-            if ctx.lazy[j]:
-                if int(loc.shape[0]) > 0:
-                    d, dx, dW = _rate_sub_bwd(side, lvj, masks_p, x_means, use_clamp, K, g_p, d_masks_p, stream)
-                    side.give(mp if mp is not None else _sub_map(loc, n_l), *d, dx=dx, dW=dW)
-                grads += [None] * 6
-                continue
-            d, d_pred = _level_rate_bwd(lvj, masks_p, None, x_means, use_clamp, K, g_p, d_masks_p, side is not None, stream)
-            if side is not None:
-                side.give(mp if mp is not None else _sub_map(loc, n_l), *d)
-                d = [None] * 4
-            grads += [*d, d_pred, None]
+        sub = [j for j in range(nl) if ctx.lazy[j] and int(lv[6 * j + 5].shape[0]) > 0]
+        bufs = dict(zip(sub, _rate_sub_bwd_buffers([(meta["sides"][j], lv[6 * j:6 * j + 6]) for j in sub], K))) if sub else {}
+        with _rate_sub_group():
+            for j in range(nl):
+                lvj, (lo, _hi), side, mp = lv[6 * j:6 * j + 6], meta["spans"][j], meta["sides"][j], meta["maps"][j]
+                loc, n_l = lvj[5], int(lvj[0].shape[0])
+                masks_p, g_p = masks.data_ptr() + 4 * K * lo, dS.data_ptr() + 12 * j
+                d_masks_p = None if d_masks is None else d_masks.data_ptr() + 4 * K * lo
+                if ctx.lazy[j]:
+                    if j in bufs:
+                        d, dx, dW = _rate_sub_bwd(side, lvj, masks_p, x_means, use_clamp, g_p, d_masks_p, bufs[j], stream)
+                        side.give(mp if mp is not None else _sub_map(loc, n_l), *d, dx=dx, dW=dW)
+                    grads += [None] * 6
+                    continue
+                d, d_pred = _level_rate_bwd(lvj, masks_p, None, x_means, use_clamp, K, g_p, d_masks_p, side is not None, stream)
+                if side is not None:
+                    side.give(mp if mp is not None else _sub_map(loc, n_l), *d)
+                    d = [None] * 4
+                grads += [*d, d_pred, None]
         return (dh, d_masks, None, None, *grads)
 
 
diff --git a/include/cgs.h b/include/cgs.h
--- a/include/cgs.h
+++ b/include/cgs.h
@@ -471,6 +471,25 @@
                      float *side_Q, float *dx_sub, float *d_masks, float *dW1, float *db1,
                      float *dW2, float *db2, void *scratch, size_t scratch_bytes, void *stream);
 
+typedef struct cgs_rate_sub_level {
+    int32_t in_dim, use_clamp;
+    int64_t n, m;
+    const float *X;
+    const int64_t *loc;
+    const float *W1, *b1, *W2, *b2, *yf, *ys, *yo, *Q, *masks, *x_means;
+    float *sums3;
+    const float *g_sums3;
+    float *side_f, *side_s, *side_o, *side_Q, *dx_sub, *d_masks, *dW1, *db1, *dW2, *db2;
+} cgs_rate_sub_level;
+int cgs_rate_sub_fwd_multi(int L, const cgs_rate_sub_level *levels, void *stream);
+size_t cgs_rate_sub_bwd_multi_scratch_bytes(int L, const cgs_rate_sub_level *levels);
+int cgs_rate_sub_bwd_multi(int L, const cgs_rate_sub_level *levels, void *scratch,
+                           size_t scratch_bytes, void *stream);
+int cgs_rate_sub_partition(int L, const int *in_dim, const int64_t *m, int C, int *blocks,
+                           int *first_block);
+int cgs_rate_sub_group_begin(void);
+int cgs_rate_sub_group_end(int launch);
+
 int cgs_ctx_level_fwd(int in_dim, const float *anchor, int64_t n_anchor, const int64_t *a_rows,
                       const uint8_t *a_mask, const float *base_f, const float *base_s, int64_t n_par,
                       const int64_t *pos, const float *hyp, int64_t n, const float *W1, const float *b1, const float *W2q, const float *b2q,
```

Measured after the change: 169.7 (median of 6 runs). 1.02x the previous value.
